# PytorchConnectomics/pytorch_connectomics

Measured on AMD Instinct MI355X. Metric: voxels/s (train + sliding-window infer), MedNeXt-S 112^3 bf16, higher is better.
Workload: dtype bf16; 1 GPU; Lucchi++ sliding-window inference (configs[1]): MedNeXt-S k3, 165x1024x768 volume, roi 112^3, overlap 0.5, bump blending, sw_batch_size 8, random-init weights; step = one whole-volume EagerSlidingWindowEngine call (TTA off); value = window-voxels/s; sw_batch_size=8, window_pipeline_streams=3

## Files before the change

### include/pytc_hip.h

```cpp
#ifndef PYTC_HIP_H
#define PYTC_HIP_H

#include <stdint.h>

#ifdef __cplusplus
extern "C" {
#endif

#define PYTC_ABI_VERSION 12

#define PYTC_OK 0
#define PYTC_ERR_INVALID 1
#define PYTC_ERR_HIP 2
#define PYTC_ERR_UNSUPPORTED 3

#define PYTC_F32 0
#define PYTC_BF16 1

#define PYTC_VIEW_FLIP_Z 1
#define PYTC_VIEW_FLIP_Y 2
#define PYTC_VIEW_FLIP_X 4
#define PYTC_VIEW_SWAP_YX 8
#define PYTC_VIEW_SWAP_ZY 16
#define PYTC_VIEW_SWAP_ZX 32

#define PYTC_PAD_CONSTANT 0
#define PYTC_PAD_REFLECT 1
#define PYTC_PAD_REPLICATE 2
#define PYTC_PAD_CIRCULAR 3

#define PYTC_BLEND_PRODUCT 0
#define PYTC_BLEND_MIN 1

#define PYTC_ACT_NONE 0
#define PYTC_ACT_SIGMOID 1
#define PYTC_ACT_TANH 2
#define PYTC_ACT_GELU 3

#define PYTC_RES_NONE 0
#define PYTC_RES_ADD 1
#define PYTC_RES_UPSAMPLE 2
#define PYTC_RES_GELU_BWD 3
#define PYTC_RES_NORM_BWD 4

int pytc_abi_version(void);
const char* pytc_last_error(void);
int pytc_device_info(int device, int* cu_count, int* lds_bytes_per_cu, char* arch, int arch_len);
int pytc_set_tuning(const char* key, int value);


int pytc_gather_windows(const float* vol, int C, int Z, int Y, int X, const int32_t* starts, int B,
                        int rz, int ry, int rx, int view, int pad_mode, float cval, void* out,
                        int out_dtype, void* stream);

int pytc_blend_accumulate(const void* pred, int pred_dtype, int B, const int32_t* starts, int rz,
                          int ry, int rx, int C, int view, const float* wz, const float* wy,
                          const float* wx, int combine, float floor_w, const int32_t* border ,
                          float* value, float* weight, int Z, int Y, int X, void* stream);

int pytc_blend_accumulate_mapped(const void* pred, int pred_dtype, int B, const int32_t* starts, int rz, int ry,
                                 int rx, int C, int view, const float* wz, const float* wy, const float* wx,
                                 int combine, float floor_w, const int32_t* border, const int32_t* chan_src,
                                 const int32_t* chan_shift, float* value, float* weight, int Z, int Y, int X,
                                 void* stream);
int pytc_blend_weight_shifted(int B, const int32_t* starts, int rz, int ry, int rx, const float* wz, const float* wy,
                              const float* wx, int combine, float floor_w, const int32_t* border,
                              const int32_t* shift, float* weight, int Z, int Y, int X, void* stream);
int pytc_normalize_covered(float* value, const float* weight, int64_t n, void* stream);
int pytc_ensemble_update_masked(float* stat, float* count, const float* x, const float* cover, int64_t n, int mode,
                                void* stream);
int pytc_ensemble_finalize_masked(const float* stat, const float* count, float* out, int64_t n, int mode, void* stream);

int pytc_blend_finalize(float* value, const float* weight, int C, int64_t nvox, float clamp,
                        int act, void* stream);

#define PYTC_ACT_SOFTMAX 4
int pytc_channel_activation(float* value, int C, int64_t nvox, int channels_last, int c0, int c1, int act,
                            float scale, void* stream);

int pytc_ensemble_update(float* acc, const float* x, int64_t n, int mode, int count, void* stream);

#define PYTC_ST_U8 0
#define PYTC_ST_I8 1
#define PYTC_ST_U16 2
#define PYTC_ST_I16 3
#define PYTC_ST_I32 4
#define PYTC_ST_F16 5
#define PYTC_ST_F32 6
int pytc_scale_cast(const float* x, void* y, int64_t n, float scale, int target, void* stream);


#define PYTC_RAW_U8 0
#define PYTC_RAW_I8 1
#define PYTC_RAW_U16 2
#define PYTC_RAW_I16 3
#define PYTC_RAW_U32 4
#define PYTC_RAW_I32 5
#define PYTC_RAW_F32 6
#define PYTC_RAW_F64 7
int pytc_resample_region(const void* raw, int raw_dtype, const int64_t* strides_czyx, int C, const int32_t* tab_i0,
                         const int32_t* tab_i1, const float* tab_f, const int32_t* dims_zyx, float* out, void* stream);

#define PYTC_NORM_NONE 0
#define PYTC_NORM_ZSCORE 1
#define PYTC_NORM_MINMAX 2
#define PYTC_NORM_DIVIDE 3
int64_t pytc_window_normalize_ws_elems(int B, int64_t n);
int pytc_window_normalize(float* x, int B, int64_t n, int mode, int binarize, float threshold, float divide, const float* clip,
                          double* workspace, void* stream);


int pytc_dwconv3d_stat_slots(int N, int D, int H, int W, int C, int K, int stride, int dtype,
                             int transposed);

int pytc_dwconv3d_kernel_variant(int N, int D, int H, int W, int C, int K, int stride, int dtype, int transposed);

int pytc_dwconv3d_fwd(const void* x, void* y, const float* w, const float* bias, float* stats,
                      int N, int D, int H, int W, int C, int K, int stride, int dtype,
                      void* stream);

int pytc_dwconv3d_fwd_wide(const void* x, void* y, const float* w, const float* bias, float* stats, int N, int D, int H,
                           int W, int C, int K, int stride, int dtype, void* stream);

int pytc_dwconv3d_res_supported(int D, int H, int W, int C, int K, int stride, int dtype);

int pytc_dwmix_supported(int D, int H, int W, int C, int C_hid, int C_out, int dtype);
int pytc_dwmix_fwd(const void* x, const float* taps, const float* dw_bias, const void* w2n, const float* b2n, const void* w3_f16,
                   const float* b3, int residual, void* y, const void* head_w, const float* head_b, float* head_y, int n_head, int N,
                   int D, int H, int W, int C, int C_hid, int C_out, int dtype, void* stream);
int pytc_dwconv3d_fwd_res(const void* x, const void* res, void* y, const float* w, const float* bias, int N, int D, int H,
                          int W, int C, int K, int stride, int dtype, void* stream);

int pytc_dwconvT3d_fwd(const void* x, void* y, const float* w, const float* bias, float* stats,
                       int N, int D, int H, int W, int C, int K, int dtype, void* stream);

int pytc_groupnorm_finalize(const float* stats, int slots, float count, const float* gamma,
                            const float* beta, float eps, float* ab, int N, int C, void* stream);


int64_t pytc_pw_packed_elems(int C_out, int C_in, int dtype);
int pytc_pw_pack_weight(const float* w, int C_out, int C_in, int transposed, void* packed,
                        int dtype, void* stream);

typedef struct {
  const void* x;
  const void* w_packed;
  const float* bias;
  const float* ab;
  const void* res;
  void* y;
  int N;
  int64_t rows_per_sample;
  int C_in, C_out;
  int in_dtype, out_dtype, w_dtype;
  int act;
  int res_mode;
  int gather;
  int Di, Hi, Wi;
  const void* res_low;
  const float* res_bias;
  int pre_act;
  int w_paired;
} pytc_pw_args;

int pytc_pw_conv_fwd(const pytc_pw_args* a, void* stream);
int pytc_pw_conv_paired_supported(const pytc_pw_args* a);
int pytc_pw_conv_rowmajor_supported(const pytc_pw_args* a);

typedef struct {
  const void* t;
  const float* ab;
  const void* w2_packed;
  const float* b2;
  const void* w3_packed;
  const float* b3;
  const void* res;
  const void* res_low;
  const float* res_bias;
  void* y;
  int N;
  int64_t rows_per_sample;
  int C_in, C_hid, C_out;
  int res_mode;
  int Di, Hi, Wi;
  int w3_format;
  int per_sample;
} pytc_mlp_args;
#define PYTC_W3_BF16 0
#define PYTC_W3_F16 1

int pytc_pw_gemm_supported(int C_in, int C_out);
int pytc_pw_gemm_fwd(const void* x, const void* w, const float* bias, const float* ab, void* y, int N, int64_t rows_per_sample,
                     int C_in, int C_out, int in_f16, int gelu_out, const void* res, const void* res_low, const float* res_bias,
                     int res_mode, int Di, int Hi, int Wi, void* stream);
int pytc_pw_mlp_supported(int C_in, int C_hid, int C_out);
int pytc_pw_pack_weight_paired(const float* w, int C_out, int C_in, int transposed, void* packed_bf16,
                               void* stream);
int pytc_pack_multi(const int64_t* table_dev, int n_items, int64_t total_elems, void* stream);
int pytc_pw_pack_weight_paired_f16(const float* w, int C_out, int C_in, int transposed, void* packed_f16,
                                   void* stream);
int pytc_pw_mlp_fwd(const pytc_mlp_args* a, void* stream);

int pytc_pw_mlp_lds_supported(int C_in, int C_hid, int C_out);
int pytc_pw_mlp_lds_fwd(const pytc_mlp_args* a, void* stream);
int pytc_pw_mlp_dma_applies(const pytc_mlp_args* a, int ignore_res_mode);
int pytc_pw_mlp_proj_supported(int C_in, int C_hid, int C_out, int C_proj);
int pytc_pw_mlp_proj_fwd(const pytc_mlp_args* a, const void* proj_w, const float* proj_b, void* z, int store_y, void* stream);
int pytc_pw_mlp_chunk_supported(int C_in, int C_hid, int C_out);
int pytc_pw_mlp_chunk_fwd(const pytc_mlp_args* a, void* stream);
int pytc_groupnorm_fold_mlp(const float* stats, int slots, float count, const float* gamma, const float* beta, float eps,
                            const float* w2, const float* b2, void* w2n, float* b2n, float* ab_out, int N, int C, int C_hid,
                            void* stream);
int pytc_pw_mlp_train_fwd(const pytc_mlp_args* a, void* hidden_pre, void* stream);
int pytc_pw_mlp_train_fwd_nostore(const pytc_mlp_args* a, void* stream);
int pytc_pw_mlp_bwd(const pytc_mlp_args* a, const void* hidden_pre, void* d_hidden, void* stream);
int pytc_pw_mlp_up_supported(int C_in, int C_hid, int C_out);
int pytc_pw_mlp_up_fwd(const pytc_mlp_args* a, const float* taps, const float* dw_bias, void* stream);
int pytc_pw_mlp_head_supported(int C_in, int C_hid, int C_out);
int pytc_pw_mlp_stemres_fwd(const pytc_mlp_args* a, const float* stem_x, const float* stem_w, const float* stem_b,
                            void* stream);
int pytc_stem_dwconv3d_stat_slots(int D, int H, int W);
int pytc_stem_dwconv3d_supported(int C_in, int C, int K);
int pytc_stem_dwconv3d_mfma_image_bytes(void);
int pytc_stem_dwconv3d_pack_mfma(const float* wx, const float* wb, const float* cst, void* image, void* stream);
int pytc_stem_dwconv3d_fwd(const float* x, const float* wx, const float* wb, const float* cst, const void* mfma_image, void* y,
                           float* stats, int N, int D, int H, int W, int C, void* stream);
int pytc_pw_mlp_head_fwd(const pytc_mlp_args* a, const void* head_w, const float* head_b, float* head_y, int n_head,
                         int store_y, void* stream);


#define PYTC_ACT_RELU 5
#define PYTC_ACT_LEAKY 6
#define PYTC_ACT_ELU 7

typedef struct {
  const void* x;
  const void* w_packed;
  const float* bias;
  const float* ab;
  const void* res;
  void* y;
  int N, D, H, W, C_in, C_out;
  int kd, kh, kw;
  int act_in;
  float act_param;
  int res_mode;
  int dtype;
} pytc_conv3d_args;

int64_t pytc_conv3d_packed_elems(int C_out, int C_in, int kd, int kh, int kw, int dtype);
int pytc_conv3d_pack_weight(const float* w, int C_out, int C_in, int kd, int kh, int kw, void* packed, int dtype,
                            void* stream);
int pytc_conv3d_fwd(const pytc_conv3d_args* a, void* stream);

int pytc_channel_stats_slots(int64_t rows);
int pytc_channel_stats(const void* x, float* stats, int N, int64_t rows, int C, int dtype, void* stream);
int pytc_norm_finalize_groups(const float* stats, int slots, float count, const float* gamma, const float* beta,
                              float eps, int groups, float* ab, int N, int C, void* stream);
int pytc_affine_act(const void* x, void* y, const float* ab, int N, int64_t rows, int C, int act, float prm,
                    int dtype, void* stream);
int pytc_maxpool3d_fwd(const void* x, void* y, int N, int D, int H, int W, int C, int fz, int fy, int fx, int dtype,
                       void* stream);
int pytc_dwconvT3d_generic_fwd(const void* x, void* y, const float* w, int N, int D, int H, int W, int C,
                               const int32_t* kernel, const int32_t* stride, const int32_t* pad, int dtype,
                               void* stream);


int pytc_groupnorm_finalize_mr(const float* stats, int slots, float count, const float* gamma, const float* beta,
                               float eps, float* ab, float* mean_rstd, int N, int C, void* stream);
int pytc_gelu(const void* x, const void* dy, void* out, int64_t n, int dtype, void* stream);
int pytc_add_inplace(void* y, const void* x, int64_t n, int dtype, void* stream);
int pytc_pw_wgrad_slots(int64_t rows_total);
int pytc_pw_wgrad(const void* x, const float* ab, const void* dy, float* dW, float* db, float* workspace, int N,
                  int64_t rows_per_sample, int C_in, int C_out, int dtype, int x_act , void* stream);
int pytc_dw_wgrad_slots(int N, const int32_t* gdims, const int32_t* xdims, int C, int K, int stride, int dtype);
int pytc_dw_wgrad(const void* g, const void* x, float* dW, float* db, float* workspace, int N, const int32_t* gdims,
                  const int32_t* xdims, int C, int K, int stride, int dtype, void* stream);

int pytc_pw_wgrad_partial(const void* x, const float* ab, const void* dy, float* workspace, int want_db, int N,
                          int64_t rows_per_sample, int C_in, int C_out, int dtype, int x_act, int* slots_out, void* stream);
int pytc_pw_wgrad_dgrad_supported(int C_in, int C_out, int dtype);
int pytc_pw_wgrad_dgrad_partial(const void* x, const void* dy, const void* w_t_paired, void* dx, float* workspace, int want_db, int N,
                                int64_t rows_per_sample, int C_in, int C_out, int dtype, int* slots_out, void* stream);
int pytc_mixer_bwd_rc_supported(int C, int C_hid, int C_out, int dtype);
int pytc_mixer_bwd_rc_sps(int N, int64_t rows_per_sample, int C_hid);
int64_t pytc_mixer_bwd_rc_ws_elems(int N, int64_t rows_per_sample, int C_hid, int gn);
int pytc_mixer_bwd_rc(const void* t, const float* ab, const float* mean_rstd, const void* dy, const void* w2_paired, const float* b2,
                      const void* w3t_paired, const float* W2, const float* gamma, float count, void* dhp, float* workspace,
                      float* s_out, float* coef, int want_db3, int gn, int N, int64_t rows_per_sample, int C, int C_hid, int C_out,
                      int dtype, int* slots_out, void* stream);
int pytc_dw_wgrad_partial(const void* g, const void* x, float* workspace, int want_db, int N, const int32_t* gdims,
                          const int32_t* xdims, int C, int K, int stride, int dtype, int* slots_out, void* stream);
int pytc_copy_zero_front(const void* src, void* dst, int N, const int32_t* dims, int C, int dtype, void* stream);
typedef struct {
  const float* part;
  float* out;
  int64_t n;
  int32_t slots;
  int32_t out_t;
} pytc_reduce_item;
int pytc_reduce_slots_multi(const pytc_reduce_item* items, int n_items, void* stream);
int pytc_norm_bwd_ws_elems(int N, int64_t rows, int C);
int pytc_norm_bwd(const void* dtn, const void* t, const float* mean_rstd, const float* gamma, float* stats_ws,
                  float* s_out, void* dt, int N, int64_t rows, float count , int C,
                  int dtype, void* stream);
int pytc_pw_wgrad_groupnorm_supported(int C, int C_hid, int dtype);
int pytc_pw_wgrad_groupnorm_sps(int N, int64_t rows_per_sample, int C, int C_hid);
int64_t pytc_pw_wgrad_groupnorm_ws_elems(int N, int64_t rows_per_sample, int C, int C_hid);
int pytc_pw_wgrad_groupnorm(const void* t, const float* mean_rstd, const float* ab, const void* dhp, const float* W2,
                            const float* gamma, float count, float* s_out, float* coef, float* workspace, int N,
                            int64_t rows_per_sample, int C, int C_hid, int dtype, void* stream);
int pytc_norm_bwd_apply(const void* dtn, const void* t, const float* mean_rstd, const float* gamma, const float* s_in,
                        int s_parts, void* dt, int N, int64_t rows, int C, float count, int dtype, const int32_t* crop_grid,
                        void* stream);
int pytc_dwconv3d_bwd_data(const void* dy, const float* w, void* dx, int N, const int32_t* xdims,
                           const int32_t* ydims, int C, int K, int stride, int dtype, void* stream);
int pytc_dwconv3d_bwd_data_add(const void* dy, const float* w, const void* addend, void* dx, int N, const int32_t* xdims,
                               const int32_t* ydims, int C, int K, int stride, int dtype, void* stream);

int pytc_conv3d_pack_weight_dgrad(const float* w, int C_out, int C_in, int kd, int kh, int kw, void* packed, int dtype,
                                  void* stream);
int pytc_conv3d_pack_plan(int C_out, int C_in, int kd, int kh, int kw, int dtype, int direct, int64_t* out);
int pytc_conv3d_pack_multi(const int64_t* table_dev, int n_items, int64_t total_blocks, void* stream);
int pytc_conv3d_launch_plan(int N, int D, int H, int W, int C_in, int C_out, int kd, int kh, int kw, int dtype, int has_pre,
                            int has_res, int phase, int64_t* out);
int pytc_norm_bwd_means(const float* s, const float* gamma, float* M, float* dgamma, float* dbeta, int N, int C, int groups,
                        float rows, void* stream);
int pytc_bn_train_finalize_cpad(const float* stats, int slots_total, float count, const float* gamma, const float* beta, float eps,
                                float momentum, float* running_mean, float* running_var, int64_t* num_batches_tracked, float* ab,
                                float* mean_rstd, int N, int C, int C_real, void* stream);
int pytc_norm_finalize_groups_cpg(const float* stats, int slots, float count, const float* gamma, const float* beta, float eps,
                                  int groups, int cpg, float* ab, float* mr, int N, int C, void* stream);
int pytc_norm_bwd_means_cpg(const float* s, const float* gamma, float* M, float* dgamma, float* dbeta, int N, int C, int groups,
                            int cpg, float rows, void* stream);
int pytc_bn_train_finalize(const float* stats, int slots_total, float count, const float* gamma, const float* beta, float eps,
                           float momentum, float* running_mean, float* running_var, int64_t* num_batches_tracked, float* ab,
                           float* mean_rstd, int N, int C, void* stream);
int pytc_bn_update_running(const float* mean_rstd, float* running_mean, float* running_var, int C, float count, float eps,
                           float momentum, void* stream);
int64_t pytc_conv3d_wgrad_ws_elems(int N, int D, int H, int W, int C_in, int C_out, const int32_t* kernel, int dtype);
int pytc_conv3d_wgrad(const void* a, const void* dy, float* dW, float* workspace, int N, int D, int H, int W, int C_in,
                      int C_out, const int32_t* kernel, int dtype, void* stream);
int pytc_act_bwd(const void* da, const void* x, const float* ab, void* dt, void* dp, int N, int64_t rows, int C, int act,
                 float prm, int dtype, void* stream);
int pytc_norm_finalize_groups_mr(const float* stats, int slots, float count, const float* gamma, const float* beta,
                                 float eps, int groups, float* ab, float* mr, int N, int C, void* stream);
int pytc_norm_bwd_stats(const void* dtn, const void* t, const float* mean_rstd, float* stats_ws, float* s_out, int N,
                        int64_t rows, int C, int dtype, void* stream);
int pytc_norm_bwd_apply_general(const void* d, const void* x, const float* mean_rstd, const float* gamma, const float* M,
                                void* dx, int N, int64_t rows, int C, int dtype, void* stream);
int pytc_act_norm_bwd_stats(const void* da, const void* x, const float* ab, const float* mean_rstd, float* stats_ws, float* s_out,
                            float* p_ws, float* p_out, int N, int64_t rows, int C, int act, float prm, int dtype, void* stream);
int pytc_act_norm_bwd_apply(const void* da, const void* x, const float* ab, const float* mean_rstd, const float* gamma,
                            const float* M, void* dx, int N, int64_t rows, int C, int act, float prm, int dtype, void* stream);
int pytc_act_norm_bwd_apply_cg(const void* da, const void* x, const float* ab, const float* mean_rstd, const float* gamma, int C_gamma,
                               const float* M, void* dx, int N, int64_t rows, int C, int act, float prm, int dtype, void* stream);
int pytc_maxpool3d_bwd(const void* x, const void* dy, void* dx, int N, int D, int H, int W, int C, int fz, int fy, int fx,
                       int dtype, void* stream);
int pytc_dwconv3d_generic_fwd(const void* x, void* y, const float* w, int N, int D, int H, int W, int C,
                              const int32_t* kernel, const int32_t* stride, const int32_t* pad, const int32_t* out_dims,
                              int dtype, void* stream);

int64_t pytc_conv3d_direct_packed_elems(int C_out, int C_in, int kd, int kh, int kw, int dtype);
int pytc_conv3d_pack_weight_direct(const float* w, int C_out, int C_in, int kd, int kh, int kw, int64_t s_o, int64_t s_c,
                                   int flip, void* packed, int dtype, void* stream);
int pytc_convT3d_c1_fwd(const void* x, const float* w, const float* bias, void* y, float* workspace, int N, const int32_t* in_dims,
                        int C_in, int dtype, void* stream);
int pytc_convT3d_phase_plan(int C_out, int C_in, int dtype, int64_t* out);
int pytc_convT3d_phase_supported(int C_out, int C_in, int dtype);
int pytc_convT3d_phase_fwd(const pytc_conv3d_args* a, const int32_t* in_dims, void* stream);
int pytc_conv3d_strided_fwd(const pytc_conv3d_args* a, const int32_t* in_dims, const int32_t* stride, const int32_t* pad,
                            int transposed, void* stream);
int64_t pytc_conv3d_wgrad_strided_ws_elems(int N, const int32_t* small_dims, int C_k, int C_o, const int32_t* kernel);
// ... 159 lines not shown
```

### pytorch_connectomics_amd/csrc/pw_common.h

```cpp
#pragma once
#include "pytc_common.h"

namespace pytc {

template <typename TW>
struct Mma;

template <>
struct Mma<bf16_t> {
  static constexpr int EPL = 8;
  static constexpr int KSTEP = 32;
  typedef bf16x8_t frag_t;
  static __device__ __forceinline__ f32x4_t mma(frag_t a, frag_t b, f32x4_t c) {
    return __builtin_amdgcn_mfma_f32_16x16x32_bf16(a, b, c, 0, 0, 0);
  }
  static __device__ __forceinline__ frag_t from_floats(const float (&v)[8]) {
    f32x8_t f;
#pragma unroll
    for (int i = 0; i < 8; ++i) f[i] = v[i];
    return __builtin_convertvector(f, frag_t);
  }
};

template <>
struct Mma<float> {
  static constexpr int EPL = 4;
  static constexpr int KSTEP = 16;
  typedef f32x4_t frag_t;
  static __device__ __forceinline__ f32x4_t mma(frag_t a, frag_t b, f32x4_t c) {
#pragma unroll
    for (int s = 0; s < 4; ++s) c = __builtin_amdgcn_mfma_f32_16x16x4f32(a[s], b[s], c, 0, 0, 0);
    return c;
  }
  static __device__ __forceinline__ frag_t from_floats(const float (&v)[4]) {
    frag_t f;
#pragma unroll
    for (int i = 0; i < 4; ++i) f[i] = v[i];
    return f;
  }
};

static_assert(Mma<bf16_t>::KSTEP == mfma_kstep(PYTC_BF16) && Mma<float>::KSTEP == mfma_kstep(PYTC_F32) &&
                  Mma<bf16_t>::EPL == elems_per_16b(PYTC_BF16) && Mma<float>::EPL == elems_per_16b(PYTC_F32),
              "the host helpers of pytc_common.h must agree with the fragment traits");

__host__ __device__ __forceinline__ int paired_row(int T, int m) {
  return (T >> 1) * 32 + (m >> 2) * 8 + (T & 1) * 4 + (m & 3);
}

struct EpiParams {
  const void* res;
  const void* res_low;
  const float* res_bias;
  void* y;
  long rps_out;
  int C_out;
  int res_mode;
  int Go_d, Go_h, Go_w;
  int Gl_d, Gl_h, Gl_w;
  int nt;
};

typedef unsigned int pytc_u32x4_t __attribute__((ext_vector_type(4)));
template <typename V>
__device__ __forceinline__ V ld_stream(const V* ptr, int nt) {
  static_assert(sizeof(V) == 16, "16-byte row pieces");
  if (nt) return __builtin_bit_cast(V, __builtin_nontemporal_load(reinterpret_cast<const pytc_u32x4_t*>(ptr)));
  return *ptr;
}

template <typename TO, int NCH, bool GELU_BWD = false, int COUT = 0>
__device__ __forceinline__ void finish_and_store(float (&v)[NCH], const EpiParams& e, int n, long orow, int o0,
                                                 const float* pre = nullptr, const int* pos = nullptr) {
  const int C_out = COUT > 0 ? COUT : e.C_out;
  TO* yn = reinterpret_cast<TO*>(e.y) + (long)n * e.rps_out * C_out;
  const TO* resn = e.res ? reinterpret_cast<const TO*>(e.res) + (long)n * e.rps_out * C_out : nullptr;
  const long off = orow * C_out + o0;
  const bool full = (C_out % NCH) == 0 && (o0 + NCH <= C_out);
  if (e.res_mode == PYTC_RES_ADD) {
    float rv[NCH];
    if (pre) {
#pragma unroll
      for (int i = 0; i < NCH; ++i) rv[i] = pre[i];
    } else if (full) VecIO<TO, NCH>::load(resn + off, rv);
    else {
#pragma unroll
      for (int i = 0; i < NCH; ++i) rv[i] = (o0 + i < C_out) ? to_f32<TO>(resn[off + i]) : 0.f;
    }
#pragma unroll
    for (int i = 0; i < NCH; ++i) v[i] += rv[i];
  } else if (GELU_BWD && e.res_mode == PYTC_RES_GELU_BWD) {
    float rv[NCH];
    if (pre) {
#pragma unroll
      for (int i = 0; i < NCH; ++i) rv[i] = pre[i];
    } else if (full) VecIO<TO, NCH>::load(resn + off, rv);
    else {
#pragma unroll
      for (int i = 0; i < NCH; ++i) rv[i] = (o0 + i < C_out) ? to_f32<TO>(resn[off + i]) : 0.f;
    }
#pragma unroll
    for (int i = 0; i < NCH; ++i) v[i] *= gelu_erf_grad(rv[i]);
  } else if (GELU_BWD && e.res_mode == PYTC_RES_NORM_BWD) {
    float rv[NCH];
    if (pre) {
#pragma unroll
      for (int i = 0; i < NCH; ++i) rv[i] = pre[i];
    } else if (full) VecIO<TO, NCH>::load(resn + off, rv);
    else {
#pragma unroll
      for (int i = 0; i < NCH; ++i) rv[i] = (o0 + i < C_out) ? to_f32<TO>(resn[off + i]) : 0.f;
    }
    const float* cf = e.res_bias + (long)n * 3 * C_out + o0;
#pragma unroll
    for (int i = 0; i < NCH; ++i)
      if (o0 + i < C_out) v[i] = fmaf(cf[i], v[i], fmaf(cf[C_out + i], rv[i], cf[2 * C_out + i]));
    if (e.Go_w > 0) {
      const unsigned ur = (unsigned)orow, gw = (unsigned)e.Go_w, gh = (unsigned)e.Go_h;
      const unsigned tq = ur / gw;
      const int px = (int)(ur - tq * gw), pz = (int)(tq / gh), py = (int)(tq - (unsigned)pz * gh);
      if (px == 0 || py == 0 || pz == 0) return;
      const long crow = ((long)(pz - 1) * (e.Go_h - 1) + (py - 1)) * (e.Go_w - 1) + (px - 1);
      TO* yc = reinterpret_cast<TO*>(e.y) + ((long)n * (e.Go_d - 1) * (e.Go_h - 1) * (e.Go_w - 1) + crow) * C_out + o0;
      if (full) VecIO<TO, NCH>::store(yc, v);
      else {
#pragma unroll
        for (int i = 0; i < NCH; ++i)
          if (o0 + i < C_out) yc[i] = from_f32<TO>(v[i]);
      }
      return;
    }
  } else if (e.res_mode == PYTC_RES_UPSAMPLE) {
    int px, py, pz;
    if (pos) { pz = pos[0]; py = pos[1]; px = pos[2]; }
    else {
      const unsigned ur = (unsigned)orow, gw = (unsigned)e.Go_w, gh = (unsigned)e.Go_h;
      const unsigned t = ur / gw;
      px = (int)(ur - t * gw);
      pz = (int)(t / gh);
      py = (int)(t - (unsigned)pz * gh);
    }
    float sk[NCH];
    if (pre) {
#pragma unroll
      for (int i = 0; i < NCH; ++i) sk[i] = pre[i];
    } else if (full) VecIO<TO, NCH>::load(resn + off, sk);
    else {
#pragma unroll
      for (int i = 0; i < NCH; ++i) sk[i] = (o0 + i < C_out) ? to_f32<TO>(resn[off + i]) : 0.f;
    }
    if (px == 0 || py == 0 || pz == 0) {
#pragma unroll
      for (int i = 0; i < NCH; ++i) v[i] = sk[i];
    } else {
      const int oz = pz - 1, oy = py - 1, ox = px - 1;
      float rl[NCH];
      if (e.res_low && !((oz | oy | ox) & 1)) {
        const TO* rp = reinterpret_cast<const TO*>(e.res_low) +
                       ((((long)n * e.Gl_d + (oz >> 1)) * e.Gl_h + (oy >> 1)) * e.Gl_w + (ox >> 1)) * C_out + o0;
        if (full) VecIO<TO, NCH>::load(rp, rl);
        else {
#pragma unroll
          for (int i = 0; i < NCH; ++i) rl[i] = (o0 + i < C_out) ? to_f32<TO>(rp[i]) : 0.f;
        }
      } else {
#pragma unroll
        for (int i = 0; i < NCH; ++i) rl[i] = (e.res_bias && o0 + i < C_out) ? e.res_bias[o0 + i] : 0.f;
      }
#pragma unroll
      for (int i = 0; i < NCH; ++i) v[i] = v[i] + rl[i] + sk[i];
    }
  }
  if (full) {
    if constexpr (sizeof(TO) == 2 && NCH == 8) {
      if (e.nt) {
        f32x8_t f;
#pragma unroll
        for (int i = 0; i < 8; ++i) f[i] = v[i];
        __builtin_nontemporal_store(__builtin_convertvector(f, bf16x8_t), reinterpret_cast<bf16x8_t*>(yn + off));
        return;
      }
    }
    VecIO<TO, NCH>::store(yn + off, v);
  } else {
#pragma unroll
    for (int i = 0; i < NCH; ++i)
      if (o0 + i < C_out) yn[off + i] = from_f32<TO>(v[i]);
  }
}

template <typename TI, int EPL>
__device__ __forceinline__ void load_row_frag(const TI* __restrict__ row, int k0, int C_in, bool vec_ok,
                                              float (&v)[EPL]) {
  if (vec_ok && k0 + EPL <= C_in) {
    if constexpr (sizeof(TI) == 4 && EPL == 8) {
      float t0[4], t1[4];
      VecIO<float, 4>::load(reinterpret_cast<const float*>(row) + k0, t0);
      VecIO<float, 4>::load(reinterpret_cast<const float*>(row) + k0 + 4, t1);
#pragma unroll
      for (int i = 0; i < 4; ++i) { v[i] = t0[i]; v[4 + i] = t1[i]; }
    } else {
      VecIO<TI, EPL>::load(row + k0, v);
    }
  } else {
#pragma unroll
    for (int j = 0; j < EPL; ++j) v[j] = (k0 + j < C_in) ? to_f32<TI>(row[k0 + j]) : 0.f;
  }
}

template <int PER>
struct WarmRegs { unsigned int r[2 * PER]; };
template <int PER>
__device__ __forceinline__ void warm_l2(const void* base, long bytes, WarmRegs<PER>& w, int first) {
  const long lines = (bytes + 127) >> 7;
  const long lin = (long)blockIdx.z * gridDim.y * gridDim.x + (long)blockIdx.y * gridDim.x + blockIdx.x;
  const long total = (long)gridDim.x * gridDim.y * gridDim.z;
  const long per_xcd = (total + 7) >> 3;
  const long stride = per_xcd * blockDim.x;
  long l = (lin >> 3) * blockDim.x + threadIdx.x;
#pragma unroll
  for (int it = 0; it < PER; ++it, l += stride) {
    const long lc = l < lines ? l : lines - 1;
    const char* ptr = reinterpret_cast<const char*>(base) + (lc << 7);
    asm volatile("global_load_dword %0, %1, off" : "=v"(w.r[first + it]) : "v"(ptr) : "memory");
  }
}
template <int PER>
__device__ __forceinline__ void warm_l2_done(WarmRegs<PER>& w) {
  asm volatile("s_waitcnt vmcnt(0)" : : : "memory");
#pragma unroll
  for (int i = 0; i < 2 * PER; ++i) asm volatile("" : : "v"(w.r[i]) : "memory");
}

__device__ __forceinline__ float apply_act(float t, int act) {
  if (act == PYTC_ACT_GELU) return gelu_erf(t);
  if (act == PYTC_ACT_SIGMOID) return 1.f / (1.f + __expf(-t));
  if (act == PYTC_ACT_TANH) return tanhf(t);
  return t;
}

}
```

### pytorch_connectomics_amd/csrc/pw_fast_kernels.hip

```cpp
#include "pw_common.h"

namespace pytc {

struct PwFastParams {
  const bf16_t* x;
  const bf16x8_t* w;
  const float* bias;
  const float* ab;
  EpiParams e;
  long rps, rps_in;
  int C_in, C_out, pre_act;
  int gather, Hi, Wi, Ho, Wo;
};

constexpr int pw_fast_waves(int ks, int nt) {
  return nt == 4 ? (ks <= 2 ? 3 : 2) : (ks <= 4 ? 4 : (ks <= 16 ? 3 : 1));
}

template <int KS, int NT>
__global__ void __launch_bounds__(256, pw_fast_waves(KS, NT))
pw_fast_kernel(PwFastParams p) {
  const int wave = threadIdx.x >> 6, lane = threadIdx.x & 63;
  const int n = blockIdx.y;
  constexpr bool WARM = KS >= 4;
  WarmRegs<2> warm;
  if (WARM) {
    const long wbytes = (long)p.C_out * p.C_in * 2;
    warm_l2(p.w, wbytes, warm, 0);
    warm_l2(reinterpret_cast<const char*>(p.w) + (wbytes >> 1), wbytes >> 1, warm, 2);
  }
  const long row0 = ((long)blockIdx.x * 4 + wave) * (NT * 16);
  if (row0 >= p.rps) {
    if (WARM) asm volatile("s_waitcnt vmcnt(0)" : : : "memory");
    return;
  }
  const int r = lane & 15, kb = lane >> 4;
  long orow[NT];
#pragma unroll
  for (int nt = 0; nt < NT; ++nt) orow[nt] = row0 + nt * 16 + r;

  bf16x8_t bact[KS][NT];
  const bf16_t* xn = p.x + (long)n * p.rps_in * p.C_in;
  {
    uint4 raw[KS][NT];
#pragma unroll
    for (int ks = 0; ks < KS; ++ks)
#pragma unroll
      for (int nt = 0; nt < NT; ++nt) {
        long rr = orow[nt] < p.rps ? orow[nt] : p.rps - 1;
        if (p.gather == 2) {
          const int ox = (int)(rr % p.Wo);
          const long t = rr / p.Wo;
          const int oy = (int)(t % p.Ho), oz = (int)(t / p.Ho);
          rr = ((long)(2 * oz) * p.Hi + 2 * oy) * p.Wi + 2 * ox;
        }
        raw[ks][nt] = *reinterpret_cast<const uint4*>(xn + rr * p.C_in + ks * 32 + kb * 8);
      }
    if (p.ab || p.pre_act == PYTC_ACT_GELU) {
      const float* an = p.ab ? p.ab + (long)n * 2 * p.C_in : nullptr;
#pragma unroll
      for (int ks = 0; ks < KS; ++ks) {
        const int k0 = ks * 32 + kb * 8;
        float av[8], bv[8];
        if (an) {
          VecIO<float, 4>::load(an + k0, reinterpret_cast<float(&)[4]>(av[0]));
          VecIO<float, 4>::load(an + k0 + 4, reinterpret_cast<float(&)[4]>(av[4]));
          VecIO<float, 4>::load(an + p.C_in + k0, reinterpret_cast<float(&)[4]>(bv[0]));
          VecIO<float, 4>::load(an + p.C_in + k0 + 4, reinterpret_cast<float(&)[4]>(bv[4]));
        }
#pragma unroll
        for (int nt = 0; nt < NT; ++nt) {
          float v[8];
          VecIO<bf16_t, 8>::load(reinterpret_cast<const bf16_t*>(&raw[ks][nt]), v);
          if (an) {
#pragma unroll
            for (int j = 0; j < 8; ++j) v[j] = fmaf(v[j], av[j], bv[j]);
          }
          if (p.pre_act == PYTC_ACT_GELU) {
#pragma unroll
            for (int j = 0; j < 8; ++j) v[j] = gelu_fast(v[j]);
          }
          bact[ks][nt] = Mma<bf16_t>::from_floats(v);
        }
      }
    } else {
#pragma unroll
      for (int ks = 0; ks < KS; ++ks)
#pragma unroll
        for (int nt = 0; nt < NT; ++nt) bact[ks][nt] = __builtin_bit_cast(bf16x8_t, raw[ks][nt]);
    }
  }

  if (WARM) warm_l2_done(warm);
  const bool pre_ok = p.e.res_mode == PYTC_RES_ADD || p.e.res_mode == PYTC_RES_GELU_BWD || p.e.res_mode == PYTC_RES_NORM_BWD;
  const bf16_t* resn = pre_ok ? reinterpret_cast<const bf16_t*>(p.e.res) + (long)n * p.rps * p.C_out : nullptr;
  const int pairs_z = p.C_out / 32 / (int)gridDim.z;
  for (int pr = blockIdx.z * pairs_z; pr < (int)(blockIdx.z + 1) * pairs_z; ++pr) {
    const int o0 = pr * 32 + kb * 8;
    uint4 rpre[NT];
    if (pre_ok) {
#pragma unroll
      for (int nt = 0; nt < NT; ++nt) {
        const long rr = orow[nt] < p.rps ? orow[nt] : p.rps - 1;
        rpre[nt] = *reinterpret_cast<const uint4*>(resn + rr * p.C_out + o0);
      }
    }
    float b[8];
#pragma unroll
    for (int j = 0; j < 8; ++j) b[j] = 0.f;
    if (p.bias) {
      VecIO<float, 4>::load(p.bias + o0, reinterpret_cast<float(&)[4]>(b[0]));
      VecIO<float, 4>::load(p.bias + o0 + 4, reinterpret_cast<float(&)[4]>(b[4]));
    }
    f32x4_t acc[2][NT];
#pragma unroll
    for (int nt = 0; nt < NT; ++nt) {
      acc[0][nt] = f32x4_t{b[0], b[1], b[2], b[3]};
      acc[1][nt] = f32x4_t{b[4], b[5], b[6], b[7]};
    }
#pragma unroll
    for (int mt = 0; mt < 2; ++mt)
#pragma unroll
      for (int ks = 0; ks < KS; ++ks) {
        const bf16x8_t a = p.w[((long)(pr * 2 + mt) * KS + ks) * 64 + lane];
#pragma unroll
        for (int nt = 0; nt < NT; ++nt) acc[mt][nt] = Mma<bf16_t>::mma(a, bact[ks][nt], acc[mt][nt]);
      }
#pragma unroll
    for (int nt = 0; nt < NT; ++nt) {
      if (orow[nt] >= p.rps) continue;
      float v[8];
#pragma unroll
      for (int j = 0; j < 4; ++j) { v[j] = acc[0][nt][j]; v[4 + j] = acc[1][nt][j]; }
      if (pre_ok) {
        float pre[8];
        VecIO<bf16_t, 8>::load(reinterpret_cast<const bf16_t*>(&rpre[nt]), pre);
        finish_and_store<bf16_t, 8, true>(v, p.e, n, orow[nt], o0, pre);
      } else {
        finish_and_store<bf16_t, 8, true>(v, p.e, n, orow[nt], o0);
      }
    }
  }
}

template <int KS, int NT>
static void launch_fast(const PwFastParams& p, int N, hipStream_t s) {
  const long rows_per_block = 4L * NT * 16;
  const long row_blocks = (p.rps + rows_per_block - 1) / rows_per_block * N;
  int zsplit = 1;
  while (row_blocks * zsplit < 512 && (p.C_out / 32) % (zsplit * 2) == 0) zsplit *= 2;
  dim3 grid((unsigned)((p.rps + rows_per_block - 1) / rows_per_block), (unsigned)N, (unsigned)zsplit), block(256);
  hipLaunchKernelGGL((pw_fast_kernel<KS, NT>), grid, block, 0, s, p);
}

bool pw_fast_supported(const pytc_pw_args* a) {
  if (a->in_dtype != PYTC_BF16 || a->out_dtype != PYTC_BF16 || a->w_dtype != PYTC_BF16) return false;
  if (a->C_in % 32 || a->C_out % 32 || (a->gather != 0 && a->gather != 2) || a->act != PYTC_ACT_NONE) return false;
  if (a->gather == 2 && a->res_mode == PYTC_RES_UPSAMPLE) return false;
  const int ks = a->C_in / 32;
  return ks == 1 || ks == 2 || ks == 4 || ks == 8 || ks == 16 || ks == 32;
}

void pw_fast_launch(const pytc_pw_args* a, const EpiParams& e, hipStream_t s) {
  PwFastParams p;
  p.x = (const bf16_t*)a->x; p.w = (const bf16x8_t*)a->w_packed; p.bias = a->bias; p.ab = a->ab; p.e = e;
  p.rps = a->rows_per_sample; p.rps_in = a->rows_per_sample; p.C_in = a->C_in; p.C_out = a->C_out; p.pre_act = a->pre_act;
  p.gather = a->gather; p.Hi = p.Wi = p.Ho = p.Wo = 0;
  if (a->gather == 2) {
    p.Hi = a->Hi; p.Wi = a->Wi; p.Ho = (a->Hi - 1) / 2 + 1; p.Wo = (a->Wi - 1) / 2 + 1;
    p.rps_in = (long)a->Di * a->Hi * a->Wi;
  }
  switch (a->C_in / 32) {
    case 1: launch_fast<1, 4>(p, a->N, s); break;
    case 2: launch_fast<2, 4>(p, a->N, s); break;
    case 4: launch_fast<4, 2>(p, a->N, s); break;
    case 8: launch_fast<8, 2>(p, a->N, s); break;
    case 16: launch_fast<16, 1>(p, a->N, s); break;
    default: launch_fast<32, 1>(p, a->N, s); break;
  }
}

}
```

### pytorch_connectomics_amd/csrc/pw_mlp_kernels.hip

```cpp
#include <cmath>
#include "pw_common.h"

namespace pytc {

struct MlpParams {
  const bf16_t* t;
  const float* ab;
  const bf16x8_t* w2;
  const float* b2;
  const bf16x8_t* w3;
  const float* b3;
  EpiParams e;
  long rps;
  int C_in, C_hid, C_out, HC;
  int w3_f16;
  long w2_stride;
  const bf16x8_t* head_w;
  const float* head_b;
  float* head_y;
  int n_head, store_y;
  bf16_t* proj_y;
  const float* stem_x;
  const float* stem_w;
  const float* stem_b;
  bf16_t* hp;
  int round_h;
  const bf16_t* hp_in;
};

constexpr int mlp_waves_per_simd(int ks, int mo, int nt) {
  if (ks >= 8 && nt == 1) return 1;
  const int regs = ks * nt * 4 + mo * nt * 4 + 2 * nt * 4;
  return regs <= 64 ? 4 : (regs <= 112 ? 3 : (regs <= 200 ? 2 : 1));
}

template <int KS_IN, int MO, int NT, int GELU_MODE, bool HEAD = false, bool STEMRES = false, bool STOREH = false, bool BWD = false>
__global__ void __launch_bounds__(256, mlp_waves_per_simd(KS_IN, MO, NT))
pw_mlp_kernel(MlpParams p) {
  constexpr int CIN = KS_IN * 32, COUT = MO * 16;
  static_assert(MO % 2 == 0, "C_out must be a multiple of 32");
  static_assert(!STEMRES || (MO == 2 && (MO / 2) * NT <= 4), "the stem-recomputing residual covers C_out = 32");
  static_assert(!HEAD || MO == 2, "the fused head covers C_out = 32");
  static_assert(GELU_MODE == 1 || GELU_MODE == 3, "sigmoid-form or packed-fp16 GELU");
  constexpr bool PREFETCH_RES = (MO / 2) * NT <= 4;
  const int wave = threadIdx.x >> 6, lane = threadIdx.x & 63;
  const int n = blockIdx.y;
  constexpr bool WARM = KS_IN * MO >= 32;
  constexpr int WPER = KS_IN * MO >= 512 ? 6 : 2;
  WarmRegs<WPER> warm;
  const bool folded = p.ab == nullptr;
  const bf16x8_t* w2 = p.w2 + (folded ? (long)n * p.w2_stride : 0L);
  const float* b2 = p.b2 + (folded ? (long)n * p.C_hid : 0L);
  if (WARM) {
    warm_l2(w2, (long)p.C_hid * CIN * 2, warm, 0);
    warm_l2(p.w3, (long)COUT * p.C_hid * 2, warm, WPER);
  }
  const long row0 = ((long)blockIdx.x * 4 + wave) * (NT * 16);
  if (row0 >= p.rps) {
    if (WARM) asm volatile("s_waitcnt vmcnt(0)" : : : "memory");
    return;
  }
  const int r = lane & 15, kb = lane >> 4;

  long orow[NT];
#pragma unroll
  for (int nt = 0; nt < NT; ++nt) orow[nt] = row0 + nt * 16 + r;

  bf16x8_t bact[KS_IN][NT];
  const bf16_t* tn = p.t + (long)n * p.rps * CIN;
  if (folded) {
#pragma unroll
    for (int ks = 0; ks < KS_IN; ++ks)
#pragma unroll
      for (int nt = 0; nt < NT; ++nt) {
        const long rr = orow[nt] < p.rps ? orow[nt] : p.rps - 1;
        bact[ks][nt] = ld_stream(reinterpret_cast<const bf16x8_t*>(tn + rr * CIN + ks * 32 + kb * 8), p.e.nt);
      }
  }
  const float* an = p.ab + (long)n * 2 * CIN;
#pragma unroll
  for (int ks = 0; ks < KS_IN; ++ks) {
    if (folded) break;
    const int k0 = ks * 32 + kb * 8;
    float av[8], bv[8];
    VecIO<float, 4>::load(an + k0, reinterpret_cast<float(&)[4]>(av[0]));
    VecIO<float, 4>::load(an + k0 + 4, reinterpret_cast<float(&)[4]>(av[4]));
    VecIO<float, 4>::load(an + CIN + k0, reinterpret_cast<float(&)[4]>(bv[0]));
    VecIO<float, 4>::load(an + CIN + k0 + 4, reinterpret_cast<float(&)[4]>(bv[4]));
#pragma unroll
    for (int nt = 0; nt < NT; ++nt) {
      const long rr = orow[nt] < p.rps ? orow[nt] : p.rps - 1;
      float v[8];
      VecIO<bf16_t, 8>::load(tn + rr * CIN + k0, v);
#pragma unroll
      for (int j = 0; j < 8; ++j) v[j] = fmaf(v[j], av[j], bv[j]);
      bact[ks][nt] = Mma<bf16_t>::from_floats(v);
    }
  }

  if (WARM) warm_l2_done(warm);

  uint4 rpre[PREFETCH_RES ? MO / 2 : 1][PREFETCH_RES ? NT : 1];
  const bool use_pre = PREFETCH_RES && p.e.res_mode != PYTC_RES_NONE;
  if constexpr (STEMRES) {
    const float* sx = p.stem_x + (long)n * p.rps;
    float sw[8], sb[8];
    VecIO<float, 4>::load(p.stem_w + kb * 8, reinterpret_cast<float(&)[4]>(sw[0]));
    VecIO<float, 4>::load(p.stem_w + kb * 8 + 4, reinterpret_cast<float(&)[4]>(sw[4]));
    VecIO<float, 4>::load(p.stem_b + kb * 8, reinterpret_cast<float(&)[4]>(sb[0]));
    VecIO<float, 4>::load(p.stem_b + kb * 8 + 4, reinterpret_cast<float(&)[4]>(sb[4]));
#pragma unroll
    for (int nt = 0; nt < NT; ++nt) {
      const float xv = sx[orow[nt] < p.rps ? orow[nt] : p.rps - 1];
      float rv[8];
#pragma unroll
      for (int j = 0; j < 8; ++j) rv[j] = fmaf(sw[j], xv, sb[j]);
      rpre[0][nt] = __builtin_bit_cast(uint4, Mma<bf16_t>::from_floats(rv));
    }
  } else if (use_pre) {
    const bf16_t* resn = reinterpret_cast<const bf16_t*>(p.e.res) + (long)n * p.rps * COUT;
#pragma unroll
    for (int pr = 0; pr < (PREFETCH_RES ? MO / 2 : 1); ++pr)
#pragma unroll
      for (int nt = 0; nt < (PREFETCH_RES ? NT : 1); ++nt) {
        const long rr = orow[nt] < p.rps ? orow[nt] : p.rps - 1;
        rpre[pr][nt] = ld_stream(reinterpret_cast<const uint4*>(resn + rr * COUT + pr * 32 + kb * 8), p.e.nt);
      }
  }

  f32x4_t acc2[MO][NT];
#pragma unroll
  for (int pr = 0; pr < MO / 2; ++pr) {
    float b[8];
    VecIO<float, 4>::load(p.b3 + pr * 32 + kb * 8, reinterpret_cast<float(&)[4]>(b[0]));
    VecIO<float, 4>::load(p.b3 + pr * 32 + kb * 8 + 4, reinterpret_cast<float(&)[4]>(b[4]));
#pragma unroll
    for (int nt = 0; nt < NT; ++nt) {
      acc2[2 * pr][nt] = f32x4_t{b[0], b[1], b[2], b[3]};
      acc2[2 * pr + 1][nt] = f32x4_t{b[4], b[5], b[6], b[7]};
    }
  }

  for (int hc = 0; hc < p.HC; ++hc) {
    float b2v[8];
    VecIO<float, 4>::load(b2 + hc * 32 + kb * 8, reinterpret_cast<float(&)[4]>(b2v[0]));
    VecIO<float, 4>::load(b2 + hc * 32 + kb * 8 + 4, reinterpret_cast<float(&)[4]>(b2v[4]));
    f32x4_t acc1[2][NT];
#pragma unroll
    for (int nt = 0; nt < NT; ++nt) {
      acc1[0][nt] = f32x4_t{b2v[0], b2v[1], b2v[2], b2v[3]};
      acc1[1][nt] = f32x4_t{b2v[4], b2v[5], b2v[6], b2v[7]};
    }
#pragma unroll
    for (int mt = 0; mt < 2; ++mt) {
#pragma unroll
      for (int ks = 0; ks < KS_IN; ++ks) {
        const bf16x8_t a = w2[((long)(hc * 2 + mt) * KS_IN + ks) * 64 + lane];
#pragma unroll
        for (int nt = 0; nt < NT; ++nt) acc1[mt][nt] = Mma<bf16_t>::mma(a, bact[ks][nt], acc1[mt][nt]);
      }
    }
    bf16x8_t bh[NT];
    h8_t bhh[GELU_MODE == 3 ? NT : 1];
#pragma unroll
    for (int nt = 0; nt < NT; ++nt) {
      float g[8];
      if constexpr (BWD) {
        const long rr = orow[nt] < p.rps ? orow[nt] : p.rps - 1;
        float hv[8];
        VecIO<bf16_t, 8>::load(p.hp_in + ((long)n * p.rps + rr) * p.C_hid + hc * 32 + kb * 8, hv);
#pragma unroll
        for (int j = 0; j < 4; ++j) {
          g[j] = acc1[0][nt][j] * gelu_erf_grad(hv[j]);
          g[4 + j] = acc1[1][nt][j] * gelu_erf_grad(hv[4 + j]);
        }
        bh[nt] = Mma<bf16_t>::from_floats(g);
        if (orow[nt] < p.rps)
          *reinterpret_cast<bf16x8_t*>(p.hp + ((long)n * p.rps + orow[nt]) * p.C_hid + hc * 32 + kb * 8) = bh[nt];
        continue;
      }
      if constexpr (STOREH) {
        float pre[8];
#pragma unroll
        for (int j = 0; j < 4; ++j) { pre[j] = acc1[0][nt][j]; pre[4 + j] = acc1[1][nt][j]; }
        const bf16x8_t hb = Mma<bf16_t>::from_floats(pre);
        if (p.hp && orow[nt] < p.rps)
          *reinterpret_cast<bf16x8_t*>(p.hp + ((long)n * p.rps + orow[nt]) * p.C_hid + hc * 32 + kb * 8) = hb;
        const f32x8_t hr = __builtin_convertvector(hb, f32x8_t);
#pragma unroll
        for (int j = 0; j < 4; ++j) { acc1[0][nt][j] = hr[j]; acc1[1][nt][j] = hr[4 + j]; }
      }
      if constexpr (GELU_MODE == 3) {
#pragma unroll
        for (int j = 0; j < 4; ++j) { g[j] = acc1[0][nt][j]; g[4 + j] = acc1[1][nt][j]; }
        bhh[nt] = gelu_h8_from_f32(g);
        continue;
      }
#pragma unroll
      for (int j = 0; j < 4; ++j) {
        g[j] = gelu_fast(acc1[0][nt][j]);
        g[4 + j] = gelu_fast(acc1[1][nt][j]);
      }
      bh[nt] = Mma<bf16_t>::from_floats(g);
    }
#pragma unroll
    for (int mo = 0; mo < MO; ++mo) {
      if constexpr (GELU_MODE == 3) {
        const h8_t a = reinterpret_cast<const h8_t*>(p.w3)[((long)mo * p.HC + hc) * 64 + lane];
#pragma unroll
        for (int nt = 0; nt < NT; ++nt) acc2[mo][nt] = __builtin_amdgcn_mfma_f32_16x16x32_f16(a, bhh[nt], acc2[mo][nt], 0, 0, 0);
      } else {
        const bf16x8_t a = p.w3[((long)mo * p.HC + hc) * 64 + lane];
#pragma unroll
        for (int nt = 0; nt < NT; ++nt) acc2[mo][nt] = Mma<bf16_t>::mma(a, bh[nt], acc2[mo][nt]);
      }
    }
  }

  if constexpr (HEAD) {
    bf16_t* yn = reinterpret_cast<bf16_t*>(p.e.y) + (long)n * p.rps * 32;
    const bf16_t* resn = p.e.res ? reinterpret_cast<const bf16_t*>(p.e.res) + (long)n * p.rps * 32 : nullptr;
    float* hy = p.head_y + (long)n * p.rps * p.n_head;
    const bf16x8_t ah = p.head_w[lane];
    float hb[4];
#pragma unroll
    for (int i = 0; i < 4; ++i) hb[i] = (p.head_b && kb * 4 + i < p.n_head) ? p.head_b[kb * 4 + i] : 0.f;
#pragma unroll
    for (int nt = 0; nt < NT; ++nt) {
      float v[8];
#pragma unroll
      for (int j = 0; j < 4; ++j) { v[j] = acc2[0][nt][j]; v[4 + j] = acc2[1][nt][j]; }
      const bool live = orow[nt] < p.rps;
      if (p.e.res_mode == PYTC_RES_ADD) {
        float rv[8];
        if (use_pre) VecIO<bf16_t, 8>::load(reinterpret_cast<const bf16_t*>(&rpre[0][PREFETCH_RES ? nt : 0]), rv);
        else VecIO<bf16_t, 8>::load(resn + (live ? orow[nt] : p.rps - 1) * 32 + kb * 8, rv);
#pragma unroll
        for (int j = 0; j < 8; ++j) v[j] += rv[j];
      }
      const bf16x8_t ob = Mma<bf16_t>::from_floats(v);
      if (p.store_y && live) *reinterpret_cast<bf16x8_t*>(yn + orow[nt] * 32 + kb * 8) = ob;
      const f32x4_t h = Mma<bf16_t>::mma(ah, ob, f32x4_t{0.f, 0.f, 0.f, 0.f});
      if (live) {
#pragma unroll
        for (int i = 0; i < 4; ++i)
          if (kb * 4 + i < p.n_head) hy[orow[nt] * p.n_head + kb * 4 + i] = h[i] + hb[i];
      }
    }
    return;
  }
  int upos[NT][3];
  const bool ups = p.e.res_mode == PYTC_RES_UPSAMPLE;
  if (ups) {
    const unsigned ur = (unsigned)row0, gw = (unsigned)p.e.Go_w, gh = (unsigned)p.e.Go_h;
    const unsigned t0 = ur / gw;
    const int bx = (int)(ur - t0 * gw);
    const int bz = (int)(t0 / gh);
    const int by = (int)(t0 - (unsigned)bz * gh);
#pragma unroll
    for (int nt = 0; nt < NT; ++nt) {
      int px = bx + nt * 16 + r, py = by, pz = bz;
      while (px >= p.e.Go_w) { px -= p.e.Go_w; ++py; }
      while (py >= p.e.Go_h) { py -= p.e.Go_h; ++pz; }
      upos[nt][0] = pz; upos[nt][1] = py; upos[nt][2] = px;
    }
  }
#pragma unroll
  for (int pr = 0; pr < MO / 2; ++pr) {
#pragma unroll
    for (int nt = 0; nt < NT; ++nt) {
      if (orow[nt] >= p.rps) continue;
      float v[8];
#pragma unroll
      for (int j = 0; j < 4; ++j) {
        v[j] = acc2[2 * pr][nt][j];
        v[4 + j] = acc2[2 * pr + 1][nt][j];
      }
      if (use_pre) {
        float pre[8];
        VecIO<bf16_t, 8>::load(reinterpret_cast<const bf16_t*>(&rpre[PREFETCH_RES ? pr : 0][PREFETCH_RES ? nt : 0]), pre);
        finish_and_store<bf16_t, 8, false, COUT>(v, p.e, n, orow[nt], pr * 32 + kb * 8, pre, ups ? upos[nt] : nullptr);
      } else {
        finish_and_store<bf16_t, 8, false, COUT>(v, p.e, n, orow[nt], pr * 32 + kb * 8, nullptr, ups ? upos[nt] : nullptr);
      }
    }
  }
}


__device__ __forceinline__ void glds16(const void* gsrc, unsigned lds_dst) {
  unsigned keep;
  asm volatile("s_mov_b32 %0, m0\n\ts_mov_b32 m0, %2\n\ts_nop 0\n\tglobal_load_lds_dwordx4 %1, off\n\ts_mov_b32 m0, %0"
               : "=&s"(keep) : "v"(gsrc), "s"(lds_dst) : "memory");
}
__device__ __forceinline__ void glds4(const void* gsrc, unsigned lds_dst) {
  unsigned keep;
  asm volatile("s_mov_b32 %0, m0\n\ts_mov_b32 m0, %2\n\ts_nop 0\n\tglobal_load_lds_dword %1, off\n\ts_mov_b32 m0, %0"
               : "=&s"(keep) : "v"(gsrc), "s"(lds_dst) : "memory");
}

template <int HCT, int KIND>
__global__ void __launch_bounds__(256, 3)
pw_mlp_dma_kernel(MlpParams p, int waves_per_sample) {
  constexpr int NT = 4, CIN = 32, COUT = 32;
  constexpr bool STEM = KIND == 1, HEAD = KIND == 2, PROJ = KIND == 3;
  __shared__ __attribute__((aligned(16))) uint4 land[4][2][NT * 64];
  __shared__ __attribute__((aligned(16))) uint4 w2s[HCT * 2 * 64], w3s[2 * HCT * 64];
  __shared__ __attribute__((aligned(16))) float b2s[HCT * 32], b3s[32];
  __shared__ __attribute__((aligned(16))) float auxa[STEM ? 32 : (HEAD ? 256 : (PROJ ? 512 : 4))], auxb[(STEM || PROJ) ? 32 : (HEAD ? 16 : 4)];
  const int wave = threadIdx.x >> 6, lane = threadIdx.x & 63;
  const int n = blockIdx.y;
  const int r = lane & 15, kb = lane >> 4;
  const long tiles = (p.rps + NT * 16 - 1) / (NT * 16);
  const bool with_res = STEM || p.e.res_mode == PYTC_RES_ADD;
  const bf16_t* tn = p.t + (long)n * p.rps * CIN;
  const bf16_t* resn = (!STEM && with_res) ? reinterpret_cast<const bf16_t*>(p.e.res) + (long)n * p.rps * COUT : nullptr;
  const float* sx = STEM ? p.stem_x + (long)n * p.rps : nullptr;
  bf16_t* yn = reinterpret_cast<bf16_t*>(p.e.y) + (long)n * p.rps * COUT;
  float* hy = HEAD ? p.head_y + (long)n * p.rps * p.n_head : nullptr;
  bf16_t* zn = PROJ ? p.proj_y + (long)n * p.rps * 32 : nullptr;
  {
    const uint4* w2 = reinterpret_cast<const uint4*>(p.w2 + (long)n * p.w2_stride);
    const uint4* w3 = reinterpret_cast<const uint4*>(p.w3);
    for (int i = threadIdx.x; i < HCT * 2 * 64; i += 256) { w2s[i] = w2[i]; w3s[i] = w3[i]; }
    if (threadIdx.x < HCT * 32) b2s[threadIdx.x] = p.b2[(long)n * p.C_hid + threadIdx.x];
    if (threadIdx.x < 32) b3s[threadIdx.x] = p.b3[threadIdx.x];
    if constexpr (STEM) {
      if (threadIdx.x < 32) { auxa[threadIdx.x] = p.stem_w[threadIdx.x]; auxb[threadIdx.x] = p.stem_b[threadIdx.x]; }
    }
    if constexpr (HEAD) {
      reinterpret_cast<float*>(auxa)[threadIdx.x] = reinterpret_cast<const float*>(p.head_w)[threadIdx.x];
      if (threadIdx.x < 16) auxb[threadIdx.x] = (p.head_b && (int)threadIdx.x < p.n_head) ? p.head_b[threadIdx.x] : 0.f;
    }
    if constexpr (PROJ) {
      auxa[threadIdx.x] = reinterpret_cast<const float*>(p.head_w)[threadIdx.x];
      auxa[threadIdx.x + 256] = reinterpret_cast<const float*>(p.head_w)[threadIdx.x + 256];
      if (threadIdx.x < 32) auxb[threadIdx.x] = p.head_b ? p.head_b[threadIdx.x] : 0.f;
    }
  }
  __syncthreads();
  asm volatile("s_waitcnt vmcnt(0)" ::: "memory");

  const unsigned lbase = __builtin_amdgcn_readfirstlane((unsigned)(size_t)(__attribute__((address_space(3))) void*)&land[wave][0][0]);
  auto request = [&](long tile) {
#pragma unroll
    for (int nt = 0; nt < NT; ++nt) {
      long row = tile * (NT * 16) + nt * 16 + r;
      row = row < p.rps ? row : p.rps - 1;
      glds16(tn + row * CIN + kb * 8, lbase + (unsigned)(nt * 64) * 16);
      if constexpr (STEM) glds4(sx + row, lbase + (unsigned)(NT * 64) * 16 + (unsigned)(nt * 64) * 4);
      else if (with_res) glds16(resn + row * COUT + kb * 8, lbase + (unsigned)((NT + nt) * 64) * 16);
    }
  };
  bf16x8_t out[NT];
  f32x4_t hout[HEAD ? NT : 1];
  bf16x8_t zout[PROJ ? NT : 1];
  auto store = [&](long tile) {
#pragma unroll
    for (int nt = 0; nt < NT; ++nt) {
      const long row = tile * (NT * 16) + nt * 16 + r;
      if (row >= p.rps) continue;
      if (!(HEAD || PROJ) || p.store_y) *reinterpret_cast<bf16x8_t*>(yn + row * COUT + kb * 8) = out[nt];
      if constexpr (PROJ) *reinterpret_cast<bf16x8_t*>(zn + row * 32 + kb * 8) = zout[nt];
      if constexpr (HEAD) {
#pragma unroll
        for (int i = 0; i < 4; ++i)
          if (kb * 4 + i < p.n_head) hy[row * p.n_head + kb * 4 + i] = hout[nt][i];
      }
    }
  };
  const long gw = (long)blockIdx.x * 4 + wave;
  long tile = gw;
  if (tile >= tiles) return;
  request(tile);
  long out_tile = -1;
  for (; tile < tiles; tile += waves_per_sample) {
    asm volatile("s_waitcnt vmcnt(0)" ::: "memory");
    __builtin_amdgcn_wave_barrier();
    if (out_tile >= 0) store(out_tile);
    bf16x8_t bact[NT];
    uint4 rpre[STEM ? 1 : NT];
    float xin[STEM ? NT : 1];
#pragma unroll
    for (int nt = 0; nt < NT; ++nt) {
      bact[nt] = __builtin_bit_cast(bf16x8_t, land[wave][0][nt * 64 + lane]);
      if constexpr (STEM) xin[nt] = reinterpret_cast<const float*>(&land[wave][1][0])[nt * 64 + lane];
      else if (with_res) rpre[nt] = land[wave][1][nt * 64 + lane];
    }
    asm volatile("s_waitcnt lgkmcnt(0)" ::: "memory");
    __builtin_amdgcn_wave_barrier();
    if (tile + waves_per_sample < tiles) request(tile + waves_per_sample);
    f32x4_t acc2[2][NT];
    {
      const f32x4_t lo = *reinterpret_cast<const f32x4_t*>(&b3s[kb * 8]), hi = *reinterpret_cast<const f32x4_t*>(&b3s[kb * 8 + 4]);
#pragma unroll
      for (int nt = 0; nt < NT; ++nt) { acc2[0][nt] = lo; acc2[1][nt] = hi; }
    }
#pragma unroll
    for (int hc = 0; hc < HCT; ++hc) {
      f32x4_t acc1[2][NT];
      {
        const f32x4_t lo = *reinterpret_cast<const f32x4_t*>(&b2s[hc * 32 + kb * 8]), hi = *reinterpret_cast<const f32x4_t*>(&b2s[hc * 32 + kb * 8 + 4]);
#pragma unroll
        for (int nt = 0; nt < NT; ++nt) { acc1[0][nt] = lo; acc1[1][nt] = hi; }
      }
#pragma unroll
      for (int mt = 0; mt < 2; ++mt) {
        const bf16x8_t a2 = __builtin_bit_cast(bf16x8_t, w2s[(hc * 2 + mt) * 64 + lane]);
#pragma unroll
        for (int nt = 0; nt < NT; ++nt) acc1[mt][nt] = Mma<bf16_t>::mma(a2, bact[nt], acc1[mt][nt]);
      }
      h8_t bhh[NT];
#pragma unroll
      for (int nt = 0; nt < NT; ++nt) {
        float g[8];
#pragma unroll
        for (int j = 0; j < 4; ++j) { g[j] = acc1[0][nt][j]; g[4 + j] = acc1[1][nt][j]; }
        bhh[nt] = gelu_h8_from_f32(g);
      }
#pragma unroll
      for (int mo = 0; mo < 2; ++mo) {
        const h8_t a3 = __builtin_bit_cast(h8_t, w3s[(mo * HCT + hc) * 64 + lane]);
#pragma unroll
        for (int nt = 0; nt < NT; ++nt) acc2[mo][nt] = __builtin_amdgcn_mfma_f32_16x16x32_f16(a3, bhh[nt], acc2[mo][nt], 0, 0, 0);
      }
    }
    float sw[STEM ? 8 : 1], sb[STEM ? 8 : 1];
    if constexpr (STEM) {
#pragma unroll
      for (int j = 0; j < 8; ++j) { sw[j] = auxa[kb * 8 + j]; sb[j] = auxb[kb * 8 + j]; }
    }
// ... 273 lines not shown
  PYTC_MLP_CASE(4, 4, 2)
  PYTC_MLP_CASE(4, 8, 2)
  PYTC_MLP_CASE(4, 16, 1)
  PYTC_MLP_CASE(8, 8, 2)
  PYTC_MLP_CASE(8, 16, 1)
  PYTC_MLP_CASE(8, 32, 1)
  PYTC_MLP_CASE(16, 16, 1)
  PYTC_MLP_CASE(16, 32, 1)
#undef PYTC_MLP_CASE
  return false;
}

static bool mlp_shape_ok(int C_in, int C_hid, int C_out) {
  if (C_in % 32 || C_hid % 32 || C_out % 32 || C_in < 32 || C_out < 32 || C_hid < 32) return false;
  const int ks = C_in / 32, mo = C_out / 16;
  static const int ok[][2] = {{1, 2}, {1, 4}, {2, 2}, {2, 4}, {2, 8}, {4, 4}, {4, 8}, {4, 16}, {8, 8},
                              {8, 16}, {8, 32}, {16, 16}, {16, 32}};
  for (auto& c : ok)
    if (c[0] == ks && c[1] == mo) return true;
  return false;
}

}

using namespace pytc;

extern "C" int pytc_pw_mlp_supported(int C_in, int C_hid, int C_out) { return mlp_shape_ok(C_in, C_hid, C_out) ? 1 : 0; }

extern "C" int pytc_groupnorm_fold_mlp(const float* stats, int slots, float count, const float* gamma, const float* beta,
                                       float eps, const float* w2, const float* b2, void* w2n, float* b2n, float* ab_out, int N,
                                       int C, int C_hid, void* stream) {
  PYTC_REQUIRE(stats && w2 && w2n && b2n && slots >= 1 && count > 0 && N >= 1, "groupnorm_fold_mlp: bad arguments");
  PYTC_REQUIRE(C == 32 || C == 64 || C == 128, "groupnorm_fold_mlp: C=%d (32, 64 or 128)", C);
  PYTC_REQUIRE(C_hid % 32 == 0 && C_hid >= 32 && C_hid <= 512, "groupnorm_fold_mlp: C_hid=%d", C_hid);
  hipLaunchKernelGGL(groupnorm_fold_mlp_kernel, dim3(N), dim3(1024), 0, (hipStream_t)stream, stats, slots, count, gamma, beta,
                     eps, w2, b2, (bf16_t*)w2n, b2n, ab_out, C, C_hid);
  PYTC_LAUNCH_CHECK("groupnorm_fold_mlp");
  return PYTC_OK;
}

extern "C" int pytc_pw_mlp_head_supported(int C_in, int C_hid, int C_out) {
  return (C_out == 32 && (C_in == 32 || C_in == 64) && C_hid % 32 == 0 && C_hid >= 32) ? 1 : 0;
}

extern "C" int pytc_pw_pack_weight_paired(const float* w, int C_out, int C_in, int transposed, void* packed,
                                          void* stream) {
  PYTC_REQUIRE(w && packed && C_out >= 1 && C_in >= 1, "pw_pack_weight_paired: bad arguments");
  PYTC_REQUIRE(C_out % 32 == 0, "pw_pack_weight_paired: C_out=%d must be a multiple of 32", C_out);
  long total = pytc_pw_packed_elems(C_out, C_in, PYTC_BF16);
  int KG = (C_in + 31) / 32;
  hipLaunchKernelGGL(pw_pack_paired_kernel<bf16_t>, dim3(ceil_div(total, 256)), dim3(256), 0, (hipStream_t)stream, w, C_out,
                     C_in, transposed, (bf16_t*)packed, KG, total);
  PYTC_LAUNCH_CHECK("pw_pack_weight_paired");
  return PYTC_OK;
}

extern "C" int pytc_pw_pack_weight_paired_f16(const float* w, int C_out, int C_in, int transposed, void* packed,
                                              void* stream) {
  PYTC_REQUIRE(w && packed && C_out >= 1 && C_in >= 1, "pw_pack_weight_paired_f16: bad arguments");
  PYTC_REQUIRE(C_out % 32 == 0, "pw_pack_weight_paired_f16: C_out=%d must be a multiple of 32", C_out);
  long total = pytc_pw_packed_elems(C_out, C_in, PYTC_BF16);
  int KG = (C_in + 31) / 32;
  hipLaunchKernelGGL(pw_pack_paired_kernel<_Float16>, dim3(ceil_div(total, 256)), dim3(256), 0, (hipStream_t)stream, w,
                     C_out, C_in, transposed, (_Float16*)packed, KG, total);
  PYTC_LAUNCH_CHECK("pw_pack_weight_paired_f16");
  return PYTC_OK;
}

extern "C" int pytc_pack_multi(const int64_t* table_dev, int n_items, int64_t total_elems, void* stream) {
  PYTC_REQUIRE(table_dev && n_items >= 1 && total_elems >= 1, "pack_multi: bad arguments");
  hipLaunchKernelGGL(pack_multi_kernel, dim3(ceil_div(total_elems, 256)), dim3(256), 0, (hipStream_t)stream,
                     reinterpret_cast<const long*>(table_dev), n_items, (long)total_elems);
  PYTC_LAUNCH_CHECK("pack_multi");
  return PYTC_OK;
}

extern "C" int pytc_pw_mlp_head_fwd(const pytc_mlp_args* a, const void* head_w, const float* head_b, float* head_y,
                                    int n_head, int store_y, void* stream) {
  PYTC_REQUIRE(a && a->t && (a->ab || a->per_sample) && a->w2_packed && a->w3_packed && a->b2 && a->b3 && head_w && head_y, "pw_mlp_head: null pointer");
  PYTC_REQUIRE(!(a->ab && a->per_sample), "pw_mlp_head: per-sample (norm-folded) expand operands come without an affine");
  PYTC_REQUIRE(!store_y || a->y, "pw_mlp_head: store_y without an output buffer");
  PYTC_REQUIRE(a->N >= 1 && a->rows_per_sample >= 1 && n_head >= 1 && n_head <= 16, "pw_mlp_head: bad shape");
  if (!pytc_pw_mlp_head_supported(a->C_in, a->C_hid, a->C_out)) {
    set_error("pw_mlp_head: no fused kernel for C_in=%d C_hid=%d C_out=%d", a->C_in, a->C_hid, a->C_out);
    return PYTC_ERR_UNSUPPORTED;
  }
  PYTC_REQUIRE(a->res_mode == PYTC_RES_NONE || (a->res_mode == PYTC_RES_ADD && a->res), "pw_mlp_head: residual add or none");
  MlpParams p;
  p.t = (const bf16_t*)a->t; p.ab = a->ab; p.w2 = (const bf16x8_t*)a->w2_packed; p.b2 = a->b2;
  p.w3 = (const bf16x8_t*)a->w3_packed; p.b3 = a->b3;
  p.rps = a->rows_per_sample; p.C_in = a->C_in; p.C_hid = a->C_hid; p.C_out = a->C_out; p.HC = a->C_hid / 32;
  p.w2_stride = (long)(a->C_hid / 16) * (a->C_in / 32) * 64;
  p.e.res = a->res; p.e.res_low = nullptr; p.e.res_bias = nullptr; p.e.y = a->y;
  p.e.rps_out = a->rows_per_sample; p.e.C_out = a->C_out; p.e.res_mode = a->res_mode;
  p.e.nt = 0;
  p.e.Go_d = p.e.Go_h = p.e.Go_w = p.e.Gl_d = p.e.Gl_h = p.e.Gl_w = 0;
  p.head_w = (const bf16x8_t*)head_w; p.head_b = head_b; p.head_y = head_y; p.n_head = n_head; p.store_y = store_y;
  p.w3_f16 = a->w3_format == PYTC_W3_F16 ? 1 : 0;
  dim3 grid((unsigned)((p.rps + 4L * 4 * 16 - 1) / (4L * 4 * 16)), (unsigned)a->N), block(256);
  hipStream_t s = (hipStream_t)stream;
  if (mlp_dma_applies(a, p)) {
    mlp_dma_launch<2>(a, p, s);
    PYTC_LAUNCH_CHECK("pw_mlp_head_dma");
    return PYTC_OK;
  }
  if (p.w3_f16) {
    if (a->C_in == 32) hipLaunchKernelGGL((pw_mlp_kernel<1, 2, 4, 3, true>), grid, block, 0, s, p);
    else hipLaunchKernelGGL((pw_mlp_kernel<2, 2, 4, 3, true>), grid, block, 0, s, p);
  } else if (a->C_in == 32) {
    hipLaunchKernelGGL((pw_mlp_kernel<1, 2, 4, 1, true>), grid, block, 0, s, p);
  } else {
    hipLaunchKernelGGL((pw_mlp_kernel<2, 2, 4, 1, true>), grid, block, 0, s, p);
  }
  PYTC_LAUNCH_CHECK("pw_mlp_head");
  return PYTC_OK;
}

extern "C" int pytc_pw_mlp_stemres_fwd(const pytc_mlp_args* a, const float* stem_x, const float* stem_w, const float* stem_b,
                                       void* stream) {
  PYTC_REQUIRE(a && a->t && (a->ab || a->per_sample) && a->w2_packed && a->w3_packed && a->b2 && a->b3 && a->y && stem_x && stem_w && stem_b,
               "pw_mlp_stemres: null pointer");
  PYTC_REQUIRE(!(a->ab && a->per_sample), "pw_mlp_stemres: per-sample (norm-folded) expand operands come without an affine");
  PYTC_REQUIRE(a->N >= 1 && a->rows_per_sample >= 1, "pw_mlp_stemres: bad shape");
  if (!(a->C_in == 32 && a->C_out == 32 && a->C_hid % 32 == 0 && a->C_hid >= 32)) {
    set_error("pw_mlp_stemres: no fused kernel for C_in=%d C_hid=%d C_out=%d", a->C_in, a->C_hid, a->C_out);
    return PYTC_ERR_UNSUPPORTED;
  }
  MlpParams p{};
  p.t = (const bf16_t*)a->t; p.ab = a->ab; p.w2 = (const bf16x8_t*)a->w2_packed; p.b2 = a->b2;
  p.w3 = (const bf16x8_t*)a->w3_packed; p.b3 = a->b3;
  p.rps = a->rows_per_sample; p.C_in = a->C_in; p.C_hid = a->C_hid; p.C_out = a->C_out; p.HC = a->C_hid / 32;
  p.w2_stride = (long)(a->C_hid / 16) * (a->C_in / 32) * 64;
  p.e.res = a->y;
  p.e.y = a->y;
  p.e.rps_out = a->rows_per_sample; p.e.C_out = a->C_out; p.e.res_mode = PYTC_RES_ADD;
  p.e.nt = 0;
  p.stem_x = stem_x; p.stem_w = stem_w; p.stem_b = stem_b;
  p.w3_f16 = a->w3_format == PYTC_W3_F16 ? 1 : 0;
  dim3 grid((unsigned)((p.rps + 4L * 4 * 16 - 1) / (4L * 4 * 16)), (unsigned)a->N), block(256);
  hipStream_t s = (hipStream_t)stream;
  pytc_mlp_args shape = *a;
  shape.res_mode = PYTC_RES_NONE;
  if (mlp_dma_applies(&shape, p)) {
    mlp_dma_launch<1>(a, p, s);
    PYTC_LAUNCH_CHECK("pw_mlp_stemres_dma");
    return PYTC_OK;
  }
  if (p.w3_f16) hipLaunchKernelGGL((pw_mlp_kernel<1, 2, 4, 3, false, true>), grid, block, 0, s, p);
  else hipLaunchKernelGGL((pw_mlp_kernel<1, 2, 4, 1, false, true>), grid, block, 0, s, p);
  PYTC_LAUNCH_CHECK("pw_mlp_stemres");
  return PYTC_OK;
}

extern "C" int pytc_pw_mlp_dma_applies(const pytc_mlp_args* a, int ignore_res_mode) {
  if (!a) return 0;
  MlpParams p{};
  p.HC = a->C_hid / 32;
  p.w3_f16 = a->w3_format == PYTC_W3_F16 ? 1 : 0;
  pytc_mlp_args shape = *a;
  if (ignore_res_mode) shape.res_mode = PYTC_RES_NONE;
  return mlp_dma_applies(&shape, p) ? 1 : 0;
}

extern "C" int pytc_pw_mlp_proj_supported(int C_in, int C_hid, int C_out, int C_proj) {
  return (C_in == 32 && C_out == 32 && C_proj == 32 && (C_hid == 64 || C_hid == 96 || C_hid == 128)) ? 1 : 0;
}
extern "C" int pytc_pw_mlp_proj_fwd(const pytc_mlp_args* a, const void* proj_w, const float* proj_b, void* z, int store_y, void* stream) {
  PYTC_REQUIRE(a && a->t && a->w2_packed && a->w3_packed && a->b2 && a->b3 && proj_w && z, "pw_mlp_proj: null pointer");
  PYTC_REQUIRE(a->per_sample && !a->ab, "pw_mlp_proj: takes the per-sample (norm-folded) expand operands");
  PYTC_REQUIRE(a->w3_format == PYTC_W3_F16, "pw_mlp_proj: the mixer's projection image must be fp16 (pytc_pw_pack_weight_paired_f16)");
  PYTC_REQUIRE(!store_y || a->y, "pw_mlp_proj: store_y without an output buffer");
  PYTC_REQUIRE(a->N >= 1 && a->rows_per_sample >= 1, "pw_mlp_proj: bad shape");
  if (!pytc_pw_mlp_proj_supported(a->C_in, a->C_hid, a->C_out, 32)) {
    set_error("pw_mlp_proj: no fused kernel for C_in=%d C_hid=%d C_out=%d", a->C_in, a->C_hid, a->C_out);
    return PYTC_ERR_UNSUPPORTED;
  }
  PYTC_REQUIRE(a->res_mode == PYTC_RES_NONE || (a->res_mode == PYTC_RES_ADD && a->res), "pw_mlp_proj: residual add or none");
  MlpParams p{};
  p.t = (const bf16_t*)a->t; p.ab = nullptr; p.w2 = (const bf16x8_t*)a->w2_packed; p.b2 = a->b2;
  p.w3 = (const bf16x8_t*)a->w3_packed; p.b3 = a->b3;
  p.rps = a->rows_per_sample; p.C_in = a->C_in; p.C_hid = a->C_hid; p.C_out = a->C_out; p.HC = a->C_hid / 32;
  p.w2_stride = (long)(a->C_hid / 16) * (a->C_in / 32) * 64;
  p.e.res = a->res; p.e.y = a->y; p.e.rps_out = a->rows_per_sample; p.e.C_out = a->C_out; p.e.res_mode = a->res_mode;
  p.head_w = (const bf16x8_t*)proj_w; p.head_b = proj_b; p.proj_y = (bf16_t*)z; p.store_y = store_y;
  p.w3_f16 = 1;
  mlp_dma_launch<3>(a, p, (hipStream_t)stream);
  PYTC_LAUNCH_CHECK("pw_mlp_proj");
  return PYTC_OK;
}

static int mlp_fwd_impl(const pytc_mlp_args* a, void* hp, void* stream, const void* hp_in = nullptr, bool round_h = false);

extern "C" int pytc_pw_mlp_bwd(const pytc_mlp_args* a, const void* hidden_pre, void* d_hidden, void* stream) {
  PYTC_REQUIRE(hidden_pre && d_hidden, "pw_mlp_bwd: null hidden buffers");
  PYTC_REQUIRE(a && a->res_mode == PYTC_RES_NONE, "pw_mlp_bwd: no residual in the backward mixer");
  return mlp_fwd_impl(a, d_hidden, stream, hidden_pre);
}

extern "C" int pytc_pw_mlp_train_fwd(const pytc_mlp_args* a, void* hidden_pre, void* stream) {
  PYTC_REQUIRE(hidden_pre, "pw_mlp_train: null hidden buffer");
  return mlp_fwd_impl(a, hidden_pre, stream);
}

extern "C" int pytc_pw_mlp_train_fwd_nostore(const pytc_mlp_args* a, void* stream) {
  return mlp_fwd_impl(a, nullptr, stream, nullptr, true);
}

extern "C" int pytc_pw_mlp_fwd(const pytc_mlp_args* a, void* stream) { return mlp_fwd_impl(a, nullptr, stream); }

static int mlp_fwd_impl(const pytc_mlp_args* a, void* hp, void* stream, const void* hp_in, bool round_h) {
  PYTC_REQUIRE(a && a->t && (a->ab || a->per_sample) && a->w2_packed && a->w3_packed && a->b2 && a->b3 && a->y, "pw_mlp: null pointer");
  PYTC_REQUIRE(!(a->ab && a->per_sample), "pw_mlp: per-sample (norm-folded) expand operands come without an affine");
  PYTC_REQUIRE(!(a->per_sample && (hp || hp_in || round_h)), "pw_mlp: the training kernels take the shared expand image and the affine");
  PYTC_REQUIRE(a->N >= 1 && a->rows_per_sample >= 1, "pw_mlp: bad shape");
  if (!mlp_shape_ok(a->C_in, a->C_hid, a->C_out)) {
    set_error("pw_mlp: no fused kernel for C_in=%d C_hid=%d C_out=%d", a->C_in, a->C_hid, a->C_out);
    return PYTC_ERR_UNSUPPORTED;
  }
  PYTC_REQUIRE(a->res_mode == PYTC_RES_NONE || a->res, "pw_mlp: residual mode without residual pointer");
  PYTC_REQUIRE(a->res_mode == PYTC_RES_NONE || a->res_mode == PYTC_RES_ADD || a->res_mode == PYTC_RES_UPSAMPLE,
               "pw_mlp: unsupported res_mode %d", a->res_mode);
  MlpParams p{};
  p.t = (const bf16_t*)a->t; p.ab = a->ab; p.w2 = (const bf16x8_t*)a->w2_packed; p.b2 = a->b2;
  p.w3 = (const bf16x8_t*)a->w3_packed; p.b3 = a->b3;
  p.rps = a->rows_per_sample; p.C_in = a->C_in; p.C_hid = a->C_hid; p.C_out = a->C_out; p.HC = a->C_hid / 32;
  p.w2_stride = (long)(a->C_hid / 16) * (a->C_in / 32) * 64;
  p.e.res = a->res; p.e.res_low = a->res_low; p.e.res_bias = a->res_bias; p.e.y = a->y;
  p.e.rps_out = a->rows_per_sample; p.e.C_out = a->C_out; p.e.res_mode = a->res_mode;
  p.e.nt = 0;
  p.e.Go_d = p.e.Go_h = p.e.Go_w = p.e.Gl_d = p.e.Gl_h = p.e.Gl_w = 0;
  p.hp = (bf16_t*)hp;
  p.hp_in = (const bf16_t*)hp_in;
  p.round_h = round_h ? 1 : 0;
  p.w3_f16 = a->w3_format == PYTC_W3_F16 ? 1 : 0;
  PYTC_REQUIRE(!(p.w3_f16 && hp_in), "pw_mlp_bwd: the backward mixer takes bf16 weight images");
  if (a->res_mode == PYTC_RES_UPSAMPLE) {
    PYTC_REQUIRE((long)a->Di * a->Hi * a->Wi == a->rows_per_sample && !(a->Di & 1) && !(a->Hi & 1) && !(a->Wi & 1),
                 "pw_mlp: RES_UPSAMPLE needs the (even) output grid");
    PYTC_REQUIRE(a->rows_per_sample < (1L << 31), "pw_mlp: RES_UPSAMPLE positions are 32-bit (rows per sample < 2^31)");
    p.e.Go_d = a->Di; p.e.Go_h = a->Hi; p.e.Go_w = a->Wi;
    p.e.Gl_d = a->Di / 2; p.e.Gl_h = a->Hi / 2; p.e.Gl_w = a->Wi / 2;
  }
  if (!hp && !hp_in && !round_h && mlp_dma_applies(a, p)) {
    mlp_dma_launch<0>(a, p, (hipStream_t)stream);
    PYTC_LAUNCH_CHECK("pw_mlp_dma");
    return PYTC_OK;
  }
  if (!dispatch_mlp(p, a->N, (hipStream_t)stream)) {
    set_error("pw_mlp: dispatch failed");
    return PYTC_ERR_UNSUPPORTED;
  }
  PYTC_LAUNCH_CHECK("pw_mlp");
  return PYTC_OK;
}
```

### pytorch_connectomics_amd/csrc/pw_mlp_lds_kernels.hip

```cpp
#include <mutex>

#include "pw_common.h"

namespace pytc {

struct MlpLdsParams {
  const bf16_t* t;
  const float* ab;
  const bf16x8_t* w2;
  const float* b2;
  const h8_t* w3;
  const float* b3;
  EpiParams e;
  long rps;
  int N, C_in, C_hid, C_out, HC;
  long w2_stride;
};

template <int KS_IN, int MO, int NT>
struct LdsTile {
  uint4 raw[KS_IN][NT];
  uint4 res[MO / 2][NT];
};

template <int KS_IN, int MO, int NT>
__device__ __forceinline__ void lds_tile_load(LdsTile<KS_IN, MO, NT>& T, const MlpLdsParams& p, int n, long row0, int r, int kb,
                                              bool with_res) {
  const bf16_t* tn = p.t + (long)n * p.rps * (KS_IN * 32);
#pragma unroll
  for (int nt = 0; nt < NT; ++nt) {
    const long o = row0 + nt * 16 + r;
    const long rr = o < p.rps ? o : p.rps - 1;
#pragma unroll
    for (int ks = 0; ks < KS_IN; ++ks) T.raw[ks][nt] = ld_stream(reinterpret_cast<const uint4*>(tn + rr * (KS_IN * 32) + ks * 32 + kb * 8), p.e.nt);
  }
  if (with_res) {
    const bf16_t* resn = reinterpret_cast<const bf16_t*>(p.e.res) + (long)n * p.rps * (MO * 16);
#pragma unroll
    for (int nt = 0; nt < NT; ++nt) {
      const long o = row0 + nt * 16 + r;
      const long rr = o < p.rps ? o : p.rps - 1;
#pragma unroll
      for (int pr = 0; pr < MO / 2; ++pr) T.res[pr][nt] = ld_stream(reinterpret_cast<const uint4*>(resn + rr * (MO * 16) + pr * 32 + kb * 8), p.e.nt);
    }
  }
}

template <int KS_IN, int MO, int NT, int NWAVES, int WPS>
__global__ void __launch_bounds__(NWAVES * 64, WPS)
pw_mlp_lds_kernel(MlpLdsParams p) {
  constexpr int CIN = KS_IN * 32, COUT = MO * 16;
  extern __shared__ __attribute__((aligned(16))) unsigned char lds_raw[];
  bf16x8_t* lw2 = reinterpret_cast<bf16x8_t*>(lds_raw);
  h8_t* lw3 = reinterpret_cast<h8_t*>(lds_raw + (size_t)p.C_hid * CIN * 2);
  float* lb2 = reinterpret_cast<float*>(lds_raw + (size_t)p.C_hid * (CIN + COUT) * 2);
  const int tid = threadIdx.x, wave = tid >> 6, lane = tid & 63;
  const int r = lane & 15, kb = lane >> 4;
  const bool folded = p.ab == nullptr;
  const int n_w2 = p.C_hid * CIN / 8, n_w3 = COUT * p.C_hid / 8;
  for (int i = tid; i < n_w3; i += NWAVES * 64) lw3[i] = p.w3[i];
  const long Ts = (p.rps + NT * 16 - 1) / (NT * 16);
  const long G = Ts * p.N;
  const long g_end = G * (blockIdx.x + 1) / gridDim.x;
  long g = G * blockIdx.x / gridDim.x;
  const bool with_res = p.e.res_mode != PYTC_RES_NONE;
  const bool ups = p.e.res_mode == PYTC_RES_UPSAMPLE;
  int staged = -1;

  while (g < g_end) {
    const int n = (int)(g / Ts);
    const long seg_end = min(g_end, (long)(n + 1) * Ts);
    if (staged < 0 || folded) {
      __syncthreads();
      const bf16x8_t* src = p.w2 + (folded ? (long)n * p.w2_stride : 0L);
      for (int i = tid; i < n_w2; i += NWAVES * 64) lw2[i] = src[i];
      const float* b2 = p.b2 + (folded ? (long)n * p.C_hid : 0L);
      for (int i = tid; i < p.C_hid; i += NWAVES * 64) lb2[i] = b2[i];
      staged = n;
      __syncthreads();
    }
    const float* an = folded ? nullptr : p.ab + (long)n * 2 * CIN;
    const long t_base = (long)n * Ts;

    for (long gt = g + wave; gt < seg_end; gt += NWAVES) {
      const long row0 = (gt - t_base) * (NT * 16);
      LdsTile<KS_IN, MO, NT> cur;
      lds_tile_load(cur, p, n, row0, r, kb, with_res);
      long orow[NT];
#pragma unroll
      for (int nt = 0; nt < NT; ++nt) orow[nt] = row0 + nt * 16 + r;

      bf16x8_t bact[KS_IN][NT];
#pragma unroll
      for (int ks = 0; ks < KS_IN; ++ks) {
        if (folded) {
#pragma unroll
          for (int nt = 0; nt < NT; ++nt) bact[ks][nt] = __builtin_bit_cast(bf16x8_t, cur.raw[ks][nt]);
        } else {
          const int k0 = ks * 32 + kb * 8;
          float av[8], bv[8];
          VecIO<float, 4>::load(an + k0, reinterpret_cast<float(&)[4]>(av[0]));
          VecIO<float, 4>::load(an + k0 + 4, reinterpret_cast<float(&)[4]>(av[4]));
          VecIO<float, 4>::load(an + CIN + k0, reinterpret_cast<float(&)[4]>(bv[0]));
          VecIO<float, 4>::load(an + CIN + k0 + 4, reinterpret_cast<float(&)[4]>(bv[4]));
#pragma unroll
          for (int nt = 0; nt < NT; ++nt) {
            float v[8];
            VecIO<bf16_t, 8>::load(reinterpret_cast<const bf16_t*>(&cur.raw[ks][nt]), v);
#pragma unroll
            for (int j = 0; j < 8; ++j) v[j] = fmaf(v[j], av[j], bv[j]);
            bact[ks][nt] = Mma<bf16_t>::from_floats(v);
          }
        }
      }
      f32x4_t acc2[MO][NT];
#pragma unroll
      for (int pr = 0; pr < MO / 2; ++pr) {
        float b[8];
        VecIO<float, 4>::load(p.b3 + pr * 32 + kb * 8, reinterpret_cast<float(&)[4]>(b[0]));
        VecIO<float, 4>::load(p.b3 + pr * 32 + kb * 8 + 4, reinterpret_cast<float(&)[4]>(b[4]));
#pragma unroll
        for (int nt = 0; nt < NT; ++nt) {
          acc2[2 * pr][nt] = f32x4_t{b[0], b[1], b[2], b[3]};
          acc2[2 * pr + 1][nt] = f32x4_t{b[4], b[5], b[6], b[7]};
        }
      }
      for (int hc = 0; hc < p.HC; ++hc) {
        const f32x4_t b2lo = *reinterpret_cast<const f32x4_t*>(lb2 + hc * 32 + kb * 8);
        const f32x4_t b2hi = *reinterpret_cast<const f32x4_t*>(lb2 + hc * 32 + kb * 8 + 4);
        f32x4_t acc1[2][NT];
#pragma unroll
        for (int nt = 0; nt < NT; ++nt) { acc1[0][nt] = b2lo; acc1[1][nt] = b2hi; }
#pragma unroll
        for (int mt = 0; mt < 2; ++mt) {
#pragma unroll
          for (int ks = 0; ks < KS_IN; ++ks) {
            const bf16x8_t a = lw2[((hc * 2 + mt) * KS_IN + ks) * 64 + lane];
#pragma unroll
            for (int nt = 0; nt < NT; ++nt) acc1[mt][nt] = Mma<bf16_t>::mma(a, bact[ks][nt], acc1[mt][nt]);
          }
        }
        h8_t bhh[NT];
#pragma unroll
        for (int nt = 0; nt < NT; ++nt) {
          float gg[8];
#pragma unroll
          for (int j = 0; j < 4; ++j) { gg[j] = acc1[0][nt][j]; gg[4 + j] = acc1[1][nt][j]; }
          bhh[nt] = gelu_h8_from_f32(gg);
        }
#pragma unroll
        for (int mo = 0; mo < MO; ++mo) {
          const h8_t a = lw3[(mo * p.HC + hc) * 64 + lane];
#pragma unroll
          for (int nt = 0; nt < NT; ++nt) acc2[mo][nt] = __builtin_amdgcn_mfma_f32_16x16x32_f16(a, bhh[nt], acc2[mo][nt], 0, 0, 0);
        }
      }
      int upos[NT][3];
      if (ups) {
        const unsigned ur = (unsigned)row0, gw = (unsigned)p.e.Go_w, gh = (unsigned)p.e.Go_h;
        const unsigned t0 = ur / gw;
        const int bx = (int)(ur - t0 * gw);
        const int bz = (int)(t0 / gh);
        const int by = (int)(t0 - (unsigned)bz * gh);
#pragma unroll
        for (int nt = 0; nt < NT; ++nt) {
          int px = bx + nt * 16 + r, py = by, pz = bz;
          while (px >= p.e.Go_w) { px -= p.e.Go_w; ++py; }
          while (py >= p.e.Go_h) { py -= p.e.Go_h; ++pz; }
          upos[nt][0] = pz; upos[nt][1] = py; upos[nt][2] = px;
        }
      }
#pragma unroll
      for (int pr = 0; pr < MO / 2; ++pr) {
#pragma unroll
        for (int nt = 0; nt < NT; ++nt) {
          if (orow[nt] >= p.rps) continue;
          float v[8];
#pragma unroll
          for (int j = 0; j < 4; ++j) { v[j] = acc2[2 * pr][nt][j]; v[4 + j] = acc2[2 * pr + 1][nt][j]; }
          if (with_res) {
            float pre[8];
            VecIO<bf16_t, 8>::load(reinterpret_cast<const bf16_t*>(&cur.res[pr][nt]), pre);
            finish_and_store<bf16_t, 8, false, COUT>(v, p.e, n, orow[nt], pr * 32 + kb * 8, pre, ups ? upos[nt] : nullptr);
          } else {
            finish_and_store<bf16_t, 8, false, COUT>(v, p.e, n, orow[nt], pr * 32 + kb * 8, nullptr, nullptr);
          }
        }
      }
    }
    g = seg_end;
  }
}

template <int KS_IN, int MO, int NT, int NWAVES, int WPS>
static void launch_mlp_lds_v(const MlpLdsParams& p, size_t lds, hipStream_t s) {
  auto kern = &pw_mlp_lds_kernel<KS_IN, MO, NT, NWAVES, WPS>;
  if (!ensure_dynamic_lds(reinterpret_cast<const void*>(kern), 160 * 1024, "pw_mlp_lds")) return;
  const long tiles = ((p.rps + NT * 16 - 1) / (NT * 16)) * p.N;
  const int by_lds = (int)((160 * 1024) / lds), by_waves = WPS * 4 / NWAVES;
  const int per_cu = by_lds < by_waves ? (by_lds < 1 ? 1 : by_lds) : by_waves;
  long blocks = 256L * per_cu;
  const long need = (tiles + NWAVES - 1) / NWAVES;
  if (blocks > need) blocks = need;
  hipLaunchKernelGGL(kern, dim3((unsigned)blocks), dim3(NWAVES * 64), lds, s, p);
}

template <int KS_IN, int MO, int NT>
static void launch_mlp_lds(const MlpLdsParams& p, int variant, hipStream_t s) {
  const size_t lds = (size_t)p.C_hid * (p.C_in + p.C_out) * 2 + (size_t)p.C_hid * 4;
  if (variant == 0) variant = (KS_IN == 4 && MO == 8) ? 3 : (MO == 2 ? 2 : 4);
  switch (variant) {
    case 1: launch_mlp_lds_v<KS_IN, MO, NT, 8, 4>(p, lds, s); break;
    case 2: launch_mlp_lds_v<KS_IN, MO, NT, 16, 4>(p, lds, s); break;
    case 3: launch_mlp_lds_v<KS_IN, MO, NT, 8, 2>(p, lds, s); break;
    default: launch_mlp_lds_v<KS_IN, MO, NT, 12, 3>(p, lds, s); break;
  }
}

}

using namespace pytc;

extern "C" int pytc_pw_mlp_lds_supported(int C_in, int C_hid, int C_out) {
  if (C_in % 32 || C_hid % 32 || C_out % 32) return 0;
  const int ks = C_in / 32, mo = C_out / 16;
  const bool shape = (ks == 2 && mo == 2) || (ks == 2 && mo == 4) || (ks == 4 && mo == 4) || (ks == 4 && mo == 8);
  const size_t lds = (size_t)C_hid * (C_in + C_out) * 2 + (size_t)C_hid * 4;
  return (shape && lds <= 160 * 1024) ? 1 : 0;
}

extern "C" int pytc_pw_mlp_lds_fwd(const pytc_mlp_args* a, void* stream) {
  PYTC_REQUIRE(a && a->t && (a->ab || a->per_sample) && a->w2_packed && a->w3_packed && a->b2 && a->b3 && a->y, "pw_mlp_lds: null pointer");
  PYTC_REQUIRE(!(a->ab && a->per_sample), "pw_mlp_lds: per-sample (norm-folded) expand operands come without an affine");
  PYTC_REQUIRE(a->w3_format == PYTC_W3_F16, "pw_mlp_lds: the projection image must be fp16 (pytc_pw_pack_weight_paired_f16)");
  PYTC_REQUIRE(a->N >= 1 && a->rows_per_sample >= 1, "pw_mlp_lds: bad shape");
  if (!pytc_pw_mlp_lds_supported(a->C_in, a->C_hid, a->C_out)) {
    set_error("pw_mlp_lds: no LDS-resident kernel for C_in=%d C_hid=%d C_out=%d", a->C_in, a->C_hid, a->C_out);
    return PYTC_ERR_UNSUPPORTED;
  }
  PYTC_REQUIRE(a->res_mode == PYTC_RES_NONE || a->res, "pw_mlp_lds: residual mode without residual pointer");
  MlpLdsParams p{};
  p.t = (const bf16_t*)a->t; p.ab = a->ab; p.w2 = (const bf16x8_t*)a->w2_packed; p.b2 = a->b2;
  p.w3 = (const h8_t*)a->w3_packed; p.b3 = a->b3;
  p.rps = a->rows_per_sample; p.N = a->N; p.C_in = a->C_in; p.C_hid = a->C_hid; p.C_out = a->C_out; p.HC = a->C_hid / 32;
  p.w2_stride = (long)(a->C_hid / 16) * (a->C_in / 32) * 64;
  p.e.res = a->res; p.e.res_low = a->res_low; p.e.res_bias = a->res_bias; p.e.y = a->y;
  p.e.rps_out = a->rows_per_sample; p.e.C_out = a->C_out; p.e.res_mode = a->res_mode;
  p.e.nt = 0;
  p.e.Go_d = p.e.Go_h = p.e.Go_w = p.e.Gl_d = p.e.Gl_h = p.e.Gl_w = 0;
  if (a->res_mode == PYTC_RES_UPSAMPLE) {
    PYTC_REQUIRE((long)a->Di * a->Hi * a->Wi == a->rows_per_sample && !(a->Di & 1) && !(a->Hi & 1) && !(a->Wi & 1) &&
                 a->rows_per_sample < (1L << 31), "pw_mlp_lds: RES_UPSAMPLE needs the (even) output grid");
    p.e.Go_d = a->Di; p.e.Go_h = a->Hi; p.e.Go_w = a->Wi;
    p.e.Gl_d = a->Di / 2; p.e.Gl_h = a->Hi / 2; p.e.Gl_w = a->Wi / 2;
  }
  hipStream_t s = (hipStream_t)stream;
  const int ks = a->C_in / 32, mo = a->C_out / 16;
  const int variant = tuning_get(K_mlp_lds_variant);
  if (ks == 2 && mo == 2) launch_mlp_lds<2, 2, 2>(p, variant, s);
  else if (ks == 2 && mo == 4) launch_mlp_lds<2, 4, 2>(p, variant, s);
  else if (ks == 4 && mo == 4) launch_mlp_lds<4, 4, 2>(p, variant, s);
  else launch_mlp_lds<4, 8, 2>(p, variant, s);
  PYTC_LAUNCH_CHECK("pw_mlp_lds");
  return PYTC_OK;
}
```

### pytorch_connectomics_amd/csrc/pytc_common.h

```cpp
#pragma once
#include <hip/hip_runtime.h>
#include <stdint.h>
#include <stdio.h>
#include <string.h>

#include "../../include/pytc_hip.h"

namespace pytc {

typedef __bf16 bf16_t;
typedef __bf16 bf16x2_t __attribute__((ext_vector_type(2)));
typedef __bf16 bf16x4_t __attribute__((ext_vector_type(4)));
typedef __bf16 bf16x8_t __attribute__((ext_vector_type(8)));
typedef float f32x2_t __attribute__((ext_vector_type(2)));
typedef float f32x4_t __attribute__((ext_vector_type(4)));
typedef float f32x8_t __attribute__((ext_vector_type(8)));
typedef float f32x16_t __attribute__((ext_vector_type(16)));
typedef short s16x8_t __attribute__((ext_vector_type(8)));

constexpr int WAVE = 64;

void set_error(const char* fmt, ...);
int hip_fail(hipError_t e, const char* what);
bool ensure_dynamic_lds(const void* kernel, size_t bytes, const char* what);
bool take_launch_failure();

#define PYTC_REQUIRE(cond, ...)                     \
  do {                                              \
    if (!(cond)) {                                  \
      pytc::set_error(__VA_ARGS__);                 \
      return PYTC_ERR_INVALID;                      \
    }                                               \
  } while (0)

#define PYTC_LAUNCH_CHECK(name)                                  \
  do {                                                           \
    if (pytc::take_launch_failure()) return PYTC_ERR_HIP;        \
    hipError_t e_ = hipGetLastError();                           \
    if (e_ != hipSuccess) return pytc::hip_fail(e_, name);       \
  } while (0)

#define PYTC_CHECK_DTYPE(dtype, what) \
  PYTC_REQUIRE((dtype) == PYTC_BF16 || (dtype) == PYTC_F32, "%s: bad dtype %d", what, (int)(dtype))

#define PYTC_DISPATCH_DTYPE(dtype, what, T, ...)      \
  do {                                                \
    if ((dtype) == PYTC_BF16) {                       \
      using T = pytc::bf16_t;                         \
      __VA_ARGS__;                                    \
    } else if ((dtype) == PYTC_F32) {                 \
      using T = float;                                \
      __VA_ARGS__;                                    \
    } else {                                          \
      PYTC_CHECK_DTYPE(dtype, what);                  \
    }                                                 \
  } while (0)

constexpr int elems_per_16b(int dtype) { return dtype == PYTC_BF16 ? 8 : 4; }
constexpr int mfma_kstep(int dtype) { return dtype == PYTC_BF16 ? 32 : 16; }
template <typename T>
constexpr int elems_per_16b_of = 16 / (int)sizeof(T);
static_assert(elems_per_16b_of<__bf16> == elems_per_16b(PYTC_BF16) && elems_per_16b_of<float> == elems_per_16b(PYTC_F32), "one width rule");

#define PYTC_KNOBS(X)                                                                                                             \
  X(channel_act_flat, 1, "channel activation of contiguous NDHWC tensors as a flat 16-byte stream; 0 = the per-voxel kernel")      \
  X(conv_wgrad_mfma, 1, "dense-conv weight gradient on the matrix cores (bf16); 0 = the VALU kernel")                              \
  X(dw_wgrad_march, 1, "depthwise K = 3 / stride 1 weight gradient as a z-march; 0 = the vector / generic kernels")                \
  X(dw_wgrad_vec, 1, "depthwise K = 3 weight gradient with 16-byte channel vectors; 0 = the generic kernel")                       \
  X(dwconvT_tile, 1, "transposed depthwise conv at C = 64 / 128 (bf16) as one tile of input cells per workgroup; 0 = cell kernel") \
  X(dwconv_march_h16, 1, "VALU z-march depthwise conv: packed-f16 in-plane partial sums; 0 = fp32 taps")                           \
  X(dwconv_mfma, 1, "bf16 stride-1 K = 3 depthwise forward (and the fused block) on the matrix cores; 0 = the VALU z-march")       \
  X(dwconv_mfma_variant, 0, "matrix-core depthwise conv: bit 0 = hi + lo weight halves, bit 1 = two planes in flight, not three")  \
  X(dwconv_s2_march, 1, "stride-2 K = 3 depthwise conv at C = 32 / 64 (bf16) as a z-march over an LDS ring; 0 = gather kernel")    \
  X(elementwise_vec, 1, "16-byte vector forms of the norm-apply / elementwise training kernels; 0 = the scalar kernels")           \
  X(mixer_bwd_rc_slot_div, 1, "recomputing mixer backward: divide the slot count (fewer, longer slots)")                           \
  X(mlp_chunk_variant, 0, "chunked-hidden mixer (pw_mlp_chunk_kernels.hip): tile shape of the launch")                             \
  X(mlp_dma, 1, "level-0 mixer with DMA-prefetched row tiles (pw_mlp_dma_kernel); 0 = one tile per wave")                          \
  X(mlp_dma_rows, 1 << 20, "fewest rows of a launch that takes the DMA mixer")                                                     \
  X(mlp_dma_wgs, 0, "DMA mixer: workgroups per sample; 0 = chosen from the row count")                                             \
  X(mlp_lds_variant, 0, "LDS-resident mixer (pw_mlp_lds_kernels.hip): tile shape of the launch")                                   \
  X(norm_bwd_from_wgrad_flat, 1, "GroupNorm-backward epilogue of the expand weight gradient as one flat kernel; 0 = chunked")      \
  X(pw_gemm_rows, 0, "LDS-tiled 1x1 GEMM: 64 / 128 forces the rows per workgroup; 0 = by problem size")                            \
  X(pw_thin, 1, "plain 1x1 convs with one input / few output channels on the thin kernels; 0 = the generic kernel")                \
  X(wgrad_dgrad_fused, 1, "projecting conv's weight gradient and the GELU-backward data gradient in one kernel; 0 = two launches")  \
  X(wgrad_small_split, 1, "matrix-core 1x1 weight gradient: more, shorter row slots when the launch would leave CUs idle")         \
  X(wgrad_valu, 0, "1: 1x1 weight gradient on the VALU kernel instead of the matrix cores")                                        \
  X(wgrad_whole_rounds, 1, "matrix-core 1x1 weight gradient: round the slot count down to whole rounds of resident workgroups")

enum Knob {
#define PYTC_KNOB_ENUM(name, dflt, doc) K_##name,
  PYTC_KNOBS(PYTC_KNOB_ENUM)
#undef PYTC_KNOB_ENUM
  K_COUNT
};
int tuning_get(Knob k);

template <typename T, int VEC>
struct VecIO;

template <int VEC>
struct VecIO<float, VEC> {
  typedef float vec_t __attribute__((ext_vector_type(VEC)));
  static __device__ __forceinline__ void load(const float* p, float (&v)[VEC]) {
    vec_t t = *reinterpret_cast<const vec_t*>(p);
#pragma unroll
    for (int i = 0; i < VEC; ++i) v[i] = t[i];
  }
  static __device__ __forceinline__ void store(float* p, const float (&v)[VEC]) {
    vec_t t;
#pragma unroll
    for (int i = 0; i < VEC; ++i) t[i] = v[i];
    *reinterpret_cast<vec_t*>(p) = t;
  }
};
template <>
struct VecIO<float, 1> {
  static __device__ __forceinline__ void load(const float* p, float (&v)[1]) { v[0] = *p; }
  static __device__ __forceinline__ void store(float* p, const float (&v)[1]) { *p = v[0]; }
};

template <int VEC>
struct VecIO<bf16_t, VEC> {
  typedef __bf16 vec_t __attribute__((ext_vector_type(VEC)));
  typedef float fvec_t __attribute__((ext_vector_type(VEC)));
  static __device__ __forceinline__ void load(const bf16_t* p, float (&v)[VEC]) {
    vec_t t = *reinterpret_cast<const vec_t*>(p);
    fvec_t f = __builtin_convertvector(t, fvec_t);
#pragma unroll
    for (int i = 0; i < VEC; ++i) v[i] = f[i];
  }
  static __device__ __forceinline__ void store(bf16_t* p, const float (&v)[VEC]) {
    fvec_t f;
#pragma unroll
    for (int i = 0; i < VEC; ++i) f[i] = v[i];
    *reinterpret_cast<vec_t*>(p) = __builtin_convertvector(f, vec_t);
  }
};
template <>
struct VecIO<bf16_t, 1> {
  static __device__ __forceinline__ void load(const bf16_t* p, float (&v)[1]) { v[0] = (float)*p; }
  static __device__ __forceinline__ void store(bf16_t* p, const float (&v)[1]) { *p = (bf16_t)v[0]; }
};

template <typename T>
__device__ __forceinline__ float to_f32(T v) { return (float)v; }
template <typename T>
__device__ __forceinline__ T from_f32(float v) { return (T)v; }

__device__ __forceinline__ float wave_sum(float v) {
#pragma unroll
  for (int o = 32; o > 0; o >>= 1) v += __shfl_xor(v, o, 64);
  return v;
}

template <int THREADS, typename T>
__device__ __forceinline__ T block_sum(T v, T* red) {
  red[threadIdx.x] = v;
  __syncthreads();
  for (int s = THREADS / 2; s > 0; s >>= 1) {
    if ((int)threadIdx.x < s) red[threadIdx.x] += red[threadIdx.x + s];
    __syncthreads();
  }
  const T r = red[0];
  __syncthreads();
  return r;
}

__device__ __forceinline__ float gelu_erf(float x) {
  const float az = fabsf(x) * 0.70710678118654752440f;
  const float t = __builtin_amdgcn_rcpf(fmaf(0.3275911f, az, 1.0f));
  float p = fmaf(t, 1.061405429f, -1.453152027f);
  p = fmaf(t, p, 1.421413741f);
  p = fmaf(t, p, -0.284496736f);
  p = fmaf(t, p, 0.254829592f);
  p *= t;
  const float pe = p * __builtin_amdgcn_exp2f(-az * az * 1.44269504088896340736f);
  const float one_plus_erf = x < 0.f ? pe : 2.0f - pe;
  return 0.5f * x * one_plus_erf;
}

__device__ __forceinline__ float gelu_erf_grad(float x) {
  const float az = fabsf(x) * 0.70710678118654752440f;
  const float t = __builtin_amdgcn_rcpf(fmaf(0.3275911f, az, 1.0f));
  float p = fmaf(t, 1.061405429f, -1.453152027f);
  p = fmaf(t, p, 1.421413741f);
  p = fmaf(t, p, -0.284496736f);
  p = fmaf(t, p, 0.254829592f);
  p *= t;
  const float e = __builtin_amdgcn_exp2f(-az * az * 1.44269504088896340736f);
  const float pe = p * e;
  const float one_plus_erf = x < 0.f ? pe : 2.0f - pe;
  return fmaf(x * 0.3989422804014327f, e, 0.5f * one_plus_erf);
}

__device__ __forceinline__ float gelu_fast(float x) {
  const float x2 = fminf(x * x, 64.0f);
  float p = fmaf(x2, 1.0142630e-3f, -1.0677572e-1f);
  p = fmaf(p, x2, -2.3011213f);
  const float e = __builtin_amdgcn_exp2f(x * p);
  return x * __builtin_amdgcn_rcpf(1.0f + e);
}

__device__ __forceinline__ void gelu_fast_with_grad(float x, float& g, float& gd) {
  const float x2 = fminf(x * x, 64.0f);
  float p = fmaf(x2, 1.0142630e-3f, -1.0677572e-1f);
  p = fmaf(p, x2, -2.3011213f);
  const float e = __builtin_amdgcn_exp2f(x * p);
  const float s = __builtin_amdgcn_rcpf(1.0f + e);
  g = x * s;
  const float q = fmaf(x2, 2.0f * 1.0142630e-3f, -1.0677572e-1f);
  const float du = fmaf(x2 + x2, q, p);
  gd = fmaf(g * (1.0f - s), du * -0.69314718055994530942f, s);
}

typedef _Float16 h2_t __attribute__((ext_vector_type(2)));
typedef _Float16 h8_t __attribute__((ext_vector_type(8)));

__device__ __forceinline__ h2_t gelu_h2(h2_t x) {
  const h2_t U = {(_Float16)3.75f, (_Float16)3.75f};
  const h2_t u = __builtin_elementwise_min(__builtin_elementwise_abs(x), U);
  const h2_t t = u * (h2_t){(_Float16)(2.0f / 3.75f), (_Float16)(2.0f / 3.75f)} + (h2_t){(_Float16)-1.0f, (_Float16)-1.0f};
#define PYTC_H2C(v) ((h2_t){(_Float16)(v), (_Float16)(v)})
  h2_t p = PYTC_H2C(-6.166994737e-02f);
  p = p * t + PYTC_H2C(6.367329291e-02f);
  p = p * t + PYTC_H2C(1.683184914e-01f);
  p = p * t + PYTC_H2C(-3.056981228e-01f);
  p = p * t + PYTC_H2C(7.903670132e-02f);
  p = p * t + PYTC_H2C(1.852329106e-01f);
  p = p * t + PYTC_H2C(-1.855973189e-01f);
  p = p * t + PYTC_H2C(5.694380662e-02f);
#undef PYTC_H2C
  return __builtin_elementwise_max(x, (h2_t){(_Float16)0.0f, (_Float16)0.0f}) - p;
// ... 43 lines not shown
```

### pytorch_connectomics_amd/hip_ops.py

```python
from __future__ import annotations

import ctypes as C
from typing import Optional, Sequence

import torch

from . import _native as nat

_DT = {torch.float32: nat.F32, torch.bfloat16: nat.BF16}


def dtype_code(dt: torch.dtype) -> int:
    try:
        return _DT[dt]
    except KeyError:
        raise TypeError(f"pytorch_connectomics_amd kernels support float32/bfloat16, got {dt}") from None


def require_device(device, what: str = "this inference path") -> None:
    if torch.device(device).type != "cuda":
        raise RuntimeError(f"{what} (pytorch_connectomics_amd) needs a CUDA(HIP) device: there is no CPU path")


def _on_device(t: torch.Tensor, name: str) -> torch.Tensor:
# ... 608 lines not shown
    a.t, a.ab, a.w2_packed, a.b2, a.w3_packed, a.b3 = (t.data_ptr(), None if ab is None else ab.data_ptr(), w2p.data_ptr(),
                                                       b2.data_ptr(), w3p.data_ptr(), b3.data_ptr())
    a.per_sample = _folded_operands(ab, w2p, b2, N, c_in, c_hid)
    a.w3_format = _w3_format(w3p)
    a.res = res.data_ptr() if res is not None else None
    a.res_low = res_low.data_ptr() if res_low is not None else None
    a.res_bias = res_bias.data_ptr() if res_bias is not None else None
    a.y = y.data_ptr()
    a.N, a.rows_per_sample, a.C_in, a.C_hid, a.C_out, a.res_mode = N, rows_per_sample, c_in, c_hid, c_out, res_mode
    a.Di, a.Hi, a.Wi = (int(v) for v in grid)
    nb = N * rows_per_sample * 2 * (c_in + c_out + (c_out if res is not None else 0))
    if hidden_pre is not None:
        _dev(hidden_pre, "hidden_pre")
        _run(f"pw_mlp_train_fwd[{c_in}->{c_hid}->{c_out}]", nb + N * rows_per_sample * 2 * c_hid, nat.lib().pytc_pw_mlp_train_fwd,
             C.byref(a), _p(hidden_pre), _stream())
        return y
    if train_nostore:
        _run(f"pw_mlp_train_fwd_nostore[{c_in}->{c_hid}->{c_out}]", nb, nat.lib().pytc_pw_mlp_train_fwd_nostore, C.byref(a), _stream(),
             symbol=f"pw_mlp_kernel<{c_in // 32}, {c_out // 16}>")
        return y
    if lds:
        _run(f"pw_mlp_fwd[{c_in}->{c_hid}->{c_out}]", nb, nat.lib().pytc_pw_mlp_lds_fwd, C.byref(a), _stream(),
             symbol=f"pw_mlp_lds_kernel<{c_in // 32}, {c_out // 16}>")
        return y
    if chunked:
        _run(f"pw_mlp_fwd[{c_in}->{c_hid}->{c_out}]", nb, nat.lib().pytc_pw_mlp_chunk_fwd, C.byref(a), _stream(),
             symbol=f"pw_mlp_chunk_kernel<{c_in // 32}, {c_out // 16}>")
        return y
    _run(f"pw_mlp_fwd[{c_in}->{c_hid}->{c_out}]", nb, nat.lib().pytc_pw_mlp_fwd, C.byref(a), _stream(),
         symbol=_mlp_symbol(a, f"pw_mlp_kernel<{c_in // 32}, {c_out // 16}>", 0))
    return y


def pw_mlp_lds_supported(c_in: int, c_hid: int, c_out: int) -> bool:
    return bool(nat.lib().pytc_pw_mlp_lds_supported(int(c_in), int(c_hid), int(c_out)))


def pw_mlp_chunk_supported(c_in: int, c_hid: int, c_out: int) -> bool:
    return bool(nat.lib().pytc_pw_mlp_chunk_supported(int(c_in), int(c_hid), int(c_out)))


def pw_gemm_supported(c_in: int, c_out: int) -> bool:
    return bool(nat.lib().pytc_pw_gemm_supported(int(c_in), int(c_out)))


def pw_gemm(x: torch.Tensor, w: torch.Tensor, bias: torch.Tensor, *, N: int, rows_per_sample: int, ab: Optional[torch.Tensor] = None,
            gelu: bool = False, res: Optional[torch.Tensor] = None, res_mode: int = nat.RES_NONE, grid: Sequence[int] = (0, 0, 0),
            res_low: Optional[torch.Tensor] = None, res_bias: Optional[torch.Tensor] = None,
            y: Optional[torch.Tensor] = None) -> torch.Tensor:
    _dev(x, "x"); _dev(w, "w")
    c_out, c_in = int(w.shape[0]), int(w.shape[1])
    if x.dtype not in (torch.bfloat16, torch.float16) or w.dtype != x.dtype or not w.is_contiguous() or int(x.shape[-1]) != c_in:
        raise TypeError(f"pw_gemm: x {tuple(x.shape)} {x.dtype} / w {tuple(w.shape)} {w.dtype}: same 16-bit type, w (C_out, C_in) contiguous")
    out_dt = torch.float16 if gelu else torch.bfloat16
    if y is None:
        y = torch.empty((N, rows_per_sample, c_out), dtype=out_dt, device=x.device)
    else:
        _check_out(y, N * rows_per_sample * c_out, out_dt, "pw_gemm")
    nb = N * rows_per_sample * 2 * (c_in + c_out + (c_out if res is not None else 0)) + 2 * c_in * c_out
    _run(f"pw_gemm[{c_in}->{c_out}]", nb, nat.lib().pytc_pw_gemm_fwd, _p(x), _p(w), _p(bias), _p(ab), _p(y), N, rows_per_sample, c_in,
         c_out, int(x.dtype == torch.float16), int(gelu), _p(res), _p(res_low), _p(res_bias), int(res_mode), *(int(v) for v in grid),
         _stream(), flops=2 * N * rows_per_sample * c_in * c_out, symbol="pw_gemm_lds_kernel")
    return y


def pw_mlp_up_supported(c_in: int, c_hid: int, c_out: int) -> bool:
    return bool(nat.lib().pytc_pw_mlp_up_supported(int(c_in), int(c_hid), int(c_out)))


def pw_mlp_up(x_low: torch.Tensor, taps: torch.Tensor, dw_bias: Optional[torch.Tensor], ab: torch.Tensor, w2p: torch.Tensor,
              b2: torch.Tensor, w3p: torch.Tensor, b3: torch.Tensor, skip: torch.Tensor, *, c_hid: int, c_out: int,
              res_low: Optional[torch.Tensor] = None, res_bias: Optional[torch.Tensor] = None) -> torch.Tensor:
    _dev(x_low, "x_low"); _dev(skip, "skip"); _dev(taps, "taps")
    if x_low.dtype != torch.bfloat16 or skip.dtype != torch.bfloat16:
        raise TypeError("pw_mlp_up runs on bfloat16 activations")
    N, D, H, W, c_in = x_low.shape
    if tuple(skip.shape) != (N, 2 * D, 2 * H, 2 * W, c_out):
        raise ValueError(f"pw_mlp_up: skip shape {tuple(skip.shape)} does not match the up-sampled grid")
    y = torch.empty((N, 2 * D, 2 * H, 2 * W, c_out), dtype=torch.bfloat16, device=x_low.device)
    a = nat.MlpArgs()
    a.t, a.ab, a.w2_packed, a.b2, a.w3_packed, a.b3 = (x_low.data_ptr(), ab.data_ptr(), w2p.data_ptr(), b2.data_ptr(),
                                                       w3p.data_ptr(), b3.data_ptr())
    if w3p.dtype != torch.bfloat16:
        raise TypeError("pw_mlp_up takes the bf16 image of the projection weights")
    a.res = skip.data_ptr()
    if dw_bias is None:
        dw_bias = torch.zeros((c_in,), dtype=torch.float32, device=x_low.device)
    if res_bias is None:
        res_bias = torch.zeros((c_out,), dtype=torch.float32, device=x_low.device)
    a.res_low = res_low.data_ptr() if res_low is not None else None
    a.res_bias = res_bias.data_ptr()
    a.y = y.data_ptr()
    a.N, a.rows_per_sample, a.C_in, a.C_hid, a.C_out, a.res_mode = N, 8 * D * H * W, c_in, c_hid, c_out, nat.RES_UPSAMPLE
    a.Di, a.Hi, a.Wi = D, H, W
    nb = _nbytes(x_low, skip, y) + (_nbytes(res_low) if res_low is not None else 0)
    _run(f"pw_mlp_up_fwd[{c_in}->{c_hid}->{c_out}]", nb, nat.lib().pytc_pw_mlp_up_fwd, C.byref(a), _p(taps), _p(dw_bias),
         _stream())
    return y


def stem_dwconv3d_supported(c_in: int, c: int, K: int) -> bool:
    return bool(nat.lib().pytc_stem_dwconv3d_supported(int(c_in), int(c), int(K)))


def stem_dwconv3d_pack(stem_w: torch.Tensor, stem_b: torch.Tensor, w_taps: torch.Tensor, bias: Optional[torch.Tensor]):
    wx = (w_taps * stem_w.view(1, -1)).contiguous()
    wb = (w_taps * stem_b.view(1, -1)).contiguous()
    cst = (wb.sum(0) + (bias if bias is not None else 0.0)).contiguous()
    image = torch.empty((nat.lib().pytc_stem_dwconv3d_mfma_image_bytes(),), dtype=torch.uint8, device=wx.device)
    _run("stem_dwconv3d_pack_mfma", 0, nat.lib().pytc_stem_dwconv3d_pack_mfma, _p(wx), _p(wb), _p(cst), _p(image), _stream())
    return wx, wb, cst, image


def stem_dwconv3d(x: torch.Tensor, packed):
    wx, wb, cst, image = packed
    _dev(x, "x"); _dev(wx, "wx")
    if x.dtype != torch.float32 or x.shape[-1] != 1:
        raise TypeError("stem_dwconv3d takes the 1-channel fp32 network input")
    N, D, H, W, _ = x.shape
    Cc = wx.shape[1]
    y = torch.empty((N, D, H, W, Cc), dtype=torch.bfloat16, device=x.device)
    slots = nat.lib().pytc_stem_dwconv3d_stat_slots(D, H, W)
    st = torch.empty((N, slots, 2, Cc), dtype=torch.float32, device=x.device)
    _run(f"stem_dwconv3d_fwd[C{Cc}_k3]", _nbytes(x, y), nat.lib().pytc_stem_dwconv3d_fwd, _p(x), _p(wx), _p(wb), _p(cst),
         _p(image), _p(y), _p(st), N, D, H, W, Cc, _stream())
    return y, st


def pw_mlp_stemres(t: torch.Tensor, ab: torch.Tensor, w2p: torch.Tensor, b2: torch.Tensor, w3p: torch.Tensor, b3: torch.Tensor,
                   x0: torch.Tensor, stem_w: torch.Tensor, stem_b: torch.Tensor, *, N: int, rows_per_sample: int, c_in: int,
                   c_hid: int, c_out: int, y: Optional[torch.Tensor] = None) -> torch.Tensor:
    _dev(t, "t"); _dev(x0, "x0")
    if t.dtype != torch.bfloat16 or x0.dtype != torch.float32:
        raise TypeError("pw_mlp_stemres: bf16 activations and the fp32 network input")
    if y is None:
        y = torch.empty((N, rows_per_sample, c_out), dtype=torch.bfloat16, device=t.device)
    else:
        _check_out(y, N * rows_per_sample * c_out, torch.bfloat16, "pw_mlp_stemres")
    a = nat.MlpArgs()
    a.t, a.ab, a.w2_packed, a.b2, a.w3_packed, a.b3 = (t.data_ptr(), None if ab is None else ab.data_ptr(), w2p.data_ptr(),
                                                       b2.data_ptr(), w3p.data_ptr(), b3.data_ptr())
    a.per_sample = _folded_operands(ab, w2p, b2, N, c_in, c_hid)
    a.w3_format = _w3_format(w3p)
    a.res = a.res_low = a.res_bias = None
    a.y = y.data_ptr()
    a.N, a.rows_per_sample, a.C_in, a.C_hid, a.C_out, a.res_mode = N, rows_per_sample, c_in, c_hid, c_out, nat.RES_ADD
    a.Di = a.Hi = a.Wi = 0
    nb = N * rows_per_sample * (2 * (c_in + c_out) + 4)
    _run(f"pw_mlp_fwd[{c_in}->{c_hid}->{c_out}]", nb, nat.lib().pytc_pw_mlp_stemres_fwd, C.byref(a), _p(x0), _p(stem_w),
         _p(stem_b), _stream(), symbol=_mlp_symbol(a, f"pw_mlp_kernel<{c_in // 32}, {c_out // 16}>+stemres", 1))
    return y


_MLP_BWD_CONSTS: dict = {}


def pw_mlp_bwd(dy: torch.Tensor, hidden_pre: torch.Tensor, w3t_p: torch.Tensor, w2t_p: torch.Tensor, *, N: int,
               rows_per_sample: int, c_in: int, c_hid: int, c_out: int):
    _dev(dy, "dy"); _dev(hidden_pre, "hidden_pre")
    if dy.dtype != torch.bfloat16:
        raise TypeError("pw_mlp_bwd runs on bfloat16 activations")
    dev = dy.device
    dx = torch.empty((N, rows_per_sample, c_in), dtype=torch.bfloat16, device=dev)
    dh = torch.empty((N, rows_per_sample, c_hid), dtype=torch.bfloat16, device=dev)
    key = (dev, N, c_in, c_hid, c_out)
    consts = _MLP_BWD_CONSTS.get(key)
    if consts is None:
        consts = (torch.cat([torch.ones((N, 1, c_out), device=dev), torch.zeros((N, 1, c_out), device=dev)], 1).contiguous(),
                  torch.zeros((c_hid,), device=dev), torch.zeros((c_in,), device=dev))
        _MLP_BWD_CONSTS[key] = consts
    ident, zh, zi = consts
    a = nat.MlpArgs()
    a.t, a.ab, a.w2_packed, a.b2, a.w3_packed, a.b3 = (dy.data_ptr(), ident.data_ptr(), w3t_p.data_ptr(), zh.data_ptr(),
                                                       w2t_p.data_ptr(), zi.data_ptr())
    a.w3_format = nat.W3_BF16
    a.res = a.res_low = a.res_bias = None
    a.y = dx.data_ptr()
    a.N, a.rows_per_sample, a.C_in, a.C_hid, a.C_out, a.res_mode = N, rows_per_sample, c_out, c_hid, c_in, nat.RES_NONE
    a.Di = a.Hi = a.Wi = 0
    nb = N * rows_per_sample * 2 * (c_out + 2 * c_hid + c_in)
    _run(f"pw_mlp_bwd[{c_out}->{c_hid}->{c_in}]", nb, nat.lib().pytc_pw_mlp_bwd, C.byref(a), _p(hidden_pre), _p(dh), _stream())
    return dx, dh


def pw_mlp_proj_supported(c_in: int, c_hid: int, c_out: int, c_proj: int) -> bool:
    return bool(nat.lib().pytc_pw_mlp_proj_supported(int(c_in), int(c_hid), int(c_out), int(c_proj)))


def pw_mlp_proj(t: torch.Tensor, w2n: torch.Tensor, b2n: torch.Tensor, w3p: torch.Tensor, b3: torch.Tensor, proj_w: torch.Tensor,
                proj_b: Optional[torch.Tensor], *, N: int, rows_per_sample: int, c_in: int, c_hid: int, c_out: int,
                res: Optional[torch.Tensor] = None, store_y: bool = False):
    _dev(t, "t"); _dev(proj_w, "proj_w")
    if t.dtype != torch.bfloat16 or proj_w.dtype != torch.bfloat16 or proj_w.numel() != 32 * 32:
        raise TypeError("pw_mlp_proj runs on bfloat16 activations and the paired bf16 image of a 32 x 32 projection")
    y = torch.empty((N, rows_per_sample, c_out), dtype=torch.bfloat16, device=t.device) if store_y else None
    z = torch.empty((N, rows_per_sample, 32), dtype=torch.bfloat16, device=t.device)
    a = nat.MlpArgs()
    a.t, a.ab, a.w2_packed, a.b2, a.w3_packed, a.b3 = t.data_ptr(), None, w2n.data_ptr(), b2n.data_ptr(), w3p.data_ptr(), b3.data_ptr()
    a.per_sample = _folded_operands(None, w2n, b2n, N, c_in, c_hid)
    a.w3_format = _w3_format(w3p)
    a.res = res.data_ptr() if res is not None else None
    a.res_low = a.res_bias = None
    a.y = y.data_ptr() if y is not None else None
    a.N, a.rows_per_sample, a.C_in, a.C_hid, a.C_out = N, rows_per_sample, c_in, c_hid, c_out
    a.res_mode = nat.RES_ADD if res is not None else nat.RES_NONE
    a.Di = a.Hi = a.Wi = 0
    nb = N * rows_per_sample * 2 * (c_in + (c_out if res is not None else 0) + (c_out if store_y else 0) + 32)
    _run(f"pw_mlp_fwd[{c_in}->{c_hid}->{c_out}]", nb, nat.lib().pytc_pw_mlp_proj_fwd, C.byref(a), _p(proj_w), _p(proj_b), _p(z),
         int(store_y), _stream(), symbol=f"pw_mlp_dma_kernel<{c_hid // 32}, 3>")
    return y, z


def pw_mlp_head_supported(c_in: int, c_hid: int, c_out: int) -> bool:
    return bool(nat.lib().pytc_pw_mlp_head_supported(int(c_in), int(c_hid), int(c_out)))


def pack_head_fragment(w: torch.Tensor) -> torch.Tensor:
    n_head = w.shape[0]
    if n_head > 16 or w.shape[1] != 32:
        raise ValueError("head weights must be (n_head <= 16, 32)")
    w16 = torch.zeros((16, 32), dtype=torch.float32, device=w.device)
    w16[:n_head] = w
    frag = w16.view(16, 4, 8).permute(1, 0, 2).reshape(64, 8).to(torch.bfloat16)
    return frag.unsqueeze(0).expand(n_head, 64, 8).contiguous()


def pw_mlp_head(t: torch.Tensor, ab: torch.Tensor, w2p: torch.Tensor, b2: torch.Tensor, w3p: torch.Tensor, b3: torch.Tensor,
                head_w: torch.Tensor, head_b: Optional[torch.Tensor], *, N: int, rows_per_sample: int, c_in: int,
                c_hid: int, c_out: int, res: Optional[torch.Tensor] = None, store_y: bool = False):
    _dev(t, "t"); _dev(head_w, "head_w")
    if t.dtype != torch.bfloat16 or head_w.dtype != torch.bfloat16 or tuple(head_w.shape[1:]) != (64, 8):
        raise TypeError("pw_mlp_head runs on bfloat16 activations and a bf16 head fragment image (n_head, 64, 8)")
    n_head = head_w.shape[0]
    y = torch.empty((N, rows_per_sample, c_out), dtype=torch.bfloat16, device=t.device) if store_y else None
    logits = torch.empty((N, rows_per_sample, n_head), dtype=torch.float32, device=t.device)
    a = nat.MlpArgs()
    a.t, a.ab, a.w2_packed, a.b2, a.w3_packed, a.b3 = (t.data_ptr(), None if ab is None else ab.data_ptr(), w2p.data_ptr(),
                                                       b2.data_ptr(), w3p.data_ptr(), b3.data_ptr())
    a.per_sample = _folded_operands(ab, w2p, b2, N, c_in, c_hid)
    a.w3_format = _w3_format(w3p)
    a.res = res.data_ptr() if res is not None else None
    a.res_low = a.res_bias = None
    a.y = y.data_ptr() if y is not None else None
    a.N, a.rows_per_sample, a.C_in, a.C_hid, a.C_out = N, rows_per_sample, c_in, c_hid, c_out
    a.res_mode = nat.RES_ADD if res is not None else nat.RES_NONE
    a.Di = a.Hi = a.Wi = 0
    nb = N * rows_per_sample * (2 * (c_in + (c_out if res is not None else 0) + (c_out if store_y else 0)) + 4 * n_head)
    _run(f"pw_mlp_fwd[{c_in}->{c_hid}->{c_out}]", nb, nat.lib().pytc_pw_mlp_head_fwd, C.byref(a), _p(head_w),
         _p(head_b), _p(logits), n_head, int(store_y), _stream(),
         symbol=_mlp_symbol(a, f"pw_mlp_kernel<{c_in // 32}, {c_out // 16}>+head", 2))
    return y, logits


def dwmix_supported(x: torch.Tensor, c_hid: int, c_out: int) -> bool:
    if x.dim() != 5 or x.dtype != torch.bfloat16:
        return False
    _, D, H, W, Cc = x.shape
    return bool(nat.lib().pytc_dwmix_supported(D, H, W, Cc, int(c_hid), int(c_out), dtype_code(x.dtype)))


def dwmix(x: torch.Tensor, w_taps: torch.Tensor, dw_bias: Optional[torch.Tensor], w2n: torch.Tensor, b2n: torch.Tensor,
          w3p: torch.Tensor, b3: torch.Tensor, *, c_hid: int, c_out: int = 32, residual: bool = True, y: Optional[torch.Tensor] = None,
          head_w: Optional[torch.Tensor] = None, head_b: Optional[torch.Tensor] = None, store_y: bool = True):
    _dev(x, "x"); _dev(w_taps, "w_taps"); _dev(w2n, "w2n"); _dev(w3p, "w3p")
    N, D, H, W, Cc = x.shape
    if x.dtype != torch.bfloat16 or w2n.dtype != torch.bfloat16 or w3p.dtype != torch.float16:
        raise TypeError("dwmix runs on bfloat16 activations, per-sample bf16 expand images and the fp16 projection image")
    if tuple(w2n.shape) != (N, c_hid * Cc) or tuple(b2n.shape) != (N, c_hid) or tuple(w_taps.shape) != (27, Cc):
        raise ValueError(f"dwmix: operands do not match N={N}, C={Cc}, C_hid={c_hid}: w2n {tuple(w2n.shape)}, b2n {tuple(b2n.shape)}, taps {tuple(w_taps.shape)}")
    logits = None
    n_head = 0
    if head_w is not None:
        if head_w.dtype != torch.bfloat16 or tuple(head_w.shape[1:]) != (64, 8):
            raise TypeError("dwmix: the head fragment image is (n_head, 64, 8) bf16 (pack_head_fragment)")
        n_head = int(head_w.shape[0])
        logits = torch.empty((N, D, H, W, n_head), dtype=torch.float32, device=x.device)
        if not store_y:
            y = None
    if y is None and (head_w is None or store_y):
        y = torch.empty((N, D, H, W, c_out), dtype=torch.bfloat16, device=x.device)
    if y is not None and (tuple(y.shape) != (N, D, H, W, c_out) or y.dtype != torch.bfloat16 or not y.is_contiguous()):
        raise ValueError(f"dwmix: output buffer must be contiguous bf16 {(N, D, H, W, c_out)}")
    nb = _nbytes(x) * (2 if residual else 1) + _nbytes(y, logits)
    _run(f"dwmix_fwd[{Cc}->{c_hid}->{c_out}]", nb, nat.lib().pytc_dwmix_fwd, _p(x), _p(w_taps), _p(dw_bias), _p(w2n), _p(b2n), _p(w3p),
         _p(b3), int(bool(residual)), _p(y), _p(head_w), _p(head_b), _p(logits), n_head, N, D, H, W, Cc, int(c_hid), int(c_out),
         dtype_code(x.dtype), _stream(), symbol="dwconv3d_k3_mfma_kernel+mix" + ("+head" if head_w is not None else ""))
    return y if head_w is None else (y, logits)


def conv3d_pack_weight(w: torch.Tensor, dtype: torch.dtype) -> torch.Tensor:
    _dev(w, "w")
    co, ci, kd, kh, kw = w.shape
    n = nat.lib().pytc_conv3d_packed_elems(co, ci, kd, kh, kw, dtype_code(dtype))
    packed = torch.empty((n,), dtype=dtype, device=w.device)
    _run("conv3d_pack_weight", _nbytes(w, packed), nat.lib().pytc_conv3d_pack_weight, _p(w), co, ci, kd, kh, kw,
         _p(packed), dtype_code(dtype), _stream())
    return packed


def conv3d_pack_weight_dgrad(w: torch.Tensor, dtype: torch.dtype) -> torch.Tensor:
    _dev(w, "w")
    co, ci, kd, kh, kw = w.shape
    n = nat.lib().pytc_conv3d_packed_elems(ci, co, kd, kh, kw, dtype_code(dtype))
    packed = torch.empty((n,), dtype=dtype, device=w.device)
    _run("conv3d_pack_weight_dgrad", _nbytes(w, packed), nat.lib().pytc_conv3d_pack_weight_dgrad, _p(w), co, ci, kd, kh, kw,
         _p(packed), dtype_code(dtype), _stream())
# ... 1564 lines not shown
```

### pytorch_connectomics_amd/models/architectures/mednext.py

```python
from __future__ import annotations

import os
from typing import Dict, List, Optional, Sequence, Union

import torch
import torch.nn as nn

from ... import _native as nat
from ... import hip_ops as ops

SMALL_ROWS_TWO_GEMMS = int(os.environ.get("PYTC_MIXER_TWO_GEMM_ROWS", "0"))

L0_SUBBATCH = int(os.environ.get("PYTC_L0_SUBBATCH", "0"))


def _conv_nd(dim: str):
    if dim == "3d":
        return nn.Conv3d, nn.ConvTranspose3d
    if dim == "2d":
        return nn.Conv2d, nn.ConvTranspose2d
    raise ValueError(f"dim must be '2d' or '3d', got {dim!r}")


class _ChannelLayerNorm(nn.Module):
# ... 238 lines not shown
            count = float((2 * D - 1) * (2 * H - 1) * (2 * W - 1))
        else:
            t, st = ops.dwconv3d(x, taps, b1, K=K, stride=2 if kind == "down" else 1, stats=not is_ln)
            count = float(t.shape[1] * t.shape[2] * t.shape[3])
        gamma, beta = self._vec(m.norm, "weight", m.norm.weight), self._vec(m.norm, "bias", m.norm.bias)
        if is_ln:
            t = ops.layernorm_rows(t, gamma, beta, m.norm.eps)
            ab = None
        else:
            ab = None
        _, Do, Ho, Wo, _ = t.shape
        rows = Do * Ho * Wo
        small = (self.fused and dt == torch.bfloat16 and not m.grn and not is_ln and N * rows < SMALL_ROWS_TWO_GEMMS
                 and ops.pw_conv_paired_supported(c_in=C, c_out=c_hid, in_dtype=dt, out_dtype=dt)
                 and ops.pw_conv_paired_supported(c_in=c_hid, c_out=c_out, in_dtype=dt, out_dtype=dt))
        if (not small and self.fused and dt == torch.bfloat16 and not m.grn and not is_ln and m.conv2.bias is not None
                and m.conv3.bias is not None and head is None and ops.MLP_F16_PROJECT
                and (rows <= self.deep_gemm_rows or (self.deep_gemm_cin and C >= self.deep_gemm_cin))
                and ops.pw_gemm_supported(C, c_hid) and ops.pw_gemm_supported(c_hid, c_out)):
            ab = ops.groupnorm_finalize(st, count, gamma, beta, m.norm.eps)
            return self._block_deep_gemm(m, x, t, ab, skip, (N, D, H, W, C), (Do, Ho, Wo), c_hid, c_out, out)
        if (not small and self.fused and dt == torch.bfloat16 and not m.grn and not is_ln and m.conv2.bias is not None
                and m.conv3.bias is not None and ops.pw_mlp_supported(C, c_hid, c_out)):
            ab, w2x, b2x = self._fold(m, st, count, C, c_hid)
            if (head is not None and kind == "block" and head.weight.shape[1] <= 16
                    and ops.pw_mlp_head_supported(C, c_hid, c_out)):
                _, logits = ops.pw_mlp_head(t, ab, w2x, b2x,
                                            self._pw_paired(m.conv3, project=True), self._vec(m.conv3, "bias", m.conv3.bias),
                                            self._head_w(head), self._vec(head, "bias", head.bias), N=N,
                                            rows_per_sample=rows, c_in=C, c_hid=c_hid, c_out=c_out,
                                            res=x if m.do_res else None, store_y=False)
                return None, logits.view(N, Do, Ho, Wo, -1)
            if (proj is not None and head is None and out is None and kind == "block" and ab is None and ops.MLP_F16_PROJECT
                    and tuple(proj.weight.shape[:2]) == (32, c_out) and ops.pw_mlp_proj_supported(C, c_hid, c_out, 32)):
                _, z = ops.pw_mlp_proj(t, w2x, b2x, self._pw_paired(m.conv3, project=True), self._vec(m.conv3, "bias", m.conv3.bias),
                                       self._pw_paired(proj), self._vec(proj, "bias", proj.bias), N=N, rows_per_sample=rows, c_in=C,
                                       c_hid=c_hid, c_out=c_out, res=x if m.do_res else None, store_y=False)
                return None, z.view(N, Do, Ho, Wo, 32)
            return self._block_fused(m, x, t, ab, skip, (N, D, H, W, C), (Do, Ho, Wo), c_hid, c_out, out, w2x, b2x)
        if not is_ln:
            ab = ops.groupnorm_finalize(st, count, gamma, beta, m.norm.eps)
        G = {}
        if small:
            h = ops.pw_conv(t, self._pw_paired(m.conv2), self._vec(m.conv2, "bias", m.conv2.bias), N=N, rows_per_sample=rows,
                            c_in=C, c_out=c_hid, out_dtype=dt, ab=ab, w_paired=True)
            w3, b3 = self._pw_paired(m.conv3), self._vec(m.conv3, "bias", m.conv3.bias)
            G = dict(pre_act=nat.ACT_GELU, w_paired=True)
        else:
            h = ops.pw_conv(t, self._pw(m.conv2, dt), self._vec(m.conv2, "bias", m.conv2.bias), N=N,
                            rows_per_sample=rows, c_in=C, c_out=c_hid, out_dtype=dt, ab=ab, act=nat.ACT_GELU)
            if m.grn:
                h = self._grn(m, h, N, (Do, Ho, Wo), c_hid, kind)
            w3, b3 = self._pw(m.conv3, dt), self._vec(m.conv3, "bias", m.conv3.bias)
        if kind == "block":
            y = ops.pw_conv(h, w3, b3, N=N, rows_per_sample=rows, c_in=c_hid, c_out=c_out, out_dtype=dt,
                            res=x if m.do_res else None, res_mode=nat.RES_ADD if m.do_res else nat.RES_NONE, **G)
        elif kind == "down":
            res = None
            if m.resample_do_res:
                res = ops.pw_conv(x, self._pw(m.res_conv, dt), self._vec(m.res_conv, "bias", m.res_conv.bias),
                                  N=N, rows_per_sample=rows, c_in=C, c_out=c_out, out_dtype=dt, gather=2,
                                  grid=(D, H, W))
            y = ops.pw_conv(h, w3, b3, N=N, rows_per_sample=rows, c_in=c_hid, c_out=c_out, out_dtype=dt,
                            res=res, res_mode=nat.RES_ADD if res is not None else nat.RES_NONE, **G)
        else:
            if skip is None:
                skip = torch.zeros((N, Do, Ho, Wo, c_out), dtype=dt, device=x.device)
            res_low = res_bias = None
            if m.resample_do_res:
                res_bias = self._vec(m.res_conv, "bias", m.res_conv.bias)
                res_low = ops.pw_conv(x, self._pw(m.res_conv, dt, transposed=True), res_bias, N=N,
                                      rows_per_sample=D * H * W, c_in=C, c_out=c_out, out_dtype=dt)
            y = ops.pw_conv(h, w3, b3, N=N, rows_per_sample=rows, c_in=c_hid, c_out=c_out, out_dtype=dt,
                            res=skip, res_mode=nat.RES_UPSAMPLE, grid=(Do, Ho, Wo), res_low=res_low,
                            res_bias=res_bias, **G)
        return y.view(N, Do, Ho, Wo, c_out)


def _block_dwmix(self, m, x, taps, b1, c_hid, c_out, head=None, out=None):
    N, D, H, W, C = x.shape
    _, st = ops.dwconv3d(x, taps, b1, K=3, store=False)
    w2n, b2n = ops.groupnorm_fold_mlp(st, float(D * H * W), self._vec(m.norm, "weight", m.norm.weight), self._vec(m.norm, "bias", m.norm.bias),
                                      m.norm.eps, self._w2_matrix(m.conv2), self._vec(m.conv2, "bias", m.conv2.bias))
    w3, b3 = self._pw_paired(m.conv3, project=True), self._vec(m.conv3, "bias", m.conv3.bias)
    if head is not None:
        _, logits = ops.dwmix(x, taps, b1, w2n, b2n, w3, b3, c_hid=c_hid, c_out=c_out, residual=bool(m.do_res),
                              head_w=self._head_w(head), head_b=self._vec(head, "bias", head.bias), store_y=False)
        return None, logits
    if out is not None and tuple(out.shape) != (N, D, H, W, c_out):
        raise ValueError(f"block output buffer {tuple(out.shape)} != {(N, D, H, W, c_out)}")
    return ops.dwmix(x, taps, b1, w2n, b2n, w3, b3, c_hid=c_hid, c_out=c_out, residual=bool(m.do_res), y=out)


HipBlockOps._block_dwmix = None


def _stem_block_fused(self, stem: nn.Module, m, x_cl: torch.Tensor, out: Optional[torch.Tensor] = None) -> Optional[torch.Tensor]:
    N, D, H, W, cin = x_cl.shape
    C = stem.weight.shape[0]
    K = m.conv1.weight.shape[-1]
    if (cin != 1 or x_cl.dtype != torch.float32 or stem.bias is None or m.kind != "block" or not m.do_res or m.grn
            or not isinstance(m.norm, nn.GroupNorm) or m.dim != "3d" or m.conv2.bias is None or m.conv3.bias is None
            or m.conv1.weight.shape[0] != C or W % 4 != 0 or not ops.stem_dwconv3d_supported(cin, C, K)):
        return None
    c_hid, c_out = m.conv2.weight.shape[0], m.conv3.weight.shape[0]
    if c_out != C or not ops.pw_mlp_supported(C, c_hid, c_out):
        return None
    sw = self.cache.get(("stemw", id(stem)), [stem.weight], lambda: stem.weight.detach().float().reshape(-1).bfloat16().float().contiguous())
    sb = self._vec(stem, "bias", stem.bias)
    taps, _ = self._taps(m.conv1)
    packed = self.cache.get(("stemdw", id(stem), id(m.conv1)), [stem.weight, stem.bias, m.conv1.weight, m.conv1.bias],
                            lambda: ops.stem_dwconv3d_pack(sw, sb, taps, self._vec(m.conv1, "bias", m.conv1.bias)))
    t, st = ops.stem_dwconv3d(x_cl, packed)
    rows = D * H * W
    ab, w2x, b2x = self._fold(m, st, float(rows), C, c_hid)
    y = ops.pw_mlp_stemres(t, ab, w2x, b2x,
                           self._pw_paired(m.conv3, project=True), self._vec(m.conv3, "bias", m.conv3.bias), x_cl.reshape(N, rows), sw, sb,
                           N=N, rows_per_sample=rows, c_in=C, c_hid=c_hid, c_out=c_out,
                           y=None if out is None else out.view(N, rows, c_out))
    return y.view(N, D, H, W, c_out)


HipBlockOps._stem_block_fused = None


def _block_fused(self, m, x, t, ab, skip, ishape, oshape, c_hid, c_out, out=None, w2=None, b2=None):
    N, D, H, W, C = ishape
    Do, Ho, Wo = oshape
    rows = Do * Ho * Wo
    dt = torch.bfloat16
    if w2 is None:
        w2, b2 = self._pw_paired(m.conv2), self._vec(m.conv2, "bias", m.conv2.bias)
    w3, b3 = self._pw_paired(m.conv3, project=True), self._vec(m.conv3, "bias", m.conv3.bias)
    kw = dict(N=N, rows_per_sample=rows, c_in=C, c_hid=c_hid, c_out=c_out)
    if (self.lds_mixer_rows and N * rows >= self.lds_mixer_rows and w3.dtype == torch.float16
            and ops.pw_mlp_lds_supported(C, c_hid, c_out)):
        kw["lds"] = True
    chunk_ok = (self.chunk_mixer_rows and N * rows >= self.chunk_mixer_rows and w3.dtype == torch.float16
                and ops.pw_mlp_chunk_supported(C, c_hid, c_out))
    if chunk_ok and (c_hid >= self.chunk_mixer_hid or (C, c_out) == (128, 64)):
        kw.pop("lds", None)
        kw["chunked"] = True
    if out is not None:
        if tuple(out.shape) != (N, Do, Ho, Wo, c_out):
            raise ValueError(f"block output buffer {tuple(out.shape)} != {(N, Do, Ho, Wo, c_out)}")
        kw["y"] = out.view(N, rows, c_out)
    if m.kind == "block":
        y = ops.pw_mlp(t, ab, w2, b2, w3, b3, res=x if m.do_res else None,
                       res_mode=nat.RES_ADD if m.do_res else nat.RES_NONE, **kw)
    elif m.kind == "down":
        res = None
        if m.resample_do_res:
            paired = ops.pw_conv_paired_supported(c_in=C, c_out=c_out, in_dtype=dt, out_dtype=dt, gather=2)
            wres = self._pw_paired(m.res_conv) if paired else self._pw(m.res_conv, dt)
            res = ops.pw_conv(x, wres, self._vec(m.res_conv, "bias", m.res_conv.bias), N=N, rows_per_sample=rows,
                              c_in=C, c_out=c_out, out_dtype=dt, gather=2, grid=(D, H, W), w_paired=paired)
        y = ops.pw_mlp(t, ab, w2, b2, w3, b3, res=res, res_mode=nat.RES_ADD if res is not None else nat.RES_NONE, **kw)
    else:
        if skip is None:
            skip = torch.zeros((N, Do, Ho, Wo, c_out), dtype=dt, device=x.device)
        res_low = res_bias = None
        if m.resample_do_res:
            res_bias = self._vec(m.res_conv, "bias", m.res_conv.bias)
            paired = ops.pw_conv_paired_supported(c_in=C, c_out=c_out, in_dtype=dt, out_dtype=dt)
            wres = self._pw_paired(m.res_conv, transposed=True) if paired else self._pw(m.res_conv, dt, transposed=True)
            res_low = ops.pw_conv(x, wres, res_bias, N=N, rows_per_sample=D * H * W, c_in=C, c_out=c_out,
                                  out_dtype=dt, w_paired=paired)
        y = ops.pw_mlp(t, ab, w2, b2, w3, b3, res=skip, res_mode=nat.RES_UPSAMPLE, grid=(Do, Ho, Wo),
                       res_low=res_low, res_bias=res_bias, **kw)
    return y.view(N, Do, Ho, Wo, c_out)


def _block_deep_gemm(self, m, x, t, ab, skip, ishape, oshape, c_hid, c_out, out=None):
    N, D, H, W, C = ishape
    Do, Ho, Wo = oshape
    rows = Do * Ho * Wo
    dt = torch.bfloat16
    w2 = self.cache.get(("gw2", id(m.conv2)), [m.conv2.weight],
                        lambda: m.conv2.weight.detach().float().reshape(c_hid, C).to(torch.bfloat16).contiguous())
    w3 = self.cache.get(("gw3", id(m.conv3)), [m.conv3.weight],
                        lambda: m.conv3.weight.detach().float().reshape(c_out, c_hid).to(torch.float16).contiguous())
    b2, b3 = self._vec(m.conv2, "bias", m.conv2.bias), self._vec(m.conv3, "bias", m.conv3.bias)
    h = ops.pw_gemm(t.view(N, rows, C), w2, b2, N=N, rows_per_sample=rows, ab=ab, gelu=True)
    kw = dict(N=N, rows_per_sample=rows)
    if out is not None:
        kw["y"] = out.view(N, rows, c_out)
    if m.kind == "block":
        y = ops.pw_gemm(h, w3, b3, res=x if m.do_res else None, res_mode=nat.RES_ADD if m.do_res else nat.RES_NONE, **kw)
    elif m.kind == "down":
        res = None
        if m.resample_do_res:
            paired = ops.pw_conv_paired_supported(c_in=C, c_out=c_out, in_dtype=dt, out_dtype=dt, gather=2)
            wres = self._pw_paired(m.res_conv) if paired else self._pw(m.res_conv, dt)
            res = ops.pw_conv(x, wres, self._vec(m.res_conv, "bias", m.res_conv.bias), N=N, rows_per_sample=rows,
                              c_in=C, c_out=c_out, out_dtype=dt, gather=2, grid=(D, H, W), w_paired=paired)
        y = ops.pw_gemm(h, w3, b3, res=res, res_mode=nat.RES_ADD if res is not None else nat.RES_NONE, **kw)
    else:
        if skip is None:
            skip = torch.zeros((N, Do, Ho, Wo, c_out), dtype=dt, device=x.device)
        res_low = res_bias = None
        if m.resample_do_res:
            res_bias = self._vec(m.res_conv, "bias", m.res_conv.bias)
            paired = ops.pw_conv_paired_supported(c_in=C, c_out=c_out, in_dtype=dt, out_dtype=dt)
            wres = self._pw_paired(m.res_conv, transposed=True) if paired else self._pw(m.res_conv, dt, transposed=True)
            res_low = ops.pw_conv(x, wres, res_bias, N=N, rows_per_sample=D * H * W, c_in=C, c_out=c_out, out_dtype=dt, w_paired=paired)
        y = ops.pw_gemm(h, w3, b3, res=skip, res_mode=nat.RES_UPSAMPLE, grid=(Do, Ho, Wo), res_low=res_low, res_bias=res_bias, **kw)
    return y.view(N, Do, Ho, Wo, c_out)


def _up_block_fused(self, m, x, skip, taps, b1, c_hid, c_out):
    N, D, H, W, C = x.shape
    dt = torch.bfloat16
    _, st = ops.dwconv3d(x, taps, b1, K=3, transposed=True, stats=True, store=False)
    ab = ops.groupnorm_finalize(st, float((2 * D - 1) * (2 * H - 1) * (2 * W - 1)), self._vec(m.norm, "weight", m.norm.weight),
                                self._vec(m.norm, "bias", m.norm.bias), m.norm.eps)
    res_low = res_bias = None
    if m.resample_do_res:
        res_bias = self._vec(m.res_conv, "bias", m.res_conv.bias)
        paired = ops.pw_conv_paired_supported(c_in=C, c_out=c_out, in_dtype=dt, out_dtype=dt)
        wres = self._pw_paired(m.res_conv, transposed=True) if paired else self._pw(m.res_conv, dt, transposed=True)
        res_low = ops.pw_conv(x, wres, res_bias, N=N, rows_per_sample=D * H * W, c_in=C, c_out=c_out, out_dtype=dt,
                              w_paired=paired)
    return ops.pw_mlp_up(x, taps, b1, ab, self._pw_paired(m.conv2), self._vec(m.conv2, "bias", m.conv2.bias),
                         self._pw_paired(m.conv3), self._vec(m.conv3, "bias", m.conv3.bias), skip.contiguous(),
                         c_hid=c_hid, c_out=c_out, res_low=res_low, res_bias=res_bias)


HipBlockOps._up_block_fused = _up_block_fused
HipBlockOps._block_deep_gemm = _block_deep_gemm
HipBlockOps._block_fused = _block_fused
HipBlockOps._stem_block_fused = _stem_block_fused
HipBlockOps._block_dwmix = _block_dwmix


def resolve_compute_dtype(module_pref: Optional[torch.dtype]) -> torch.dtype:
    if module_pref is not None:
        return module_pref
    if torch.is_autocast_enabled("cuda"):
        adt = torch.get_autocast_dtype("cuda")
        if adt == torch.bfloat16:
            return torch.bfloat16
        if adt == torch.float16:
            raise RuntimeError("fp16 autocast is not supported by the MI355X engine; use bf16-mixed")
    return torch.float32


def embed_stencil_2d(w: torch.Tensor) -> torch.Tensor:
    k = w.shape[-1]
    out = w.new_zeros((w.shape[0], w.shape[1], k, k, k))
    out[:, :, k // 2] = w
    return out


def to_channels_last(x: torch.Tensor) -> torch.Tensor:
    if x.shape[1] == 1:
        return x.reshape(x.shape[0], *x.shape[2:], 1)
    return x.permute(0, 2, 3, 4, 1).contiguous()


def to_channels_first(y: torch.Tensor) -> torch.Tensor:
    if y.shape[-1] == 1:
        return y.reshape(y.shape[0], 1, *y.shape[1:-1])
    return y.permute(0, 4, 1, 2, 3).contiguous()


class MedNeXt(nn.Module):

    def __init__(self, in_channels: int, n_channels: int, n_classes: int, exp_r: Union[int, Sequence[int]] = 4,
                 kernel_size: int = 7, enc_kernel_size: Optional[int] = None,
                 dec_kernel_size: Optional[int] = None, deep_supervision: bool = False, do_res: bool = False,
                 do_res_up_down: bool = False, checkpoint_style: Optional[str] = None,
                 block_counts: Sequence[int] = (2, 2, 2, 2, 2, 2, 2, 2, 2), norm_type: str = "group",
                 dim: str = "3d", grn: bool = False):
        super().__init__()
        if checkpoint_style not in (None, "outside_block"):
            raise ValueError("checkpoint_style must be None or 'outside_block'")
        if len(block_counts) != 9:
            raise ValueError("block_counts must have exactly 9 elements")
        self.do_ds = deep_supervision
        self.inside_block_checkpointing = False
        self.outside_block_checkpointing = checkpoint_style == "outside_block"
        self.checkpoint_policy = "auto"
        if kernel_size is not None:
            enc_kernel_size = dec_kernel_size = kernel_size
        conv, _ = _conv_nd(dim)
        if isinstance(exp_r, int):
            exp_r = [exp_r] * 9
        exp_r = list(exp_r)
        n = n_channels
        self.dim = dim
        self.stem = conv(in_channels, n, kernel_size=1)

        def blocks(c, r, k, count):
            return nn.Sequential(*[MedNeXtBlock(c, c, r, k, do_res, norm_type, dim=dim, grn=grn)
                                   for _ in range(count)])

        for lvl in range(4):
            setattr(self, f"enc_block_{lvl}", blocks(n << lvl, exp_r[lvl], enc_kernel_size, block_counts[lvl]))
            setattr(self, f"down_{lvl}", MedNeXtDownBlock(n << lvl, n << (lvl + 1), exp_r[lvl + 1], enc_kernel_size,
                                                          do_res=do_res_up_down, norm_type=norm_type, dim=dim, grn=grn))
        self.bottleneck = blocks(n << 4, exp_r[4], dec_kernel_size, block_counts[4])
        for i, lvl in enumerate((3, 2, 1, 0)):
            setattr(self, f"up_{lvl}", MedNeXtUpBlock(n << (lvl + 1), n << lvl, exp_r[5 + i], dec_kernel_size,
                                                      do_res=do_res_up_down, norm_type=norm_type, dim=dim, grn=grn))
            setattr(self, f"dec_block_{lvl}", blocks(n << lvl, exp_r[5 + i], dec_kernel_size, block_counts[5 + i]))
        self.out_0 = OutBlock(n, n_classes, dim)
        self.dummy_tensor = nn.Parameter(torch.tensor([1.0]), requires_grad=True)
        if deep_supervision:
            for h in (1, 2, 3, 4):
                setattr(self, f"out_{h}", OutBlock(n << h, n_classes, dim))
        self.block_counts = list(block_counts)
        self.compute_dtype: Optional[torch.dtype] = None
        self._hip = HipBlockOps()
        self.fuse_head = True
        self.fuse_stem = True
        self.l0_subbatch = L0_SUBBATCH

# ... 170 lines not shown
```

Measured before the change: 1.820 billion voxels/s.

## Fuse residual 1x1 convs of down/up blocks into the mixer kernels

Down blocks at levels 0/1 now compute the strided residual 1x1 conv inside the MLP mixer kernel from the block input, rather than launching a separate pw_conv and reading its output back. The level-0 up block on the LDS-resident mixer likewise computes the low-resolution residual conv in-kernel for even positions, with the conv weights kept in LDS. This removes two launches and the round trip of an intermediate residual tensor through memory. In exchange the mixer kernels do extra MFMA work, hold more registers (which may lower occupancy), and use more LDS.

```diff
diff --git a/include/pytc_hip.h b/include/pytc_hip.h
--- a/include/pytc_hip.h
+++ b/include/pytc_hip.h
@@ -7,7 +7,7 @@
 extern "C" {
 #endif
 
-#define PYTC_ABI_VERSION 12
+#define PYTC_ABI_VERSION 13
 
 #define PYTC_OK 0
 #define PYTC_ERR_INVALID 1
@@ -203,6 +203,8 @@
 
 int pytc_pw_mlp_lds_supported(int C_in, int C_hid, int C_out);
 int pytc_pw_mlp_lds_fwd(const pytc_mlp_args* a, void* stream);
+int pytc_pw_mlp_lds_upres_supported(int C_in, int C_hid, int C_out);
+int pytc_pw_mlp_lds_upres_fwd(const pytc_mlp_args* a, const void* x_low, const void* res_w_packed_t, void* stream);
 int pytc_pw_mlp_dma_applies(const pytc_mlp_args* a, int ignore_res_mode);
 int pytc_pw_mlp_proj_supported(int C_in, int C_hid, int C_out, int C_proj);
 int pytc_pw_mlp_proj_fwd(const pytc_mlp_args* a, const void* proj_w, const float* proj_b, void* z, int store_y, void* stream);
@@ -219,6 +221,9 @@
 int pytc_pw_mlp_head_supported(int C_in, int C_hid, int C_out);
 int pytc_pw_mlp_stemres_fwd(const pytc_mlp_args* a, const float* stem_x, const float* stem_w, const float* stem_b,
                             void* stream);
+int pytc_pw_mlp_convres_supported(int C_in, int C_hid, int C_out);
+int pytc_pw_mlp_convres_fwd(const pytc_mlp_args* a, const void* x, const void* res_w_packed, const float* res_conv_bias, int Di, int Hi,
+                            int Wi, void* stream);
 int pytc_stem_dwconv3d_stat_slots(int D, int H, int W);
 int pytc_stem_dwconv3d_supported(int C_in, int C, int K);
 int pytc_stem_dwconv3d_mfma_image_bytes(void);
diff --git a/pytorch_connectomics_amd/csrc/pw_common.h b/pytorch_connectomics_amd/csrc/pw_common.h
--- a/pytorch_connectomics_amd/csrc/pw_common.h
+++ b/pytorch_connectomics_amd/csrc/pw_common.h
@@ -71,7 +71,7 @@
 
 template <typename TO, int NCH, bool GELU_BWD = false, int COUT = 0>
 __device__ __forceinline__ void finish_and_store(float (&v)[NCH], const EpiParams& e, int n, long orow, int o0,
-                                                 const float* pre = nullptr, const int* pos = nullptr) {
+                                                 const float* pre = nullptr, const int* pos = nullptr, const float* rlow = nullptr) {
   const int C_out = COUT > 0 ? COUT : e.C_out;
   TO* yn = reinterpret_cast<TO*>(e.y) + (long)n * e.rps_out * C_out;
   const TO* resn = e.res ? reinterpret_cast<const TO*>(e.res) + (long)n * e.rps_out * C_out : nullptr;
@@ -155,7 +155,10 @@
     } else {
       const int oz = pz - 1, oy = py - 1, ox = px - 1;
       float rl[NCH];
-      if (e.res_low && !((oz | oy | ox) & 1)) {
+      if (rlow && !((oz | oy | ox) & 1)) {
+#pragma unroll
+        for (int i = 0; i < NCH; ++i) rl[i] = rlow[i];
+      } else if (e.res_low && !((oz | oy | ox) & 1)) {
         const TO* rp = reinterpret_cast<const TO*>(e.res_low) +
                        ((((long)n * e.Gl_d + (oz >> 1)) * e.Gl_h + (oy >> 1)) * e.Gl_w + (ox >> 1)) * C_out + o0;
         if (full) VecIO<TO, NCH>::load(rp, rl);
@@ -187,6 +190,40 @@
     for (int i = 0; i < NCH; ++i)
       if (o0 + i < C_out) yn[off + i] = from_f32<TO>(v[i]);
   }
+}
+
+template <int KS, int NT>
+__device__ __forceinline__ void pw_pair_gemm(const bf16x8_t* __restrict__ w, const float* __restrict__ bias, int pr, int lane,
+                                             const bf16x8_t (&b)[KS][NT], f32x4_t (&acc)[2][NT]) {
+  const int o0 = pr * 32 + (lane >> 4) * 8;
+  float bv[8];
+#pragma unroll
+  for (int j = 0; j < 8; ++j) bv[j] = 0.f;
+  if (bias) {
+    VecIO<float, 4>::load(bias + o0, reinterpret_cast<float(&)[4]>(bv[0]));
+    VecIO<float, 4>::load(bias + o0 + 4, reinterpret_cast<float(&)[4]>(bv[4]));
+  }
+#pragma unroll
+  for (int nt = 0; nt < NT; ++nt) {
+    acc[0][nt] = f32x4_t{bv[0], bv[1], bv[2], bv[3]};
+    acc[1][nt] = f32x4_t{bv[4], bv[5], bv[6], bv[7]};
+  }
+#pragma unroll
+  for (int mt = 0; mt < 2; ++mt)
+#pragma unroll
+    for (int ks = 0; ks < KS; ++ks) {
+      const bf16x8_t a = w[((long)(pr * 2 + mt) * KS + ks) * 64 + lane];
+#pragma unroll
+      for (int nt = 0; nt < NT; ++nt) acc[mt][nt] = Mma<bf16_t>::mma(a, b[ks][nt], acc[mt][nt]);
+    }
+}
+template <int NT>
+__device__ __forceinline__ void pw_pair_stored(const f32x4_t (&acc)[2][NT], int nt, float (&v)[8]) {
+  float f[8];
+#pragma unroll
+  for (int j = 0; j < 4; ++j) { f[j] = acc[0][nt][j]; f[4 + j] = acc[1][nt][j]; }
+  const bf16x8_t rb = Mma<bf16_t>::from_floats(f);
+  VecIO<bf16_t, 8>::load(reinterpret_cast<const bf16_t*>(&rb), v);
 }
 
 template <typename TI, int EPL>
diff --git a/pytorch_connectomics_amd/csrc/pw_fast_kernels.hip b/pytorch_connectomics_amd/csrc/pw_fast_kernels.hip
--- a/pytorch_connectomics_amd/csrc/pw_fast_kernels.hip
+++ b/pytorch_connectomics_amd/csrc/pw_fast_kernels.hip
@@ -105,27 +105,8 @@
         rpre[nt] = *reinterpret_cast<const uint4*>(resn + rr * p.C_out + o0);
       }
     }
-    float b[8];
-#pragma unroll
-    for (int j = 0; j < 8; ++j) b[j] = 0.f;
-    if (p.bias) {
-      VecIO<float, 4>::load(p.bias + o0, reinterpret_cast<float(&)[4]>(b[0]));
-      VecIO<float, 4>::load(p.bias + o0 + 4, reinterpret_cast<float(&)[4]>(b[4]));
-    }
     f32x4_t acc[2][NT];
-#pragma unroll
-    for (int nt = 0; nt < NT; ++nt) {
-      acc[0][nt] = f32x4_t{b[0], b[1], b[2], b[3]};
-      acc[1][nt] = f32x4_t{b[4], b[5], b[6], b[7]};
-    }
-#pragma unroll
-    for (int mt = 0; mt < 2; ++mt)
-#pragma unroll
-      for (int ks = 0; ks < KS; ++ks) {
-        const bf16x8_t a = p.w[((long)(pr * 2 + mt) * KS + ks) * 64 + lane];
-#pragma unroll
-        for (int nt = 0; nt < NT; ++nt) acc[mt][nt] = Mma<bf16_t>::mma(a, bact[ks][nt], acc[mt][nt]);
-      }
+    pw_pair_gemm<KS, NT>(p.w, p.bias, pr, lane, bact, acc);
 #pragma unroll
     for (int nt = 0; nt < NT; ++nt) {
       if (orow[nt] >= p.rps) continue;
diff --git a/pytorch_connectomics_amd/csrc/pw_mlp_kernels.hip b/pytorch_connectomics_amd/csrc/pw_mlp_kernels.hip
--- a/pytorch_connectomics_amd/csrc/pw_mlp_kernels.hip
+++ b/pytorch_connectomics_amd/csrc/pw_mlp_kernels.hip
@@ -23,6 +23,11 @@
   const float* stem_x;
   const float* stem_w;
   const float* stem_b;
+  const bf16_t* cres_x;
+  const bf16x8_t* cres_w;
+  const float* cres_b;
+  long cres_rps_in;
+  int cres_Hi, cres_Wi, cres_Ho, cres_Wo;
   bf16_t* hp;
   int round_h;
   const bf16_t* hp_in;
@@ -34,7 +39,8 @@
   return regs <= 64 ? 4 : (regs <= 112 ? 3 : (regs <= 200 ? 2 : 1));
 }
 
-template <int KS_IN, int MO, int NT, int GELU_MODE, bool HEAD = false, bool STEMRES = false, bool STOREH = false, bool BWD = false>
+template <int KS_IN, int MO, int NT, int GELU_MODE, bool HEAD = false, bool STEMRES = false, bool STOREH = false, bool BWD = false,
+          bool CONVRES = false>
 __global__ void __launch_bounds__(256, mlp_waves_per_simd(KS_IN, MO, NT))
 pw_mlp_kernel(MlpParams p) {
   constexpr int CIN = KS_IN * 32, COUT = MO * 16;
@@ -42,7 +48,8 @@
   static_assert(!STEMRES || (MO == 2 && (MO / 2) * NT <= 4), "the stem-recomputing residual covers C_out = 32");
   static_assert(!HEAD || MO == 2, "the fused head covers C_out = 32");
   static_assert(GELU_MODE == 1 || GELU_MODE == 3, "sigmoid-form or packed-fp16 GELU");
-  constexpr bool PREFETCH_RES = (MO / 2) * NT <= 4;
+  static_assert(!CONVRES || !(HEAD || STEMRES || STOREH || BWD), "the conv-recomputing residual is a form of the plain inference mixer");
+  constexpr bool PREFETCH_RES = !CONVRES && (MO / 2) * NT <= 4;
   const int wave = threadIdx.x >> 6, lane = threadIdx.x & 63;
   const int n = blockIdx.y;
   constexpr bool WARM = KS_IN * MO >= 32;
@@ -77,6 +84,27 @@
         bact[ks][nt] = ld_stream(reinterpret_cast<const bf16x8_t*>(tn + rr * CIN + ks * 32 + kb * 8), p.e.nt);
       }
   }
+  bf16x8_t xres[CONVRES ? KS_IN : 1][CONVRES ? NT : 1];
+  if constexpr (CONVRES) {
+    const bf16_t* xn = p.cres_x + (long)n * p.cres_rps_in * CIN;
+    const unsigned ur = (unsigned)row0, gw = (unsigned)p.cres_Wo, gh = (unsigned)p.cres_Ho;
+    const unsigned t0 = ur / gw;
+    const int bx = (int)(ur - t0 * gw);
+    const int bz = (int)(t0 / gh);
+    const int by = (int)(t0 - (unsigned)bz * gh);
+    const int last_z = (int)((unsigned)(p.rps - 1) / (gw * gh));
+#pragma unroll
+    for (int nt = 0; nt < NT; ++nt) {
+      int px = bx + nt * 16 + r, py = by, pz = bz;
+      while (px >= p.cres_Wo) { px -= p.cres_Wo; ++py; }
+      while (py >= p.cres_Ho) { py -= p.cres_Ho; ++pz; }
+      if (orow[nt] >= p.rps) { pz = last_z; py = p.cres_Ho - 1; px = p.cres_Wo - 1; }
+      const long irow = ((long)(2 * pz) * p.cres_Hi + 2 * py) * p.cres_Wi + 2 * px;
+#pragma unroll
+      for (int ks = 0; ks < KS_IN; ++ks)
+        xres[ks][nt] = ld_stream(reinterpret_cast<const bf16x8_t*>(xn + irow * CIN + ks * 32 + kb * 8), p.e.nt);
+    }
+  }
   const float* an = p.ab + (long)n * 2 * CIN;
 #pragma unroll
   for (int ks = 0; ks < KS_IN; ++ks) {
@@ -267,6 +295,8 @@
   }
 #pragma unroll
   for (int pr = 0; pr < MO / 2; ++pr) {
+    f32x4_t racc[2][CONVRES ? NT : 1];
+    if constexpr (CONVRES) pw_pair_gemm<KS_IN, NT>(p.cres_w, p.cres_b, pr, lane, xres, racc);
 #pragma unroll
     for (int nt = 0; nt < NT; ++nt) {
       if (orow[nt] >= p.rps) continue;
@@ -276,7 +306,11 @@
         v[j] = acc2[2 * pr][nt][j];
         v[4 + j] = acc2[2 * pr + 1][nt][j];
       }
-      if (use_pre) {
+      if constexpr (CONVRES) {
+        float pre[8];
+        pw_pair_stored<NT>(racc, nt, pre);
+        finish_and_store<bf16_t, 8, false, COUT>(v, p.e, n, orow[nt], pr * 32 + kb * 8, pre);
+      } else if (use_pre) {
         float pre[8];
         VecIO<bf16_t, 8>::load(reinterpret_cast<const bf16_t*>(&rpre[PREFETCH_RES ? pr : 0][PREFETCH_RES ? nt : 0]), pre);
         finish_and_store<bf16_t, 8, false, COUT>(v, p.e, n, orow[nt], pr * 32 + kb * 8, pre, ups ? upos[nt] : nullptr);
@@ -856,6 +890,50 @@
   return PYTC_OK;
 }
 
+extern "C" int pytc_pw_mlp_convres_supported(int C_in, int C_hid, int C_out) {
+  if (tuning_get(K_mlp_convres) == 0) return 0;
+  return (((C_in == 32 && C_out == 64) || (C_in == 64 && C_out == 128)) && C_hid % 32 == 0 && C_hid >= 32) ? 1 : 0;
+}
+
+extern "C" int pytc_pw_mlp_convres_fwd(const pytc_mlp_args* a, const void* x, const void* res_w_packed, const float* res_conv_bias,
+                                       int Di, int Hi, int Wi, void* stream) {
+  PYTC_REQUIRE(a && a->t && (a->ab || a->per_sample) && a->w2_packed && a->w3_packed && a->b2 && a->b3 && a->y && x && res_w_packed,
+               "pw_mlp_convres: null pointer");
+  PYTC_REQUIRE(!(a->ab && a->per_sample), "pw_mlp_convres: per-sample (norm-folded) expand operands come without an affine");
+  PYTC_REQUIRE(a->N >= 1 && a->rows_per_sample >= 1 && a->rows_per_sample < (1L << 31), "pw_mlp_convres: bad shape");
+  PYTC_REQUIRE(Di >= 1 && Hi >= 1 && Wi >= 1, "pw_mlp_convres: the block-input grid");
+  const int Do = (Di - 1) / 2 + 1, Ho = (Hi - 1) / 2 + 1, Wo = (Wi - 1) / 2 + 1;
+  PYTC_REQUIRE((long)Do * Ho * Wo == a->rows_per_sample, "pw_mlp_convres: the block-input grid does not match the output rows");
+  if (!pytc_pw_mlp_convres_supported(a->C_in, a->C_hid, a->C_out)) {
+    set_error("pw_mlp_convres: no fused kernel for C_in=%d C_hid=%d C_out=%d", a->C_in, a->C_hid, a->C_out);
+    return PYTC_ERR_UNSUPPORTED;
+  }
+  MlpParams p{};
+  p.t = (const bf16_t*)a->t; p.ab = a->ab; p.w2 = (const bf16x8_t*)a->w2_packed; p.b2 = a->b2;
+  p.w3 = (const bf16x8_t*)a->w3_packed; p.b3 = a->b3;
+  p.rps = a->rows_per_sample; p.C_in = a->C_in; p.C_hid = a->C_hid; p.C_out = a->C_out; p.HC = a->C_hid / 32;
+  p.w2_stride = (long)(a->C_hid / 16) * (a->C_in / 32) * 64;
+  p.e.res = a->y;
+  p.e.y = a->y;
+  p.e.rps_out = a->rows_per_sample; p.e.C_out = a->C_out; p.e.res_mode = PYTC_RES_ADD;
+  p.e.nt = 0;
+  p.cres_x = (const bf16_t*)x; p.cres_w = (const bf16x8_t*)res_w_packed; p.cres_b = res_conv_bias;
+  p.cres_rps_in = (long)Di * Hi * Wi; p.cres_Hi = Hi; p.cres_Wi = Wi; p.cres_Ho = Ho; p.cres_Wo = Wo;
+  p.w3_f16 = a->w3_format == PYTC_W3_F16 ? 1 : 0;
+  hipStream_t s = (hipStream_t)stream;
+  if (a->C_in == 32) {
+    dim3 grid((unsigned)((p.rps + 4L * 4 * 16 - 1) / (4L * 4 * 16)), (unsigned)a->N), block(256);
+    if (p.w3_f16) hipLaunchKernelGGL((pw_mlp_kernel<1, 4, 4, 3, false, false, false, false, true>), grid, block, 0, s, p);
+    else hipLaunchKernelGGL((pw_mlp_kernel<1, 4, 4, 1, false, false, false, false, true>), grid, block, 0, s, p);
+  } else {
+    dim3 grid((unsigned)((p.rps + 4L * 2 * 16 - 1) / (4L * 2 * 16)), (unsigned)a->N), block(256);
+    if (p.w3_f16) hipLaunchKernelGGL((pw_mlp_kernel<2, 8, 2, 3, false, false, false, false, true>), grid, block, 0, s, p);
+    else hipLaunchKernelGGL((pw_mlp_kernel<2, 8, 2, 1, false, false, false, false, true>), grid, block, 0, s, p);
+  }
+  PYTC_LAUNCH_CHECK("pw_mlp_convres");
+  return PYTC_OK;
+}
+
 extern "C" int pytc_pw_mlp_dma_applies(const pytc_mlp_args* a, int ignore_res_mode) {
   if (!a) return 0;
   MlpParams p{};
diff --git a/pytorch_connectomics_amd/csrc/pw_mlp_lds_kernels.hip b/pytorch_connectomics_amd/csrc/pw_mlp_lds_kernels.hip
--- a/pytorch_connectomics_amd/csrc/pw_mlp_lds_kernels.hip
+++ b/pytorch_connectomics_amd/csrc/pw_mlp_lds_kernels.hip
@@ -15,6 +15,8 @@
   long rps;
   int N, C_in, C_hid, C_out, HC;
   long w2_stride;
+  const bf16_t* ur_x;
+  const bf16x8_t* ur_w;
 };
 
 template <int KS_IN, int MO, int NT>
@@ -46,7 +48,7 @@
   }
 }
 
-template <int KS_IN, int MO, int NT, int NWAVES, int WPS>
+template <int KS_IN, int MO, int NT, int NWAVES, int WPS, bool UPRES = false>
 __global__ void __launch_bounds__(NWAVES * 64, WPS)
 pw_mlp_lds_kernel(MlpLdsParams p) {
   constexpr int CIN = KS_IN * 32, COUT = MO * 16;
@@ -59,6 +61,10 @@
   const bool folded = p.ab == nullptr;
   const int n_w2 = p.C_hid * CIN / 8, n_w3 = COUT * p.C_hid / 8;
   for (int i = tid; i < n_w3; i += NWAVES * 64) lw3[i] = p.w3[i];
+  bf16x8_t* lwr = reinterpret_cast<bf16x8_t*>(lds_raw + (size_t)p.C_hid * (CIN + COUT) * 2 + (size_t)p.C_hid * 4);
+  if constexpr (UPRES) {
+    for (int i = tid; i < MO * KS_IN * 64; i += NWAVES * 64) lwr[i] = p.ur_w[i];
+  }
   const long Ts = (p.rps + NT * 16 - 1) / (NT * 16);
   const long G = Ts * p.N;
   const long g_end = G * (blockIdx.x + 1) / gridDim.x;
@@ -170,15 +176,51 @@
           upos[nt][0] = pz; upos[nt][1] = py; upos[nt][2] = px;
         }
       }
+      bf16x8_t xl[UPRES ? KS_IN : 1][UPRES ? NT : 1];
+      bool wave_even = false;
+      if constexpr (UPRES) {
+        bool even[NT];
+        bool any = false;
+#pragma unroll
+        for (int nt = 0; nt < NT; ++nt) {
+          even[nt] = orow[nt] < p.rps && (upos[nt][0] & upos[nt][1] & upos[nt][2] & 1);
+          any = any || even[nt];
+        }
+        wave_even = __builtin_amdgcn_ballot_w64(any) != 0;
+        if (wave_even) {
+          const bf16_t* xn = p.ur_x + (long)n * ((long)p.e.Gl_d * p.e.Gl_h * p.e.Gl_w) * CIN;
+#pragma unroll
+          for (int nt = 0; nt < NT; ++nt) {
+            const long lrow = even[nt] ? ((long)((upos[nt][0] - 1) >> 1) * p.e.Gl_h + ((upos[nt][1] - 1) >> 1)) * p.e.Gl_w + ((upos[nt][2] - 1) >> 1) : 0L;
+#pragma unroll
+            for (int ks = 0; ks < KS_IN; ++ks)
+              xl[ks][nt] = ld_stream(reinterpret_cast<const bf16x8_t*>(xn + lrow * CIN + ks * 32 + kb * 8), p.e.nt);
+          }
+        }
+      }
 #pragma unroll
       for (int pr = 0; pr < MO / 2; ++pr) {
+        f32x4_t racc[2][UPRES ? NT : 1];
+        if constexpr (UPRES) {
+          if (wave_even) {
+            pw_pair_gemm<KS_IN, NT>(lwr, p.e.res_bias, pr, lane, xl, racc);
+          } else {
+#pragma unroll
+            for (int nt = 0; nt < NT; ++nt) racc[0][nt] = racc[1][nt] = f32x4_t{0.f, 0.f, 0.f, 0.f};
+          }
+        }
 #pragma unroll
         for (int nt = 0; nt < NT; ++nt) {
           if (orow[nt] >= p.rps) continue;
           float v[8];
 #pragma unroll
           for (int j = 0; j < 4; ++j) { v[j] = acc2[2 * pr][nt][j]; v[4 + j] = acc2[2 * pr + 1][nt][j]; }
-          if (with_res) {
+          if constexpr (UPRES) {
+            float pre[8], rl[8];
+            VecIO<bf16_t, 8>::load(reinterpret_cast<const bf16_t*>(&cur.res[pr][nt]), pre);
+            pw_pair_stored<NT>(racc, nt, rl);
+            finish_and_store<bf16_t, 8, false, COUT>(v, p.e, n, orow[nt], pr * 32 + kb * 8, pre, upos[nt], rl);
+          } else if (with_res) {
             float pre[8];
             VecIO<bf16_t, 8>::load(reinterpret_cast<const bf16_t*>(&cur.res[pr][nt]), pre);
             finish_and_store<bf16_t, 8, false, COUT>(v, p.e, n, orow[nt], pr * 32 + kb * 8, pre, ups ? upos[nt] : nullptr);
@@ -192,9 +234,9 @@
   }
 }
 
-template <int KS_IN, int MO, int NT, int NWAVES, int WPS>
+template <int KS_IN, int MO, int NT, int NWAVES, int WPS, bool UPRES = false>
 static void launch_mlp_lds_v(const MlpLdsParams& p, size_t lds, hipStream_t s) {
-  auto kern = &pw_mlp_lds_kernel<KS_IN, MO, NT, NWAVES, WPS>;
+  auto kern = &pw_mlp_lds_kernel<KS_IN, MO, NT, NWAVES, WPS, UPRES>;
   if (!ensure_dynamic_lds(reinterpret_cast<const void*>(kern), 160 * 1024, "pw_mlp_lds")) return;
   const long tiles = ((p.rps + NT * 16 - 1) / (NT * 16)) * p.N;
   const int by_lds = (int)((160 * 1024) / lds), by_waves = WPS * 4 / NWAVES;
@@ -205,15 +247,15 @@
   hipLaunchKernelGGL(kern, dim3((unsigned)blocks), dim3(NWAVES * 64), lds, s, p);
 }
 
-template <int KS_IN, int MO, int NT>
+template <int KS_IN, int MO, int NT, bool UPRES = false>
 static void launch_mlp_lds(const MlpLdsParams& p, int variant, hipStream_t s) {
-  const size_t lds = (size_t)p.C_hid * (p.C_in + p.C_out) * 2 + (size_t)p.C_hid * 4;
+  const size_t lds = (size_t)p.C_hid * (p.C_in + p.C_out) * 2 + (size_t)p.C_hid * 4 + (UPRES ? (size_t)p.C_in * p.C_out * 2 : 0);
   if (variant == 0) variant = (KS_IN == 4 && MO == 8) ? 3 : (MO == 2 ? 2 : 4);
   switch (variant) {
-    case 1: launch_mlp_lds_v<KS_IN, MO, NT, 8, 4>(p, lds, s); break;
-    case 2: launch_mlp_lds_v<KS_IN, MO, NT, 16, 4>(p, lds, s); break;
-    case 3: launch_mlp_lds_v<KS_IN, MO, NT, 8, 2>(p, lds, s); break;
-    default: launch_mlp_lds_v<KS_IN, MO, NT, 12, 3>(p, lds, s); break;
+    case 1: launch_mlp_lds_v<KS_IN, MO, NT, 8, 4, UPRES>(p, lds, s); break;
+    case 2: launch_mlp_lds_v<KS_IN, MO, NT, 16, 4, UPRES>(p, lds, s); break;
+    case 3: launch_mlp_lds_v<KS_IN, MO, NT, 8, 2, UPRES>(p, lds, s); break;
+    default: launch_mlp_lds_v<KS_IN, MO, NT, 12, 3, UPRES>(p, lds, s); break;
   }
 }
 
@@ -229,7 +271,27 @@
   return (shape && lds <= 160 * 1024) ? 1 : 0;
 }
 
-extern "C" int pytc_pw_mlp_lds_fwd(const pytc_mlp_args* a, void* stream) {
+static int mlp_lds_impl(const pytc_mlp_args* a, const void* x_low, const void* res_w_t, void* stream);
+
+extern "C" int pytc_pw_mlp_lds_fwd(const pytc_mlp_args* a, void* stream) { return mlp_lds_impl(a, nullptr, nullptr, stream); }
+
+extern "C" int pytc_pw_mlp_lds_upres_supported(int C_in, int C_hid, int C_out) {
+  if (tuning_get(K_mlp_lds_upres) == 0 || C_in != 64 || C_out != 32 || C_hid % 32 || C_hid < 32) return 0;
+  const size_t lds = (size_t)C_hid * (C_in + C_out) * 2 + (size_t)C_hid * 4 + (size_t)C_in * C_out * 2;
+  return lds <= 160 * 1024 ? 1 : 0;
+}
+
+extern "C" int pytc_pw_mlp_lds_upres_fwd(const pytc_mlp_args* a, const void* x_low, const void* res_w_packed_t, void* stream) {
+  PYTC_REQUIRE(a && x_low && res_w_packed_t, "pw_mlp_lds_upres: null pointer");
+  PYTC_REQUIRE(a->res_mode == PYTC_RES_UPSAMPLE, "pw_mlp_lds_upres: the up block's epilogue (PYTC_RES_UPSAMPLE)");
+  if (!pytc_pw_mlp_lds_upres_supported(a->C_in, a->C_hid, a->C_out)) {
+    set_error("pw_mlp_lds_upres: no kernel for C_in=%d C_hid=%d C_out=%d", a->C_in, a->C_hid, a->C_out);
+    return PYTC_ERR_UNSUPPORTED;
+  }
+  return mlp_lds_impl(a, x_low, res_w_packed_t, stream);
+}
+
+static int mlp_lds_impl(const pytc_mlp_args* a, const void* x_low, const void* res_w_t, void* stream) {
   PYTC_REQUIRE(a && a->t && (a->ab || a->per_sample) && a->w2_packed && a->w3_packed && a->b2 && a->b3 && a->y, "pw_mlp_lds: null pointer");
   PYTC_REQUIRE(!(a->ab && a->per_sample), "pw_mlp_lds: per-sample (norm-folded) expand operands come without an affine");
   PYTC_REQUIRE(a->w3_format == PYTC_W3_F16, "pw_mlp_lds: the projection image must be fp16 (pytc_pw_pack_weight_paired_f16)");
@@ -244,10 +306,11 @@
   p.w3 = (const h8_t*)a->w3_packed; p.b3 = a->b3;
   p.rps = a->rows_per_sample; p.N = a->N; p.C_in = a->C_in; p.C_hid = a->C_hid; p.C_out = a->C_out; p.HC = a->C_hid / 32;
   p.w2_stride = (long)(a->C_hid / 16) * (a->C_in / 32) * 64;
-  p.e.res = a->res; p.e.res_low = a->res_low; p.e.res_bias = a->res_bias; p.e.y = a->y;
+  p.e.res = a->res; p.e.res_low = x_low ? nullptr : a->res_low; p.e.res_bias = a->res_bias; p.e.y = a->y;
   p.e.rps_out = a->rows_per_sample; p.e.C_out = a->C_out; p.e.res_mode = a->res_mode;
   p.e.nt = 0;
   p.e.Go_d = p.e.Go_h = p.e.Go_w = p.e.Gl_d = p.e.Gl_h = p.e.Gl_w = 0;
+  p.ur_x = (const bf16_t*)x_low; p.ur_w = (const bf16x8_t*)res_w_t;
   if (a->res_mode == PYTC_RES_UPSAMPLE) {
     PYTC_REQUIRE((long)a->Di * a->Hi * a->Wi == a->rows_per_sample && !(a->Di & 1) && !(a->Hi & 1) && !(a->Wi & 1) &&
                  a->rows_per_sample < (1L << 31), "pw_mlp_lds: RES_UPSAMPLE needs the (even) output grid");
@@ -257,7 +320,8 @@
   hipStream_t s = (hipStream_t)stream;
   const int ks = a->C_in / 32, mo = a->C_out / 16;
   const int variant = tuning_get(K_mlp_lds_variant);
-  if (ks == 2 && mo == 2) launch_mlp_lds<2, 2, 2>(p, variant, s);
+  if (x_low) launch_mlp_lds<2, 2, 2, true>(p, variant, s);
+  else if (ks == 2 && mo == 2) launch_mlp_lds<2, 2, 2>(p, variant, s);
   else if (ks == 2 && mo == 4) launch_mlp_lds<2, 4, 2>(p, variant, s);
   else if (ks == 4 && mo == 4) launch_mlp_lds<4, 4, 2>(p, variant, s);
   else launch_mlp_lds<4, 8, 2>(p, variant, s);
diff --git a/pytorch_connectomics_amd/csrc/pytc_common.h b/pytorch_connectomics_amd/csrc/pytc_common.h
--- a/pytorch_connectomics_amd/csrc/pytc_common.h
+++ b/pytorch_connectomics_amd/csrc/pytc_common.h
@@ -75,9 +75,11 @@
   X(elementwise_vec, 1, "16-byte vector forms of the norm-apply / elementwise training kernels; 0 = the scalar kernels")           \
   X(mixer_bwd_rc_slot_div, 1, "recomputing mixer backward: divide the slot count (fewer, longer slots)")                           \
   X(mlp_chunk_variant, 0, "chunked-hidden mixer (pw_mlp_chunk_kernels.hip): tile shape of the launch")                             \
+  X(mlp_convres, 1, "down blocks of levels 0 / 1: residual 1x1 conv computed inside the mixer; 0 = its own launch, loaded back")  \
   X(mlp_dma, 1, "level-0 mixer with DMA-prefetched row tiles (pw_mlp_dma_kernel); 0 = one tile per wave")                          \
   X(mlp_dma_rows, 1 << 20, "fewest rows of a launch that takes the DMA mixer")                                                     \
   X(mlp_dma_wgs, 0, "DMA mixer: workgroups per sample; 0 = chosen from the row count")                                             \
+  X(mlp_lds_upres, 1, "level-0 up block on the LDS-resident mixer: low-resolution residual conv computed in the kernel; 0 = own launch") \
   X(mlp_lds_variant, 0, "LDS-resident mixer (pw_mlp_lds_kernels.hip): tile shape of the launch")                                   \
   X(norm_bwd_from_wgrad_flat, 1, "GroupNorm-backward epilogue of the expand weight gradient as one flat kernel; 0 = chunked")      \
   X(pw_gemm_rows, 0, "LDS-tiled 1x1 GEMM: 64 / 128 forces the rows per workgroup; 0 = by problem size")                            \
diff --git a/pytorch_connectomics_amd/hip_ops.py b/pytorch_connectomics_amd/hip_ops.py
--- a/pytorch_connectomics_amd/hip_ops.py
+++ b/pytorch_connectomics_amd/hip_ops.py
@@ -784,6 +784,72 @@
     return y
 
 
+def pw_mlp_convres_supported(c_in: int, c_hid: int, c_out: int) -> bool:
+    return bool(nat.lib().pytc_pw_mlp_convres_supported(int(c_in), int(c_hid), int(c_out)))
+
+
+def pw_mlp_convres(t: torch.Tensor, ab: Optional[torch.Tensor], w2p: torch.Tensor, b2: torch.Tensor, w3p: torch.Tensor, b3: torch.Tensor,
+                   x: torch.Tensor, wres_p: torch.Tensor, res_bias: Optional[torch.Tensor], *, N: int, rows_per_sample: int, c_in: int,
+                   c_hid: int, c_out: int, y: Optional[torch.Tensor] = None) -> torch.Tensor:
+    _dev(t, "t"); _dev(x, "x")
+    if t.dtype != torch.bfloat16 or x.dtype != torch.bfloat16 or wres_p.dtype != torch.bfloat16:
+        raise TypeError("pw_mlp_convres runs on bfloat16 activations and the bf16 image of the residual conv")
+    if x.dim() != 5 or int(x.shape[0]) != N or int(x.shape[-1]) != c_in or not x.is_contiguous():
+        raise ValueError(f"pw_mlp_convres: block input {tuple(x.shape)}: contiguous (N, D, H, W, {c_in})")
+    if y is None:
+        y = torch.empty((N, rows_per_sample, c_out), dtype=torch.bfloat16, device=t.device)
+    else:
+        _check_out(y, N * rows_per_sample * c_out, torch.bfloat16, "pw_mlp_convres")
+    a = nat.MlpArgs()
+    a.t, a.ab, a.w2_packed, a.b2, a.w3_packed, a.b3 = (t.data_ptr(), None if ab is None else ab.data_ptr(), w2p.data_ptr(),
+                                                       b2.data_ptr(), w3p.data_ptr(), b3.data_ptr())
+    a.per_sample = _folded_operands(ab, w2p, b2, N, c_in, c_hid)
+    a.w3_format = _w3_format(w3p)
+    a.res = a.res_low = a.res_bias = None
+    a.y = y.data_ptr()
+    a.N, a.rows_per_sample, a.C_in, a.C_hid, a.C_out, a.res_mode = N, rows_per_sample, c_in, c_hid, c_out, nat.RES_ADD
+    a.Di = a.Hi = a.Wi = 0
+    nb = N * rows_per_sample * 2 * (2 * c_in + c_out)
+    _run(f"pw_mlp_fwd[{c_in}->{c_hid}->{c_out}]", nb, nat.lib().pytc_pw_mlp_convres_fwd, C.byref(a), _p(x), _p(wres_p), _p(res_bias),
+         *(int(v) for v in x.shape[1:4]), _stream(), symbol=f"pw_mlp_kernel<{c_in // 32}, {c_out // 16}>+convres")
+    return y
+
+
+def pw_mlp_lds_upres_supported(c_in: int, c_hid: int, c_out: int) -> bool:
+    return bool(nat.lib().pytc_pw_mlp_lds_upres_supported(int(c_in), int(c_hid), int(c_out)))
+
+
+def pw_mlp_lds_upres(t: torch.Tensor, ab: Optional[torch.Tensor], w2p: torch.Tensor, b2: torch.Tensor, w3p: torch.Tensor, b3: torch.Tensor,
+                     skip: torch.Tensor, x_low: torch.Tensor, wres_t_p: torch.Tensor, res_bias: Optional[torch.Tensor], *, N: int,
+                     rows_per_sample: int, c_in: int, c_hid: int, c_out: int, grid: Sequence[int],
+                     y: Optional[torch.Tensor] = None) -> torch.Tensor:
+    _dev(t, "t"); _dev(x_low, "x_low"); _dev(skip, "skip")
+    if t.dtype != torch.bfloat16 or x_low.dtype != torch.bfloat16 or skip.dtype != torch.bfloat16 or wres_t_p.dtype != torch.bfloat16:
+        raise TypeError("pw_mlp_lds_upres runs on bfloat16 activations and the bf16 image of the residual conv")
+    Do, Ho, Wo = (int(v) for v in grid)
+    if (x_low.dim() != 5 or tuple(x_low.shape) != (N, Do // 2, Ho // 2, Wo // 2, c_in) or not x_low.is_contiguous()
+            or Do * Ho * Wo != rows_per_sample):
+        raise ValueError(f"pw_mlp_lds_upres: block input {tuple(x_low.shape)} does not match the output grid {(Do, Ho, Wo)}")
+    if y is None:
+        y = torch.empty((N, rows_per_sample, c_out), dtype=torch.bfloat16, device=t.device)
+    else:
+        _check_out(y, N * rows_per_sample * c_out, torch.bfloat16, "pw_mlp_lds_upres")
+    a = nat.MlpArgs()
+    a.t, a.ab, a.w2_packed, a.b2, a.w3_packed, a.b3 = (t.data_ptr(), None if ab is None else ab.data_ptr(), w2p.data_ptr(),
+                                                       b2.data_ptr(), w3p.data_ptr(), b3.data_ptr())
+    a.per_sample = _folded_operands(ab, w2p, b2, N, c_in, c_hid)
+    a.w3_format = _w3_format(w3p)
+    a.res, a.res_low = skip.data_ptr(), None
+    a.res_bias = res_bias.data_ptr() if res_bias is not None else None
+    a.y = y.data_ptr()
+    a.N, a.rows_per_sample, a.C_in, a.C_hid, a.C_out, a.res_mode = N, rows_per_sample, c_in, c_hid, c_out, nat.RES_UPSAMPLE
+    a.Di, a.Hi, a.Wi = Do, Ho, Wo
+    nb = N * rows_per_sample * 2 * (c_in + 2 * c_out) + _nbytes(x_low)
+    _run(f"pw_mlp_fwd[{c_in}->{c_hid}->{c_out}]", nb, nat.lib().pytc_pw_mlp_lds_upres_fwd, C.byref(a), _p(x_low), _p(wres_t_p), _stream(),
+         symbol=f"pw_mlp_lds_kernel<{c_in // 32}, {c_out // 16}>+upres")
+    return y
+
+
 _MLP_BWD_CONSTS: dict = {}
 
 
diff --git a/pytorch_connectomics_amd/models/architectures/mednext.py b/pytorch_connectomics_amd/models/architectures/mednext.py
--- a/pytorch_connectomics_amd/models/architectures/mednext.py
+++ b/pytorch_connectomics_amd/models/architectures/mednext.py
@@ -414,6 +414,11 @@
         res = None
         if m.resample_do_res:
             paired = ops.pw_conv_paired_supported(c_in=C, c_out=c_out, in_dtype=dt, out_dtype=dt, gather=2)
+            if (paired and x.dtype == dt and x.is_contiguous() and not kw.get("lds") and not kw.get("chunked")
+                    and ops.pw_mlp_convres_supported(C, c_hid, c_out)):
+                y = ops.pw_mlp_convres(t, ab, w2, b2, w3, b3, x, self._pw_paired(m.res_conv),
+                                       self._vec(m.res_conv, "bias", m.res_conv.bias), **kw)
+                return y.view(N, Do, Ho, Wo, c_out)
             wres = self._pw_paired(m.res_conv) if paired else self._pw(m.res_conv, dt)
             res = ops.pw_conv(x, wres, self._vec(m.res_conv, "bias", m.res_conv.bias), N=N, rows_per_sample=rows,
                               c_in=C, c_out=c_out, out_dtype=dt, gather=2, grid=(D, H, W), w_paired=paired)
@@ -425,6 +430,12 @@
         if m.resample_do_res:
             res_bias = self._vec(m.res_conv, "bias", m.res_conv.bias)
             paired = ops.pw_conv_paired_supported(c_in=C, c_out=c_out, in_dtype=dt, out_dtype=dt)
+            if (paired and kw.get("lds") and x.dtype == dt and x.is_contiguous() and skip.dtype == dt
+                    and (Do, Ho, Wo) == (2 * D, 2 * H, 2 * W) and ops.pw_mlp_lds_upres_supported(C, c_hid, c_out)):
+                kw.pop("lds")
+                y = ops.pw_mlp_lds_upres(t, ab, w2, b2, w3, b3, skip.contiguous(), x, self._pw_paired(m.res_conv, transposed=True),
+                                         res_bias, grid=(Do, Ho, Wo), **kw)
+                return y.view(N, Do, Ho, Wo, c_out)
             wres = self._pw_paired(m.res_conv, transposed=True) if paired else self._pw(m.res_conv, dt, transposed=True)
             res_low = ops.pw_conv(x, wres, res_bias, N=N, rows_per_sample=D * H * W, c_in=C, c_out=c_out,
                                   out_dtype=dt, w_paired=paired)
```

Measured after the change: 1.849 billion voxels/s, median of 6. 1.02x the previous value.
